# Guillaume-SOULIER/SOS-Radiative-Transfer

Measured on AMD Instinct MI355X. Metric: SOS columns/sec to 1e-4 convergence (Ntau=200, Nmu=128), higher is better.
Workload: dtype f64

## Files before the change

### __graft_entry__.py

```python
import os
import subprocess
import sys

ROOT = os.path.dirname(os.path.abspath(__file__))
PKG = os.path.join(ROOT, "sos-radiative-transfer_amd")
CSRC = os.path.join(PKG, "csrc")
LIB = os.path.join(PKG, "libsosrt.so")
SOURCES = ["api.hip", "kernels.hip", "jn_gemm.hip", "jn_gemm_f32.hip", "transport_fast.hip", "transport_ring.hip", "transport_scan.hip", "order_loop.hip", "epilogue.hip", "plan.cpp", "comm.cpp"]
HEADERS = ["kernels.hpp", "plan.hpp", "transport_util.hpp", "transport_scan_body.hpp", "jn_gemm_tile.hpp", "comm.hpp", os.path.join(ROOT, "include", "sosrt.h")]


OBJDIR = os.path.join(PKG, "build")
FLAGS = ["-O3", "--offload-arch=gfx950", "-std=c++17", "-fPIC", "-Wno-unused-value"]


def _deps():
    return [h if os.path.isabs(h) else os.path.join(CSRC, h) for h in HEADERS]


def _obj(src):
    return os.path.join(OBJDIR, src + ".o")


def _obj_stale(src):
    o = _obj(src)
    if not os.path.exists(o):
        return True
    t = os.path.getmtime(o)
    return any(os.path.getmtime(d) > t for d in [os.path.join(CSRC, src)] + _deps())


def _stale():
    if not os.path.exists(LIB):
        return True
    t = os.path.getmtime(LIB)
    deps = [os.path.join(CSRC, s) for s in SOURCES] + _deps()
    return any(os.path.getmtime(d) > t for d in deps)


def _hipcc():
    return os.environ.get("HIPCC") or ("/opt/rocm/bin/hipcc" if os.path.exists("/opt/rocm/bin/hipcc") else "hipcc")


def build(force: bool = False) -> None:
    if force or _stale():
        import fcntl
        with open(os.path.join(PKG, ".build.lock"), "w") as lock:
            fcntl.flock(lock, fcntl.LOCK_EX)
            if force or _stale():
                os.makedirs(OBJDIR, exist_ok=True)
                extra = os.environ.get("SOSRT_CXXFLAGS", "").split()
                todo = [s for s in SOURCES if force or extra or _obj_stale(s)]
                procs = []
                for src in todo:
                    cmd = [_hipcc()] + FLAGS + extra + ["-c", src, "-o", _obj(src)]
                    print("[build]", " ".join(cmd), file=sys.stderr, flush=True)
                    procs.append((src, subprocess.Popen(cmd, cwd=CSRC)))
                bad = [src for src, p in procs if p.wait() != 0]
                if bad:
                    raise RuntimeError("hipcc failed for: " + ", ".join(bad))
                tmp = LIB + ".tmp.%d" % os.getpid()
                cmd = [_hipcc(), "--offload-arch=gfx950", "-shared", "-fPIC", "-o", tmp] + [_obj(s) for s in SOURCES] + ["-ldl"]
                print("[build]", " ".join(cmd), file=sys.stderr, flush=True)
                subprocess.run(cmd, cwd=CSRC, check=True)
                os.replace(tmp, LIB)
    if PKG not in sys.path:
        sys.path.insert(0, PKG)
    import sosrt
    from sosrt import _lib
    _lib.lib()


def smoke() -> None:
    build()
    import numpy as np
    sys.path.insert(0, os.path.join(ROOT, "oracle"))
    import sos_oracle as O
    from sosrt.main import SOS_Aer
    p = dict(mu0=0.5, nb_layers=50, nb_angles=32, grd_alb=0.15, atm_phase_fun="iso", aer_phase_fun="iso")
    r = SOS_Aer(**p)
    mu = O.make_mu(32)
    P0, P = O.phase_isotropic(32, mu)
    c = O.make_column(0.5, 120, 25, 17, 50, 0.104, 0.120, 0.15, 1.0, 1.0, 32, P0, P, P0, P)
    ref = O.solve_column(c, literal=False)
    scale = np.max(np.abs(ref.I))
    sig = np.abs(ref.I) > 1e-9 * scale
    err = max(np.max(np.abs(r.I - ref.I)[sig] / np.abs(ref.I)[sig]), np.max(np.abs(r.I - ref.I)) / scale)
    print("[smoke] n=%d (oracle %d)  max rel err vs oracle %.3e  TOA-up max %.16g" % (r.n, ref.n, err, r.I[0, 32:].max()))
    assert r.n == ref.n and err < 1e-10, "HIP path disagrees with the oracle"


if __name__ == "__main__":
# ... 5 lines not shown
```

### include/sosrt.h

```cpp
#ifndef SOSRT_H
#define SOSRT_H

#ifdef __cplusplus
extern "C" {
#endif

typedef struct sosrt_handle sosrt_t;

#define SOSRT_OK              0
#define SOSRT_E_INVALID      -1
#define SOSRT_E_HIP          -2
#define SOSRT_E_STATE        -3
#define SOSRT_E_NOMEM        -4

#define SOSRT_COL_OK           0
#define SOSRT_COL_INDEXERROR   1
#define SOSRT_COL_MAXORDERS    2
#define SOSRT_COL_INTERNAL     3

#define SOSRT_GEOM_THREE_ZONE  0
#define SOSRT_GEOM_SINGLE_SLAB 1

#define SOSRT_SURFACE_NONE       0
#define SOSRT_SURFACE_SPECULAR   1
#define SOSRT_SURFACE_LAMBERTIAN 2
#define SOSRT_SURFACE_LAMBERTIAN_README 3

const char* sosrt_last_error(void);
#define SOSRT_VERSION 105
int sosrt_version(void);

int sosrt_create(int device, int L, int N, int max_batch, int max_orders, sosrt_t** out);
int sosrt_destroy(sosrt_t* h);
int sosrt_set_stream(sosrt_t* h, void* hip_stream);
int sosrt_use_own_stream(sosrt_t* h);
int sosrt_synchronize(sosrt_t* h);
int sosrt_set_saved_orders(sosrt_t* h, int slots);
int sosrt_set_order_budget(sosrt_t* h, int max_orders);

int sosrt_set_grid(sosrt_t* h, const double* mu);
int sosrt_set_phase(sosrt_t* h, const double* P_atm, const double* P_aer);

#define SOSRT_MAX_PHASE_SETS 64
int sosrt_set_phase_sets(sosrt_t* h, const double* P_atm, int S, const double* P_aer );
int sosrt_set_phase_sets_dev(sosrt_t* h, const double* P_atm , int S, const double* d_P_aer );
int sosrt_set_aerosol_sets(sosrt_t* h, int B, int nzmax, const int* zone_set );
int sosrt_phase_sets_info(sosrt_t* h, int* out );

int sosrt_set_atm_phase_sets(sosrt_t* h, int S_atm, const double* P_atm_sets );
int sosrt_set_atmosphere_sets(sosrt_t* h, int B, const int* col_set );
int sosrt_atm_sets_info(sosrt_t* h, int* out );

#define SOSRT_FIRST_ORDER_CODED 0
#define SOSRT_FIRST_ORDER_README 1
int sosrt_set_first_order(sosrt_t* h, int mode);

#define SOSRT_CONTRACT_F64 0
#define SOSRT_CONTRACT_F32 1
#define SOSRT_CONTRACT_F64_FULL 2
#define SOSRT_CONTRACT_F64_DENSE 3
#define SOSRT_SYMMETRY_TOL 1e-12
#define SOSRT_LOWRANK_TOL 1e-12
int sosrt_set_contraction(sosrt_t* h, int mode);

int sosrt_set_order_loop(sosrt_t* h, int mode);
int sosrt_order_loop_stats(sosrt_t* h, int* launches, int* refused, long long* column_orders );
int sosrt_phase_asymmetry(sosrt_t* h, double* asymmetry, int* uses_symmetry);
int sosrt_phase_rank(sosrt_t* h, int* rank, double* residual, int* uses);

int sosrt_set_columns(sosrt_t* h, int B, int geometry, int surface,
                      const int* idx_up, const int* idx_down,
                      const double* mu0, const double* grd_alb,
                      const double* alb_atm, const double* alb_aer,
                      const double* dtau_atm, const double* dtau_aer,
                      const double* tauStar_tot);

#define SOSRT_MAX_ZONES 8
int sosrt_set_columns_zones(sosrt_t* h, int B, int surface, int nzmax, const int* nz, const int* zone_r0, const int* zone_mix,
                            const double* mu0, const double* grd_alb, const double* alb_atm, const double* dtau_atm,
                            const double* zone_alb_aer, const double* zone_dtau_aer, const double* tauStar_tot);

int sosrt_first_order(sosrt_t* h, int B, const double* tau, const double* P0_atm, const double* P0_aer,
                      double* I1_out);
int sosrt_source(sosrt_t* h, int B, const double* In_1, double* Jn_out);
int sosrt_transport(sosrt_t* h, int B, const double* tau, const double* Jn, double* In_out, int* status_out);

int sosrt_solve(sosrt_t* h, int B, const double* tau, const double* P0_atm, const double* P0_aer,
                double tol, const double* I1_in,
                double* I_out, double* I_saved_out, int* n_orders_out, int* status_out);
int sosrt_solve_dev(sosrt_t* h, int B, const double* d_tau, const double* d_P0_atm, const double* d_P0_aer,
                    double tol, const double* d_I1_in,
                    double* d_I_out, double* d_I_saved_out, int* d_n_orders_out, int* d_status_out);
int sosrt_last_solve_stats(sosrt_t* h, int* max_orders_run, long long* sum_orders);

int sosrt_fluxes(sosrt_t* h, int B, const double* tau, const double* I, int beam_norm,
                 double* flux_down, double* flux_up);

int sosrt_epilogue_dev(sosrt_t* h, int B, const double* d_tau, const double* d_I, int beam_norm,
                       const double* d_z_profile, double* d_flux_down, double* d_flux_up, double* d_diffusivity,
                       double* d_heating_rate, double* d_net_toa);
int sosrt_epilogue(sosrt_t* h, int B, int beam_norm, const double* z_profile, double* flux_down, double* flux_up,
                   double* diffusivity, double* heating_rate, double* net_toa);

#define SOSRT_PHASE_ISO       0
#define SOSRT_PHASE_RAYLEIGH  1
#define SOSRT_PHASE_HG        2
#define SOSRT_PHASE_TABLE     3
int sosrt_phase_table(sosrt_t* h, const double* tab_mu, const double* tab_p, int ntab);
int sosrt_phase_table_dev(sosrt_t* h, const double* d_tab_mu, const double* d_tab_p, int ntab);

#define SOSRT_MIE_MAX_X 20000.0
#define SOSRT_MIE_MAX_MX 200000.0
#define SOSRT_MIE_MAX_WORKSPACE (2ull << 30)
int sosrt_mie_ensembles(sosrt_t* h, int S, const double* wl, const double* m_re, const double* m_im, const double* r_m,
                        const double* sig, int nb_radius, double r_min, double r_max, int ntab, double* p_out, double* bulk_out);
int sosrt_mie_ensembles_dev(sosrt_t* h, int S, const double* wl, const double* m_re, const double* m_im, const double* r_m,
                            const double* sig, int nb_radius, double r_min, double r_max, int ntab, double* d_p_out,
                            double* d_bulk_out);
int sosrt_mie_efficiencies(sosrt_t* h, int K, const double* m_re, const double* m_im, const double* x, double* out);
int sosrt_mie_timing(sosrt_t* h, double* ms );

int sosrt_phase_p0_dev(sosrt_t* h, int B, int kind, double g, const double* d_mu0, double* d_P0_out);
int sosrt_phase_p0(sosrt_t* h, int B, int kind, double g, const double* mu0, double* P0_out);
int sosrt_phase_matrix(sosrt_t* h, int kind, double g, double* P_out);
int sosrt_phase_matrix_dev(sosrt_t* h, int kind, double g, double* d_P_out);

#define SOSRT_MAX_MODES 64
int sosrt_phase_modes(sosrt_t* h, int kind, double g, int m_first, int m_count, int nphi, double* P_out);
int sosrt_phase_modes_dev(sosrt_t* h, int kind, double g, int m_first, int m_count, int nphi, int sign_odd, double* d_P_out);
int sosrt_phase_p0_modes_dev(sosrt_t* h, int B, int kind, double g, int m_first, int m_count, int nphi, const double* d_mu0,
                             double* d_P0_out);
int sosrt_phase_p0_modes(sosrt_t* h, int B, int kind, double g, int m_first, int m_count, int nphi, const double* mu0,
                         double* P0_out);
int sosrt_set_order_targets(sosrt_t* h, const int* d_targets);
int sosrt_azimuth_accumulate_dev(sosrt_t* h, int B, int m, const double* d_Im, int nlev, const int* d_levels, int nphi_out,
                                 const double* d_phi, double* d_out);
int sosrt_azimuth_synthesize_dev(sosrt_t* h, int B, int M, const double* d_I0, const double* d_Im, int nlev, const int* d_levels,
                                 int nphi_out, const double* d_phi, double* d_out);

int sosrt_comm_unique_id(void* id_out);
int sosrt_comm_init(sosrt_t* h, int rank, int world, const void* unique_id);
int sosrt_gather(sosrt_t* h, int root, const long long* counts, const double* d_send, double* d_recv);
int sosrt_comm_destroy(sosrt_t* h);

int sosrt_limit_mu_down(sosrt_t* h, int R, int idx, const double* rows, double* out);
int sosrt_asymptotic_down(sosrt_t* h, int R, int stride, const int* len, const double* J, const double* tau,
                          const double* tau_t, const double* mu, double* out);

int sosrt_plan_weights(sosrt_t* h, double* w_out );
// ... 33 lines not shown
```

### sos-radiative-transfer_amd/csrc/api.hip

```cpp
#include <hip/hip_runtime.h>

#include <algorithm>
#include <cmath>
#include <cstdarg>
#include <cstdio>
#include <cstdlib>
#include <chrono>
#include <cstring>
#include <mutex>
#include <new>
#include <string>
#include <vector>

#include "../../include/sosrt.h"
#include "comm.hpp"
#include "kernels.hpp"
#include "plan.hpp"

using namespace sosrt;

namespace {
thread_local std::string g_err;

int fail(int code, const char* fmt, ...) {
// ... 64 lines not shown
    char* h_mie = nullptr;
    size_t mie_cap = 0, mie_hcap = 0;
    hipEvent_t mie_ev = nullptr, mie_t[4] = {nullptr, nullptr, nullptr, nullptr};
    bool mie_timed = false;
    bool resident = false;
    int resident_B = 0;
    FixTab* d_fix = nullptr;
    int* d_small = nullptr;
    int *d_idx_up = nullptr, *d_idx_down = nullptr;
    int *d_nz = nullptr, *d_zr0 = nullptr, *d_zmix = nullptr;
    double *d_zwr = nullptr, *d_zdtr = nullptr;
    int max_nz = 1;
    bool simple_zones = true;
    double* d_scal = nullptr;
    ColDesc* d_desc = nullptr;
    double *d_rca = nullptr, *d_rcr = nullptr;
    int* d_slabrows = nullptr;
    int* d_mainrows = nullptr;
    int nslab = 0, nmain = 0;
    int max_main = 0, max_slab = 0;
    static constexpr int kMaxMixGroups = 32;
    static constexpr int kMaxMixGroupsSets = 128;
    static constexpr size_t kMixCacheBytes = 256ull << 20;
    int mix_groups_max = 1 << 30;
    bool wr_on_device = false;
    int nsets = 1;
    std::vector<std::vector<double>> Wrx_h;
    double* d_Wrsets = nullptr;
    size_t wrsets_capacity = 0;
    double* d_Wrsets_s = nullptr;
    size_t wrsets_s_capacity = 0;
    int* d_mixset = nullptr;
    int max_set_used = 0;
    int natm = 1;
    int max_atm_used = 0;
    std::vector<int> c_atmset;
    double* d_Wasets = nullptr;
    double *d_lrUsets = nullptr, *d_lrVsets = nullptr;
    int* d_lrranks = nullptr;
    int atm_capacity = 0;
    int* d_colatm = nullptr;
    int* d_mixatm = nullptr;
    int p0_zones = 0;
    double* d_P0rz = nullptr;
    size_t p0rz_capacity = 0;
    std::vector<int> c_nz, c_zr0, c_zmix, c_zset;
    std::vector<double> c_zwr, c_zdtr, c_alb_atm, c_dtau_atm;
    int mix_groups = 0;
    bool mix_dirty = true;
    double *d_Wmix = nullptr, *d_mixca = nullptr, *d_mixcr = nullptr;
    int* d_mixgroup = nullptr;
    int* d_slabtilegroup = nullptr;
    int contraction = SOSRT_CONTRACT_F64;
    double asymmetry = 0;
    bool sym_ok = false;
    bool sym_dirty = true, symmix_dirty = true, symsets_dirty = true;
    double *d_Wa_s = nullptr, *d_Wr_s = nullptr, *d_Wmix_s = nullptr;
    int lr_rank = -1;
    double lr_residual = 0;
    double *d_lrU = nullptr, *d_lrV = nullptr;
    size_t mixs_capacity = 0;
    float *d_Wa32 = nullptr, *d_Wmix32 = nullptr;
    size_t mix32_capacity = 0;
    bool w32_dirty = true;
    int* d_livelist = nullptr;
    size_t mix_capacity = 0;
    double *d_tau = nullptr, *d_P0a = nullptr, *d_P0r = nullptr;
    double *d_Jn = nullptr, *d_InA = nullptr, *d_InB = nullptr, *d_I = nullptr, *d_E = nullptr;
    int use_etab = 1;
    int *d_active = nullptr, *d_norders = nullptr, *d_status = nullptr, *d_redo = nullptr, *d_erep = nullptr;
    int *d_nactive_sets = nullptr, *d_nactive = nullptr;
    int nactive_set = 0;
    unsigned long long* d_tauhash = nullptr;
    int transport_mode = 3;
    int scan_cols = 200;
    bool ring_ok = false, scan_ok = false, scan_split_ok = false;
    int scan_split = 1;
    int cu_count = 0;
    double* d_scan_scratch = nullptr;
    int* d_scan_sync = nullptr;
    int gemm_tail_cols = 1 << 30;
    double gemm_tail_frac = 0.6;
    int gemm_small_cols = 200;
    int dense_live_list = 1;
    int gemm_regs_cols = -1;
    bool fast_ok = false;
    double* d_ratio = nullptr;
    int* h_pub = nullptr;
    bool need_small = true;
    int pub_seq = 0;
    int last_max_orders = 0;
    long long last_sum_orders = 0;
    Prof prof[kMaxGroups];
    int order_loop = 0;
    double ol_frac = 0.5;
    int* d_olsync = nullptr;
    int* h_oldone = nullptr;
    unsigned long long* d_ollog = nullptr;
    int ol_launches = 0, ol_refused = 0;
    bool ol_group_used[kMaxGroups] = {false, false};
    Rccl::comm_t comm = nullptr;
    int comm_rank = -1, comm_world = 0;
};

namespace {

size_t field_elems(const sosrt_handle* h) { return (size_t)h->max_batch * h->L * h->D; }

template <class T>
int dalloc(T** p, size_t n) {
    hipError_t e = hipMalloc((void**)p, n * sizeof(T));
    if (e != hipSuccess) return fail(SOSRT_E_NOMEM, "hipMalloc of %zu bytes failed: %s", n * sizeof(T), hipGetErrorString(e));
    return 0;
}

void mie_linspace(double a, double b, int n, double* out) {
    if (n == 1) { out[0] = a; return; }
    const double step = (b - a) / (n - 1);
    for (int i = 0; i < n; ++i) {
        volatile double t = i * step;
        out[i] = t + a;
    }
    out[n - 1] = b;
}

bool prof_room(Prof& p) {
    if (p.used + 2 > p.ev.size()) {
        const size_t n0 = p.ev.size();
        p.ev.resize(n0 + 4096);
        for (size_t i = n0; i < p.ev.size(); ++i)
            if (hipEventCreateWithFlags(&p.ev[i], hipEventDisableSystemFence) != hipSuccess) { p.ev.resize(i); break; }
        if (p.used + 2 > p.ev.size()) return false;
    }
    if (p.nint >= p.kind.size()) {
        const size_t n = p.kind.size() + 4096;
        p.kind.resize(n, -1); p.first.resize(n, 0); p.last.resize(n, 0);
    }
    return true;
}
hipStream_t group_stream(sosrt_handle* h, int grp) { return grp == 0 ? h->stream : h->stream2; }
void prof_begin(sosrt_handle* h, int kind, int grp = 0) {
    Prof& p = h->prof[grp];
    p.open = -1;
    if (!p.on || !prof_room(p)) return;
    if (p.adjacent >= 0) {
        p.open = p.adjacent;
    } else {
        p.open = (int)p.used++;
        hipEventRecord(p.ev[p.open], group_stream(h, grp));
    }
}
void prof_end(sosrt_handle* h, int kind, int grp = 0) {
    Prof& p = h->prof[grp];
    if (!p.on || p.open < 0) return;
    const int e = (int)p.used++;
    hipEventRecord(p.ev[e], group_stream(h, grp));
    p.kind[p.nint] = kind; p.first[p.nint] = p.open; p.last[p.nint] = e;
    ++p.nint;
    p.adjacent = e;
    p.open = -1;
}
void prof_break(sosrt_handle* h) { for (auto& p : h->prof) p.adjacent = -1; }

int need_gpu(sosrt_handle* h) {
    if (!h) return fail(SOSRT_E_INVALID, "null handle");
    if (!h->gpu) return fail(SOSRT_E_STATE, "handle was created host-only (device < 0)");
// ... 95 lines not shown
    if (!std::isfinite(wmax)) return -1;
    int rank = -1;
    for (int r = 0; r <= kLowRankMax; ++r) {
        size_t at = 0;
        const double amax = absmax(R, &at);
        *residual = wmax > 0 ? amax / wmax : amax;
        if (std::isnan(amax)) return -1;
        if (amax <= SOSRT_LOWRANK_TOL * wmax) { rank = r; break; }
        if (r == kLowRankMax) return -1;
        const int i = (int)(at / D), j = (int)(at % D);
        const long double piv = R[at];
        for (int k = 0; k < D; ++k) Ut[(size_t)r * D + k] = (double)(R[(size_t)k * D + j] / piv);
        for (int m = 0; m < D; ++m) V[(size_t)r * D + m] = R[(size_t)i * D + m];
        for (int k = 0; k < D; ++k) {
            const long double u = Ut[(size_t)r * D + k];
            double* row = &R[(size_t)k * D];
            const double* v = &V[(size_t)r * D];
            for (int m = 0; m < D; ++m) row[m] = (double)(row[m] - u * v[m]);
        }
    }
    double res = 0;
    for (int k = 0; k < D; ++k)
        for (int m = 0; m < D; ++m) {
            long double uv = 0;
            for (int q = 0; q < rank; ++q) uv += (long double)Ut[(size_t)q * D + k] * V[(size_t)q * D + m];
            const double d = std::fabs((double)(W[(size_t)k * D + m] - uv));
            if (!(d <= res)) res = d;
        }
    *residual = wmax > 0 ? res / wmax : res;
    return (res <= SOSRT_LOWRANK_TOL * wmax) ? rank : -1;
}

int ensure_matrices(sosrt_handle* h, hipStream_t s) {
    const Grid& g = h->g;
    const size_t per = (size_t)g.Dp * g.Wld;
    const bool mixed = h->mix_groups > 0 && h->mix_dirty;
    if (mixed) {
        prof_break(h);
        const bool sets = h->max_set_used > 0, atm = h->max_atm_used > 0;
        launch_wmix(s, per, h->mix_groups, atm ? h->d_Wasets : h->d_Wa, sets ? h->d_Wrsets : h->d_Wr, h->d_mixca, h->d_mixcr,
                    h->d_Wmix, sets ? h->d_mixset : nullptr, atm ? h->d_mixatm : nullptr);
        h->mix_dirty = false;
        h->symmix_dirty = true;
    }
    if (!use_sym(h)) return 0;
    if (h->sym_dirty) {
        prof_break(h);
        if (!h->d_Wa_s) { if (int e = dalloc(&h->d_Wa_s, per)) return e; }
        if (!h->d_Wr_s) { if (int e = dalloc(&h->d_Wr_s, per)) return e; }
        launch_symfold(s, 1, g.N, g.D, g.Dp, g.Wld, h->d_Wa, h->d_Wa_s);
        launch_symfold(s, 1, g.N, g.D, g.Dp, g.Wld, h->d_Wr, h->d_Wr_s);
        h->sym_dirty = false;
        h->symsets_dirty = true;
    }
    if (h->symsets_dirty && h->nsets > 1 && h->mix_groups == 0 && h->max_set_used > 0) {
        prof_break(h);
        {
            if (per * h->nsets > h->wrsets_s_capacity) {
                if (h->d_Wrsets_s) hipFree(h->d_Wrsets_s);
                h->d_Wrsets_s = nullptr; h->wrsets_s_capacity = 0;
                if (int e = dalloc(&h->d_Wrsets_s, per * h->nsets)) return e;
                h->wrsets_s_capacity = per * h->nsets;
            }
            launch_symfold(s, h->nsets, g.N, g.D, g.Dp, g.Wld, h->d_Wrsets, h->d_Wrsets_s);
        }
        h->symsets_dirty = false;
    }
    if (h->mix_groups > 0 && h->symmix_dirty) {
        prof_break(h);
        const size_t need = per * h->mix_groups;
        if (need > h->mixs_capacity) {
            if (h->d_Wmix_s) hipFree(h->d_Wmix_s);
            h->d_Wmix_s = nullptr; h->mixs_capacity = 0;
            if (int e = dalloc(&h->d_Wmix_s, need)) return e;
            h->mixs_capacity = need;
        }
        launch_symfold(s, h->mix_groups, g.N, g.D, g.Dp, g.Wld, h->d_Wmix, h->d_Wmix_s);
        h->symmix_dirty = false;
    }
    return 0;
}

void run_source(sosrt_handle* h, const double* In_1, double* Jn, const int* active, int tail_cols = 0, int pub_tag = 0,
                int grp = -1, bool all_live = false, bool regs_tile = false, int dense_live_cap = 0) {
    const int g0 = grp < 0 ? 0 : grp, g1 = grp < 0 ? h->ngroups : grp + 1;
    const int pg = grp < 0 ? 0 : grp;
    hipStream_t s = group_stream(h, pg);
    GemmArgs ga;
    ga.A = In_1; ga.Wa = h->d_Wa; ga.Wr = h->d_Wr; ga.ca = h->d_rca; ga.cr = h->d_rcr;
    if (h->nslab > 0) {
        ga.rows_main = h->d_mainrows + h->main_off[g0];
        ga.n_main = h->main_off[g1] - h->main_off[g0];
    } else {
        ga.rows_main = nullptr;
        ga.n_main = (h->gb[g1] - h->gb[g0]) * h->L;
        ga.A = In_1 + (size_t)h->gb[g0] * h->L * h->D;
        Jn += (size_t)h->gb[g0] * h->L * h->D;
        ga.ca = h->d_rca + (size_t)h->gb[g0] * h->L;
        ga.cr = h->d_rcr + (size_t)h->gb[g0] * h->L;
        if (active) active += h->gb[g0];
    }
    ga.rows_slab = h->d_slabrows + h->slab_off[g0]; ga.n_slab = h->slab_off[g1] - h->slab_off[g0];
    ga.D = h->g.D; ga.Dp = h->g.Dp; ga.Wld = h->g.Wld; ga.L = h->L; ga.C = Jn; ga.active = active;
    if (grp >= 0 && h->ngroups > 1) ga.pad_lds = h->coresident_pad;
    if (pub_tag) {
        ga.nactive = h->d_nactive + pg; ga.need_small = h->d_nactive + sosrt_handle::kMaxGroups;
        ga.host_pub = h->h_pub + 8 * pg; ga.tag = pub_tag;
    }
    ga.check_tiles = all_live ? 0 : 1;
    if (ensure_matrices(h, s)) return;
    if (h->mix_groups > 0) {
        ga.Wmix = h->d_Wmix; ga.mix_group = h->d_mixgroup; ga.slab_tile_group = h->d_slabtilegroup + h->slab_off[g0] / 32;
    }
    const bool two_pass_sets = h->mix_groups == 0 && h->max_set_used > 0 && h->nslab > 0;
    if (two_pass_sets) {
        ga.Wr = h->d_Wrsets; ga.mix_group = h->d_mixgroup; ga.slab_tile_group = h->d_slabtilegroup + h->slab_off[g0] / 32;
    }
    if (use_lowrank(h)) { ga.lr_rank = h->lr_rank; ga.lrU = h->d_lrU; ga.lrV = h->d_lrV; }
    AtmSets at;
    const AtmSets* atp = nullptr;
    if (h->max_atm_used > 0) {
        at.col_atm = h->d_colatm + (h->nslab > 0 ? 0 : h->gb[g0]);
        at.lr_ranks = h->d_lrranks;
        ga.lrU = h->d_lrUsets; ga.lrV = h->d_lrVsets;
        atp = &at;
    }
    if (use_sym(h)) {
        ga.sym = 1; ga.Ks = (h->g.N + GEMM_KC - 1) / GEMM_KC * GEMM_KC;
#ifdef SOSRT_DIAG
        if (h->diag_ks_mult > 1 && ga.Ks * h->diag_ks_mult <= h->g.Dp) ga.Ks *= h->diag_ks_mult;
#endif
        ga.Wa = h->d_Wa_s; ga.Wr = two_pass_sets ? h->d_Wrsets_s : h->d_Wr_s;
        if (ga.Wmix) ga.Wmix = h->d_Wmix_s;
    }
    if (h->contraction == SOSRT_CONTRACT_F32) {
        if (h->w32_dirty) {
            prof_break(h);
            const size_t per = (size_t)h->g.Dp * h->g.Wld;
            launch_to_float(s, per, h->d_Wa, h->d_Wa32);
            if (h->mix_groups > 0) launch_to_float(s, per * h->mix_groups, h->d_Wmix, h->d_Wmix32);
            h->w32_dirty = false;
        }
        prof_begin(h, SOSRT_K_GEMM, pg);
        launch_gemm_f32(s, ga, h->d_Wa32, h->d_Wmix32);
        prof_end(h, SOSRT_K_GEMM, pg);
        return;
    }
    prof_begin(h, SOSRT_K_GEMM, pg);
    if (tail_cols > 0 && active && h->nslab >= 0) {
        ga.col0 = h->nslab > 0 ? h->gb[g0] : 0; ga.B = h->gb[g1] - h->gb[g0];
        ga.max_main = h->max_main; ga.max_slab = h->max_slab;
        ga.idx_up = h->nslab > 0 ? h->d_idx_up : nullptr; ga.idx_down = h->nslab > 0 ? h->d_idx_down : nullptr;
        ga.live_list = h->d_livelist + h->gb[g0]; ga.live_cap = tail_cols;
        launch_gemm_tail(s, ga, tail_cols, tail_cols <= h->gemm_small_cols, regs_tile, atp);
    } else {
        if (dense_live_cap > 0 && active && h->nslab >= 0) {
            ga.col0 = h->nslab > 0 ? h->gb[g0] : 0; ga.B = h->gb[g1] - h->gb[g0];
            ga.live_list = h->d_livelist + h->gb[g0]; ga.live_cap = dense_live_cap;
        }
        launch_gemm(s, ga, atp);
    }
    prof_end(h, SOSRT_K_GEMM, pg);
}

struct SolveShape {
    bool ring_like = false;
    bool fast = false;
    int nzcap = kRingZones;
    int ring_mode = 1;
};
SolveShape solve_shape(const sosrt_handle* h, int max_nz) {
    SolveShape sh;
    sh.ring_like = h->transport_mode >= 2 && h->ring_ok && (max_nz <= kRingZones || transport_ring_fits(h->g, max_nz));
    sh.fast = h->transport_mode >= 1 && h->fast_ok && (max_nz <= kRingZones || sh.ring_like);
    sh.nzcap = max_nz > kRingZones ? max_nz : kRingZones;
    sh.ring_mode = (h->transport_mode >= 2 && h->ring_ok) ? 3 : 1;
    return sh;
}
struct OrderInputs {
    int nb = 0;
    int known = 0;
    int surface = SOSRT_SURFACE_NONE;
    bool simple_zones = true;
    bool slabs_mixed = true;
    bool need_small = false;
    bool saving = false;
    int orders_left = 1 << 30;
    int cu_share = 0;
};
struct LaunchPlan {
    int tail_cols = 0;
    int live_cap = 0;
    int gemm = SOSRT_PLAN_GEMM_DENSE;
    int transport = SOSRT_PLAN_TRANSPORT_GENERAL;
    int parts = 1;
    int repair = 0;
    int order_loop = 0;
    int ol_parts = 0;
    int ol_grid = 0;
};
LaunchPlan plan_order(const sosrt_handle* h, const SolveShape& sh, const OrderInputs& in) {
    LaunchPlan pl;
    const Grid& g = h->g;
    const bool live_tiling = h->contraction != SOSRT_CONTRACT_F32 && in.simple_zones && in.known <= h->gemm_tail_cols &&
                             (in.known <= h->gemm_tail_frac * in.nb || in.nb <= h->gemm_small_cols) &&
                             (in.known < in.nb || in.nb <= h->gemm_small_cols);
    pl.tail_cols = live_tiling ? in.known : 0;
    pl.gemm = !live_tiling ? SOSRT_PLAN_GEMM_DENSE
                           : (pl.tail_cols <= h->gemm_small_cols ? ((use_sym(h) && pl.tail_cols <= 32) ? SOSRT_PLAN_GEMM_LIVE32_DEEP : SOSRT_PLAN_GEMM_LIVE32)
                                                                 : SOSRT_PLAN_GEMM_LIVE64);
    {
        const int nct = (g.D + GEMM_BN - 1) / GEMM_BN;
        const int auto_cap = (3 * h->cu_count / 2) / (((g.L + 15) / 16 + 1) * nct);
        const int cap = h->gemm_regs_cols >= 0 ? h->gemm_regs_cols : auto_cap;
        if (live_tiling && use_sym(h) && pl.tail_cols <= cap && 16 * (g.D + 2) * 8 <= 150 * 1024 &&
            ((g.N + GEMM_KC - 1) / GEMM_KC * GEMM_KC) % 64 == 0) pl.gemm = SOSRT_PLAN_GEMM_LIVE16_REGS;
    }
    pl.live_cap = live_tiling ? pl.tail_cols : ((h->contraction != SOSRT_CONTRACT_F32 && h->dense_live_list && in.known < in.nb) ? in.known : 0);
    {
        const int cols_now = pl.live_cap > 0 ? pl.live_cap : in.nb;
        const int split_cap = sh.ring_mode == 3 ? h->cu_count : 4 * h->cu_count;
        const bool can_split = h->scan_split && h->scan_split_ok && transport_scan_parts(g) * cols_now <= split_cap &&
                               (in.surface == SOSRT_SURFACE_SPECULAR || in.surface == SOSRT_SURFACE_NONE);
        const bool want_scan = h->transport_mode == 4 || (h->transport_mode == 3 && cols_now <= h->scan_cols);
        const bool split = can_split && transport_scan_fits(g, sh.nzcap, true) && (sh.fast || (h->use_etab && h->transport_mode >= 3));
        const bool scan = want_scan && ((sh.fast && sh.ring_mode == 3 && h->scan_ok && transport_scan_fits(g, sh.nzcap, false)) || split);
        pl.transport = scan ? SOSRT_PLAN_TRANSPORT_SCAN
                            : (!sh.fast ? SOSRT_PLAN_TRANSPORT_GENERAL : (sh.ring_mode == 3 ? SOSRT_PLAN_TRANSPORT_RING : SOSRT_PLAN_TRANSPORT_FAST));
        if (scan && split) pl.parts = transport_scan_parts(g);
        pl.repair = (h->N - 3 > 61 && pl.transport == SOSRT_PLAN_TRANSPORT_FAST) ? 1 : 0;
    }
    if (h->order_loop && in.cu_share > 0 && h->transport_mode == 3 && sh.fast && sh.ring_mode == 3 && sh.nzcap <= kRingZones &&
        use_sym(h) && in.simple_zones && in.slabs_mixed && !in.saving && !in.need_small && in.orders_left >= 1 &&
        in.known <= kOrderLoopMaxCols) {
        Grid gt = g;
        gt.nsmall = 0;
        const bool split_ok = h->scan_split && (in.surface == SOSRT_SURFACE_SPECULAR || in.surface == SOSRT_SURFACE_NONE) && order_loop_ok(gt, true);
        const int sp = order_loop_parts(gt, true);
        if (split_ok && sp * in.known <= h->ol_frac * in.cu_share) {
            pl.order_loop = 1; pl.ol_parts = sp;
        } else if (order_loop_ok(gt, false) && in.known <= h->ol_frac * in.cu_share) {
            pl.order_loop = 1; pl.ol_parts = 1;
        }
        if (pl.order_loop) pl.ol_grid = in.cu_share;
    }
    return pl;
}

std::mutex g_ol_mutex;
int g_ol_held[64];
int ol_acquire(int device, int total, int want, int least) {
    if (device < 0 || device >= 64) return 0;
    std::lock_guard<std::mutex> lk(g_ol_mutex);
    int got = total - g_ol_held[device];
    if (got > want) got = want;
    if (got < least || got <= 0) return 0;
    g_ol_held[device] += got;
    return got;
}
void ol_release(int device, int n) {
    if (device < 0 || device >= 64 || n <= 0) return;
    std::lock_guard<std::mutex> lk(g_ol_mutex);
    g_ol_held[device] -= n;
}

}

extern "C" {

const char* sosrt_last_error(void) { return g_err.c_str(); }
int sosrt_version(void) { return SOSRT_VERSION; }

int sosrt_plan_fix_count(double tau_ref, int N) { return fix_count(tau_ref, N); }

int sosrt_create(int device, int L, int N, int max_batch, int max_orders, sosrt_t** out) {
    if (!out) return fail(SOSRT_E_INVALID, "out is null");
    *out = nullptr;
    if (L < 2) return fail(SOSRT_E_INVALID, "nb_layers must be >= 2 (got %d)", L);
    if (N < 4) return fail(SOSRT_E_INVALID, "nb_angles must be >= 4 (got %d)", N);
    if (N > 1024) return fail(SOSRT_E_INVALID, "nb_angles must be <= 1024 (got %d)", N);
    if (max_batch < 1 || max_orders < 1) return fail(SOSRT_E_INVALID, "max_batch and max_orders must be >= 1");
    {
        const int nt = (N + 63) / 64 * 64;
        const size_t need = (size_t)(3 * (size_t)L + nt + nt / 64 + 4) * sizeof(double);
        if (need > 64 * 1024)
            return fail(SOSRT_E_INVALID, "nb_layers = %d does not fit: at most %d layers at nb_angles = %d", L,
                        (int)((64 * 1024 / sizeof(double) - nt - nt / 64 - 4) / 3), N);
    }
    sosrt_handle* h = new (std::nothrow) sosrt_handle();
    if (!h) return fail(SOSRT_E_NOMEM, "out of host memory");
    h->device = device; h->L = L; h->N = N; h->D = 2 * N; h->max_batch = max_batch; h->max_orders = max_orders;
    h->order_budget = max_orders;
    h->saved_slots = max_orders;
    h->gpu = device >= 0;
    h->cu_count = 256;
    if (const char* ev = getenv("SOSRT_ETAB")) h->use_etab = atoi(ev);
    if (const char* ev = getenv("SOSRT_CONTRACT"))
        if (strcmp(ev, "full") == 0) h->contraction = SOSRT_CONTRACT_F64_FULL;
    if (const char* ev = getenv("SOSRT_TRANSPORT"))
        h->transport_mode = strcmp(ev, "general") == 0 ? 0 : (strcmp(ev, "ring") == 0 ? 2 : (strcmp(ev, "scan") == 0 ? 4 : (strcmp(ev, "auto") == 0 ? 3 : 1)));
    if (const char* ev = getenv("SOSRT_SCAN_COLS")) h->scan_cols = atoi(ev);
    if (const char* ev = getenv("SOSRT_SCAN_SPLIT")) h->scan_split = atoi(ev);
    if (const char* ev = getenv("SOSRT_GEMM_TAIL")) h->gemm_tail_cols = atoi(ev);
    if (const char* ev = getenv("SOSRT_GEMM_TAIL_FRAC")) h->gemm_tail_frac = atof(ev);
    if (const char* ev = getenv("SOSRT_GEMM_SMALL")) h->gemm_small_cols = atoi(ev);
    if (const char* ev = getenv("SOSRT_DENSE_LIVE_LIST")) h->dense_live_list = atoi(ev) != 0;
    if (const char* ev = getenv("SOSRT_GEMM_REGS")) h->gemm_regs_cols = atoi(ev);
    if (const char* ev = getenv("SOSRT_GROUPS")) h->want_groups = atoi(ev) >= 2 ? 2 : (atoi(ev) == 1 ? 1 : 0);
    if (const char* ev = getenv("SOSRT_SPLIT_MIN")) h->split_min = atoi(ev);
    if (const char* ev = getenv("SOSRT_MIX_GROUPS")) h->mix_groups_max = atoi(ev);
#ifdef SOSRT_DIAG
    if (const char* ev = getenv("SOSRT_STAGGER")) h->stagger = atof(ev);
    if (const char* ev = getenv("SOSRT_GROUP_SPLIT")) h->split_at = atoi(ev);
    if (const char* ev = getenv("SOSRT_GROUP_PRIO")) h->prio2 = atoi(ev);
    if (const char* ev = getenv("SOSRT_GEMM_PAD_LDS")) h->coresident_pad = atoi(ev);
    if (const char* ev = getenv("SOSRT_GEMM_KS_MULT")) h->diag_ks_mult = atoi(ev);
#endif
    if (const char* ev = getenv("SOSRT_GROUP_RING_SLOTS")) h->coresident_slots = atoi(ev);
    if (const char* ev = getenv("SOSRT_ORDER_LOOP")) h->order_loop = atoi(ev) != 0;
    if (const char* ev = getenv("SOSRT_RING_SLOTS")) g_ring_slots = atoi(ev);
#ifdef SOSRT_RING_DEBUG
    if (const char* ev = getenv("SOSRT_RING_DEBUG")) g_ring_debug = atoi(ev);
#endif
    Grid& g = h->g;
    g.L = L; g.N = N; g.D = 2 * N;
    g.Dp = (g.D + GEMM_KC - 1) / GEMM_KC * GEMM_KC;
    g.Wld = (g.D + GEMM_BN - 1) / GEMM_BN * GEMM_BN;
    if (h->gpu) {
        int e = 0;
        auto body = [&]() -> int {
            HIPCHK(hipSetDevice(device));
            HIPCHK(hipStreamCreateWithFlags(&h->own_stream, hipStreamDefault));
            h->stream = h->own_stream;
            HIPCHK(hipEventCreateWithFlags(&h->ev_fork, hipEventDisableTiming));
            HIPCHK(hipEventCreateWithFlags(&h->ev_join, hipEventDisableTiming));
            const size_t mb = max_batch, fe = field_elems(h);
            if ((e = dalloc(&h->d_mu, g.D))) return e;
            if ((e = dalloc(&h->d_Wa, (size_t)g.Dp * g.Wld))) return e;
            if ((e = dalloc(&h->d_Wr, (size_t)g.Dp * g.Wld))) return e;
            if ((e = dalloc(&h->d_lrU, (size_t)kLowRankMax * g.D))) return e;
            if ((e = dalloc(&h->d_lrV, (size_t)kLowRankMax * g.D))) return e;
            if ((e = dalloc(&h->d_wfdn, N))) return e;
            if ((e = dalloc(&h->d_wfup, N))) return e;
            if ((e = dalloc(&h->d_w, g.D))) return e;
            if ((e = dalloc(&h->d_phi, 2 * kNPhi))) return e;
            if ((e = dalloc(&h->d_z, L))) return e;
            if ((e = dalloc(&h->d_fix, 4))) return e;
            if ((e = dalloc(&h->d_small, N))) return e;
            if ((e = dalloc(&h->d_idx_up, mb))) return e;
            if ((e = dalloc(&h->d_idx_down, mb))) return e;
            if ((e = dalloc(&h->d_nz, mb))) return e;
            if ((e = dalloc(&h->d_zr0, mb * kMaxZones))) return e;
            if ((e = dalloc(&h->d_zmix, mb * kMaxZones))) return e;
            if ((e = dalloc(&h->d_zwr, mb * kMaxZones))) return e;
            if ((e = dalloc(&h->d_zdtr, mb * kMaxZones))) return e;
            if ((e = dalloc(&h->d_scal, 7 * mb))) return e;
            if ((e = dalloc(&h->d_desc, mb))) return e;
            if ((e = dalloc(&h->d_rca, mb * L))) return e;
            if ((e = dalloc(&h->d_rcr, mb * L))) return e;
            if ((e = dalloc(&h->d_slabrows, mb * L + 64 * (size_t)sosrt_handle::kMaxMixGroupsSets * sosrt_handle::kMaxGroups))) return e;
            if ((e = dalloc(&h->d_slabtilegroup, mb * L / 32 + 2 * sosrt_handle::kMaxMixGroupsSets * sosrt_handle::kMaxGroups + 2))) return e;
            if ((e = dalloc(&h->d_mainrows, mb * L))) return e;
            if ((e = dalloc(&h->d_tau, mb * L))) return e;
            if ((e = dalloc(&h->d_P0a, mb * g.D))) return e;
            if ((e = dalloc(&h->d_P0r, mb * g.D))) return e;
            if ((e = dalloc(&h->d_Jn, fe))) return e;
            if ((e = dalloc(&h->d_InA, fe))) return e;
            if ((e = dalloc(&h->d_InB, fe))) return e;
            if ((e = dalloc(&h->d_I, fe))) return e;
            if ((e = dalloc(&h->d_E, fe))) return e;
            if ((e = dalloc(&h->d_active, mb))) return e;
            if ((e = dalloc(&h->d_norders, mb))) return e;
            if ((e = dalloc(&h->d_status, mb))) return e;
            if ((e = dalloc(&h->d_nactive_sets, 2 * (sosrt_handle::kMaxGroups + 1)))) return e;
            HIPCHK(hipMemset(h->d_nactive_sets, 0, 2 * (sosrt_handle::kMaxGroups + 1) * sizeof(int)));
            h->d_nactive = h->d_nactive_sets;
            if ((e = dalloc(&h->d_redo, mb))) return e;
            if ((e = dalloc(&h->d_erep, mb))) return e;
            if ((e = dalloc(&h->d_mixgroup, mb))) return e;
            if ((e = dalloc(&h->d_livelist, mb))) return e;
            if ((e = dalloc(&h->d_mixca, sosrt_handle::kMaxMixGroupsSets))) return e;
            if ((e = dalloc(&h->d_mixcr, sosrt_handle::kMaxMixGroupsSets))) return e;
            if ((e = dalloc(&h->d_mixset, sosrt_handle::kMaxMixGroupsSets))) return e;
            if ((e = dalloc(&h->d_mixatm, sosrt_handle::kMaxMixGroupsSets))) return e;
            if ((e = dalloc(&h->d_colatm, mb))) return e;
            if ((e = dalloc(&h->d_tauhash, mb))) return e;
            if ((e = dalloc(&h->d_ratio, mb))) return e;
            if ((e = dalloc(&h->d_scan_scratch, mb * transport_scan_scratch_doubles()))) return e;
            if ((e = dalloc(&h->d_scan_sync, 2 * mb))) return e;
            if ((e = dalloc(&h->d_olsync, sosrt_handle::kMaxGroups * order_loop_sync_ints(kOrderLoopMaxCols)))) return e;
            HIPCHK(hipHostMalloc((void**)&h->h_oldone, 2 * sosrt_handle::kMaxGroups * sizeof(int), hipHostMallocCoherent));
            memset(h->h_oldone, 0, 2 * sosrt_handle::kMaxGroups * sizeof(int));
            HIPCHK(hipMemset(h->d_scan_sync, 0, 2 * mb * sizeof(int)));
            HIPCHK(hipDeviceGetAttribute(&h->cu_count, hipDeviceAttributeMultiprocessorCount, device));
            HIPCHK(hipHostMalloc((void**)&h->h_pub, (8 * sosrt_handle::kMaxGroups + 2) * sizeof(int), hipHostMallocCoherent));
            memset(h->h_pub, 0, (8 * sosrt_handle::kMaxGroups + 2) * sizeof(int));

            HIPCHK(hipMemset(h->d_Wa, 0, (size_t)g.Dp * g.Wld * sizeof(double)));
            HIPCHK(hipMemset(h->d_Wr, 0, (size_t)g.Dp * g.Wld * sizeof(double)));
            HIPCHK(hipMemset(h->d_status, 0, mb * sizeof(int)));
            HIPCHK(hipMemset(h->d_redo, 0, mb * sizeof(int)));
            HIPCHK(hipMemset(h->d_tau, 0, mb * L * sizeof(double)));
            return 0;
        };
        if ((e = body())) { sosrt_destroy(h); return e; }
        g.mu = h->d_mu; g.Wa = h->d_Wa; g.Wr = h->d_Wr; g.fix = h->d_fix; g.small_lanes = h->d_small;
        g.wflux_dn = h->d_wfdn; g.wflux_up = h->d_wfup; g.nsmall = 0;
    }
    *out = h;
    return 0;
}

int sosrt_destroy(sosrt_t* h) {
    if (!h) return 0;
    if (h->gpu) {
        hipSetDevice(h->device);
        if (h->comm) { rccl().CommDestroy(h->comm); h->comm = nullptr; }
        if (h->own_stream) hipStreamSynchronize(h->own_stream);
        void* ptrs[] = {h->d_mu, h->d_Wa, h->d_Wr, h->d_wfdn, h->d_wfup, h->d_fix, h->d_small, h->d_idx_up,
                        h->d_idx_down, h->d_scal, h->d_desc, h->d_rca, h->d_rcr, h->d_slabrows, h->d_mainrows, h->d_tau, h->d_P0a,
                        h->d_P0r, h->d_Jn, h->d_InA, h->d_InB, h->d_I, h->d_E, h->d_active, h->d_norders, h->d_status,
                        h->d_nactive_sets, h->d_ratio, h->d_redo, h->d_erep, h->d_tauhash, h->d_Wmix, h->d_mixca, h->d_mixcr,
                        h->d_mixgroup, h->d_Wa_s, h->d_Wr_s, h->d_Wmix_s, h->d_scan_scratch, h->d_scan_sync, h->d_w, h->d_phi, h->d_z, h->d_tab, h->d_slabtilegroup, h->d_livelist, h->d_Wa32, h->d_Wmix32, h->d_nz, h->d_zr0, h->d_zmix, h->d_zwr, h->d_zdtr, h->d_olsync, h->d_ollog, h->d_modetab, h->d_lrU, h->d_lrV, h->d_Wrsets, h->d_Wrsets_s, h->d_mixset, h->d_P0rz,
                        h->d_Wasets, h->d_lrUsets, h->d_lrVsets, h->d_lrranks, h->d_colatm, h->d_mixatm};
        for (void* p : ptrs)
            if (p) hipFree(p);
        if (h->h_pub) hipHostFree(h->h_pub);
        if (h->h_oldone) hipHostFree(h->h_oldone);
        if (h->d_mie) hipFree(h->d_mie);
        if (h->h_mie) hipHostFree(h->h_mie);
        if (h->mie_ev) hipEventDestroy(h->mie_ev);
        for (auto& e : h->mie_t)
            if (e) hipEventDestroy(e);

        for (auto& p : h->prof)
            for (auto& e : p.ev) hipEventDestroy(e);
        if (h->stream2) { hipStreamSynchronize(h->stream2); hipStreamDestroy(h->stream2); }
        if (h->ev_fork) hipEventDestroy(h->ev_fork);
        if (h->ev_join) hipEventDestroy(h->ev_join);
        if (h->own_stream) hipStreamDestroy(h->own_stream);
    }
    delete h;
    return 0;
}

int sosrt_set_stream(sosrt_t* h, void* s) {
    if (int e = need_gpu(h)) return e;
    h->stream = (hipStream_t)s;
    return 0;
}

int sosrt_use_own_stream(sosrt_t* h) {
    if (int e = need_gpu(h)) return e;
    h->stream = h->own_stream;
    return 0;
}

int sosrt_set_saved_orders(sosrt_t* h, int slots) {
    if (!h) return fail(SOSRT_E_INVALID, "null handle");
    if (slots < 1 || slots > h->max_orders) return fail(SOSRT_E_INVALID, "slots must be in 1..max_orders=%d (got %d)", h->max_orders, slots);
    h->saved_slots = slots;
    return 0;
}

int sosrt_set_order_budget(sosrt_t* h, int max_orders) {
    if (!h) return fail(SOSRT_E_INVALID, "null handle");
    if (max_orders < 1 || max_orders > h->max_orders)
        return fail(SOSRT_E_INVALID, "the order budget must be in 1..max_orders=%d of sosrt_create (got %d)", h->max_orders, max_orders);
    h->order_budget = max_orders;
    return 0;
}

int sosrt_set_first_order(sosrt_t* h, int mode) {
    if (int e = need_gpu(h)) return e;
    if (mode != SOSRT_FIRST_ORDER_CODED && mode != SOSRT_FIRST_ORDER_README) return fail(SOSRT_E_INVALID, "unknown first-order mode %d", mode);
    if (mode == SOSRT_FIRST_ORDER_README && (h->nsets > 1 || h->p0_zones > 0))
        return fail(SOSRT_E_INVALID, "SOSRT_FIRST_ORDER_README reads one aerosol matrix: it cannot be combined with several phase sets");
    if (mode == SOSRT_FIRST_ORDER_README && (h->natm > 1 || h->max_atm_used > 0))
        return fail(SOSRT_E_INVALID, "SOSRT_FIRST_ORDER_README reads one atmosphere matrix: it cannot be combined with atmosphere phase sets");
    if (mode == SOSRT_FIRST_ORDER_README && h->geom != SOSRT_GEOM_THREE_ZONE)
        return fail(SOSRT_E_INVALID, "the README's Lambertian first order needs the three-zone geometry (it has a surface)");
    h->first_order_mode = mode;
    return 0;
}

int sosrt_set_contraction(sosrt_t* h, int mode) {
    if (int e = need_gpu(h)) return e;
    if (mode != SOSRT_CONTRACT_F64 && mode != SOSRT_CONTRACT_F32 && mode != SOSRT_CONTRACT_F64_FULL && mode != SOSRT_CONTRACT_F64_DENSE) return fail(SOSRT_E_INVALID, "unknown contraction mode %d", mode);
    if (mode != SOSRT_CONTRACT_F64 && (h->natm > 1 || h->max_atm_used > 0))
        return fail(SOSRT_E_INVALID, "atmosphere phase sets are in use: their plain rows exist in the low-rank form of SOSRT_CONTRACT_F64 only "
                                     "(the other contractions tile row lists that straddle columns)");
    if (mode == SOSRT_CONTRACT_F32) {
        HIPCHK(hipSetDevice(h->device));
        const size_t per = (size_t)h->g.Dp * h->g.Wld;
        if (!h->d_Wa32) { if (int e = dalloc(&h->d_Wa32, per)) return e; }
        h->w32_dirty = true;
    }
    h->contraction = mode;
    return 0;
}

int sosrt_set_order_loop(sosrt_t* h, int mode) {
    if (!h) return fail(SOSRT_E_INVALID, "null handle");
    if (mode < 0 || mode > 2) return fail(SOSRT_E_INVALID, "order-loop mode must be 0, 1 or 2 (got %d)", mode);
    h->order_loop = mode;
    return 0;
}

int sosrt_order_loop_stats(sosrt_t* h, int* launches, int* refused, long long* column_orders) {
    if (!h) return fail(SOSRT_E_INVALID, "null handle");
    if (launches) *launches = h->ol_launches;
    if (refused) *refused = h->ol_refused;
    if (column_orders) {
        *column_orders = 0;
        if (h->gpu && h->ol_launches > 0) {
            HIPCHK(hipSetDevice(h->device));
            HIPCHK(hipStreamSynchronize(h->stream));
            if (h->stream2) HIPCHK(hipStreamSynchronize(h->stream2));
            for (int k = 0; k < sosrt_handle::kMaxGroups; ++k) {
                if (!h->ol_group_used[k]) continue;
                int v = 0;
                HIPCHK(hipMemcpy(&v, h->d_olsync + (size_t)k * order_loop_sync_ints(kOrderLoopMaxCols) + kOlOrders, sizeof v, hipMemcpyDeviceToHost));
                *column_orders += v;
            }
        }
    }
    return 0;
}

int sosrt_plan_launch(sosrt_t* h, int batch, int live, int surface, int zones, int cus, int* out) {
    if (!h || !out) return fail(SOSRT_E_INVALID, "null argument");
    if (!h->have_grid) return fail(SOSRT_E_STATE, "sosrt_set_grid has not been called");
    if (batch < 1 || live < 0 || live > batch) return fail(SOSRT_E_INVALID, "need 0 <= live <= batch, batch >= 1");
    if (zones < 1 || zones > kMaxZones) return fail(SOSRT_E_INVALID, "zones must be in 1..%d", kMaxZones);
    int want = h->want_groups;
    if (want == 0) want = batch > h->split_min ? 2 : 1;
    const int ng = (want >= 2 && batch >= h->split_min && batch >= 2) ? 2 : 1;
    const int nb = ng == 2 ? batch / 2 : batch;
    const int saved_cus = h->cu_count;
    if (cus > 0) h->cu_count = cus;
    const SolveShape sh = solve_shape(h, zones);
    OrderInputs oi;
    oi.nb = nb; oi.known = live < nb ? live : nb; oi.surface = surface;
    oi.simple_zones = zones == 3 || zones == 1;
    oi.cu_share = h->cu_count / ng;
    const bool saved_sym = h->sym_ok;
    if (!h->have_phase) h->sym_ok = true;
    const LaunchPlan pl = plan_order(h, sh, oi);
    h->sym_ok = saved_sym;
    h->cu_count = saved_cus;
    out[0] = ng; out[1] = pl.gemm; out[2] = pl.tail_cols; out[3] = pl.transport; out[4] = pl.parts; out[5] = pl.repair;
    out[6] = pl.order_loop; out[7] = pl.ol_parts; out[8] = pl.ol_grid;
    return 0;
}

int sosrt_phase_asymmetry(sosrt_t* h, double* asymmetry, int* uses_symmetry) {
    if (!h) return fail(SOSRT_E_INVALID, "null handle");
    if (!h->have_phase) return fail(SOSRT_E_STATE, "sosrt_set_phase has not been called");
    if (asymmetry) *asymmetry = h->asymmetry;
    if (uses_symmetry) *uses_symmetry = use_sym(h) ? 1 : 0;
    return 0;
}

int sosrt_phase_rank(sosrt_t* h, int* rank, double* residual, int* uses) {
    if (!h) return fail(SOSRT_E_INVALID, "null handle");
    if (!h->have_phase) return fail(SOSRT_E_STATE, "sosrt_set_phase has not been called");
    if (rank) *rank = h->lr_rank;
    if (residual) *residual = h->lr_residual;
    if (uses) *uses = use_lowrank(h) ? 1 : 0;
    return 0;
}

int sosrt_synchronize(sosrt_t* h) {
    if (int e = need_gpu(h)) return e;
    HIPCHK(hipStreamSynchronize(h->stream));
    return 0;
}

int sosrt_set_grid(sosrt_t* h, const double* mu) {
    if (!h || !mu) return fail(SOSRT_E_INVALID, "null argument");
    for (int k = 0; k < h->D; ++k)
        if (!std::isfinite(mu[k])) return fail(SOSRT_E_INVALID, "mu[%d] is not finite", k);
    for (int k = 0; k < h->N; ++k) {
        if (!(mu[k] <= 0)) return fail(SOSRT_E_INVALID, "mu[%d]=%g: the first nb_angles directions must be <= 0", k, mu[k]);
        if (!(mu[h->N + k] >= 0)) return fail(SOSRT_E_INVALID, "mu[%d]=%g: the last nb_angles directions must be >= 0", h->N + k, mu[h->N + k]);
    }
    h->plan.set_grid(h->N, mu);
    for (int b = 0; b < 4; ++b)
        if (h->plan.fix[b].idx > kFixMaxIdx) return fail(SOSRT_E_INVALID, "nb_angles too large for the extrapolation tables");
    h->have_grid = true;
    h->have_phase = false;
    h->fast_ok = transport_fast_ok(h->plan);
    if (h->gpu) {
        HIPCHK(hipSetDevice(h->device));
        HIPCHK(hipMemcpy(h->d_mu, mu, h->D * sizeof(double), hipMemcpyHostToDevice));
        HIPCHK(hipMemcpy(h->d_wfdn, h->plan.wflux_dn.data(), h->N * sizeof(double), hipMemcpyHostToDevice));
        HIPCHK(hipMemcpy(h->d_wfup, h->plan.wflux_up.data(), h->N * sizeof(double), hipMemcpyHostToDevice));
        HIPCHK(hipMemcpy(h->d_w, h->plan.w.data(), h->D * sizeof(double), hipMemcpyHostToDevice));
        {
            double phi[kNPhi], tab[2 * kNPhi];
            const double step = 3.141592653589793 / (kNPhi - 1);
            for (int q = 0; q < kNPhi; ++q) phi[q] = q * step;
            phi[kNPhi - 1] = 3.141592653589793;
            for (int q = 0; q < kNPhi; ++q) {
                tab[q] = std::cos(0 - phi[q]);
                tab[kNPhi + q] = ((q > 0 ? phi[q] - phi[q - 1] : 0.0) + (q + 1 < kNPhi ? phi[q + 1] - phi[q] : 0.0)) / 2;
            }
            HIPCHK(hipMemcpy(h->d_phi, tab, sizeof tab, hipMemcpyHostToDevice));
        }
// ... 702 lines not shown
    const double* src = I1 + (size_t)b * n;
    for (size_t i = tid; i < n; i += blockDim.x) {
        const double v = src[i];
        In1[(size_t)b * n + i] = v;
        I[(size_t)b * n + i] = v;
        if (saved) saved[(size_t)b * saved_col_stride + i] = v;
    }
    if (tid == 0) {
        double a = 1.0 / src[g.N];
        for (int m = g.N + 1; m < g.D; ++m) { const double x = 1.0 / src[m]; if (x > a) a = x; }
        const double* last = src + (size_t)(g.L - 1) * g.D;
        double bb = 1.0 / last[0];
        for (int m = 1; m < g.N; ++m) { const double x = 1.0 / last[m]; if (x > bb) bb = x; }
        const double r = (bb > a) ? bb : a;
        cv.ratio[b] = r; cv.norders[b] = 1; cv.status[b] = SOSRT_COL_OK;
        const int go = conv_go(cv, b, 1, r) ? 1 : 0;
        cv.active[b] = go;
        if (go) atomicAdd(cv.nactive, 1);
    }
}

int sosrt_solve_dev(sosrt_t* h, int B, const double* d_tau, const double* d_P0_atm, const double* d_P0_aer, double tol,
                    const double* d_I1_in, double* d_I_out, double* d_I_saved_out, int* d_n_orders_out,
                    int* d_status_out) {
    if (int e = check_ready(h, B, true)) return e;
    if (!d_tau || !d_I_out) return fail(SOSRT_E_INVALID, "null argument");
    if (!d_I1_in && !d_P0_atm) return fail(SOSRT_E_INVALID, "P0_atm is required unless I1 is supplied");
    if (!d_I1_in && h->geom == SOSRT_GEOM_THREE_ZONE && !d_P0_aer) return fail(SOSRT_E_INVALID, "three-zone geometry needs P0_aer");
    if (h->max_orders >= 65536) return fail(SOSRT_E_INVALID, "max_orders must be < 65536");
    HIPCHK(hipSetDevice(h->device));
    if (int e = ensure_w32(h)) return e;
    hipStream_t s = h->stream;
    const Grid& g = h->g;
    const size_t LD = (size_t)h->L * h->D;
    const size_t saved_stride = (size_t)h->saved_slots * LD;
    const int NG = h->ngroups;

    prof_break(h);
    h->nactive_set ^= 1;
    h->d_nactive = h->d_nactive_sets + h->nactive_set * (sosrt_handle::kMaxGroups + 1);
    SolveSetup su;
    su.zero_next = h->d_nactive_sets + (h->nactive_set ^ 1) * (sosrt_handle::kMaxGroups + 1);
    su.n_zero = sosrt_handle::kMaxGroups + 1;
    su.redo = h->d_redo;
    su.hash = h->d_tauhash;
    su.scan_sync = h->d_scan_sync;
    launch_prepare(s, g, B, h->geom, h->surface, scalars_of(h), d_tau, h->d_desc, h->d_rca, h->d_rcr,
                   h->d_nactive + sosrt_handle::kMaxGroups, su);
    h->need_small = true;
    const int small_tag = ((++h->pub_seq) & 0x3fffffff) | 0x40000000;
    bool small_published = false;
    const SolveShape shape = solve_shape(h, h->max_nz);
    const bool fast = shape.fast;
    const int nzcap = shape.nzcap;
    if (h->use_etab || fast) {
        launch_tau_groups(s, g, B, d_tau, h->d_tauhash, h->d_erep, h->d_nactive + sosrt_handle::kMaxGroups,
                          h->h_pub + 8 * sosrt_handle::kMaxGroups, small_tag);
        launch_attenuation(s, g, B, d_tau, h->d_E, h->d_erep);
        small_published = true;
    }
    if (int e = ensure_matrices(h, s)) return e;
    bool forked = false;
    int ol_held[sosrt_handle::kMaxGroups] = {0, 0};
    auto bail = [&](int code) {
        if (forked && hipEventRecord(h->ev_join, h->stream2) == hipSuccess) (void)hipStreamWaitEvent(s, h->ev_join, 0);
        for (int k = 0; k < NG; ++k)
            if (ol_held[k]) {
                (void)hipStreamSynchronize(group_stream(h, k));
                ol_release(h->device, ol_held[k]);
                ol_held[k] = 0;
            }
        return code;
    };

    struct GroupState {
        int b0 = 0, nb = 0, n = 1, known = 0;
        bool done = false, started = false;
        bool ol_pending = false, ol_off = false;
        int ol_tag = 0;
        unsigned ol_polls = 0;
        double *In_1 = nullptr, *In = nullptr;
        Conv cv;
    } gs[sosrt_handle::kMaxGroups];
    h->ol_launches = 0; h->ol_refused = 0;
    for (bool& u : h->ol_group_used) u = false;
    bool used_order_loop = false;
    const int tagbase = ((++h->pub_seq) & 0x3fff) << 16;
    for (int k = 0; k < NG; ++k) {
        GroupState& q = gs[k];
        q.b0 = h->gb[k]; q.nb = h->gb[k + 1] - h->gb[k]; q.known = q.nb;
        q.In_1 = h->d_InA; q.In = h->d_InB;
        if (!d_I1_in && h->first_order_mode != SOSRT_FIRST_ORDER_README) q.In_1 = d_I_out;
        q.cv = make_conv(h, tol);
        q.cv.active += q.b0; q.cv.norders += q.b0; q.cv.status += q.b0; q.cv.ratio += q.b0; q.cv.redo += q.b0;
        q.cv.nactive = h->d_nactive + k;
        if (h->d_targets) q.cv.target = h->d_targets + q.b0;
    }
    auto start_group = [&](int k) {
        GroupState& q = gs[k];
        q.started = true;
        hipStream_t sg = group_stream(h, k);
        const size_t fo = (size_t)q.b0 * LD;
        prof_begin(h, SOSRT_K_FIRST, k);
        if (d_I1_in)
            hipLaunchKernelGGL(k_init_from_I1, dim3(q.nb), dim3(256), 0, sg, g, d_I1_in + fo, q.In_1 + fo, d_I_out + fo,
                               d_I_saved_out ? d_I_saved_out + (size_t)q.b0 * saved_stride : nullptr, saved_stride, q.cv);
        else if (h->first_order_mode == SOSRT_FIRST_ORDER_README)
            launch_first_order_readme(sg, g, h->d_w, q.nb, d_tau + (size_t)q.b0 * h->L, d_P0_atm + (size_t)q.b0 * g.D,
                                      d_P0_aer ? d_P0_aer + (size_t)q.b0 * g.D : nullptr, h->d_desc + q.b0, q.In_1 + fo,
                                      d_I_out + fo, d_I_saved_out ? d_I_saved_out + (size_t)q.b0 * saved_stride : nullptr,
                                      saved_stride, q.cv, 1);
        else
            launch_first_order(sg, g, q.nb, d_tau + (size_t)q.b0 * h->L, d_P0_atm + (size_t)q.b0 * g.D,
                               d_P0_aer ? d_P0_aer + (size_t)q.b0 * g.D * (h->p0_zones > 0 ? h->p0_zones : 1) : nullptr, h->d_desc + q.b0,
                               d_I_out + fo, nullptr, d_I_saved_out ? d_I_saved_out + (size_t)q.b0 * saved_stride : nullptr, saved_stride,
                               q.cv, 1, h->p0_zones);
        prof_end(h, SOSRT_K_FIRST, k);
    };
    start_group(0);
    if (NG > 1) {
        HIPCHK(hipEventRecord(h->ev_fork, s));
        HIPCHK(hipStreamWaitEvent(h->stream2, h->ev_fork, 0));
        forked = true;
    }
    if (small_published && g.nsmall > 0) {
        volatile int* slot = h->h_pub + 8 * sosrt_handle::kMaxGroups;
        const auto t0 = std::chrono::steady_clock::now();
        for (unsigned it = 1; __atomic_load_n(&slot[1], __ATOMIC_ACQUIRE) != small_tag; ++it) {
            if ((it & 0x3fff) == 0 && std::chrono::steady_clock::now() - t0 > std::chrono::seconds(120))
                return bail(fail(SOSRT_E_HIP, "order loop: no progress for 120 s"));
            __builtin_ia32_pause();
        }
        h->need_small = slot[0] != 0;
    }
    int live_groups = NG, n_max = 1;
    while (live_groups > 0) {
        bool progressed = false;
        for (int k = 0; k < NG; ++k) {
            GroupState& q = gs[k];
            if (q.done) continue;
            if (q.ol_pending) {
                volatile int* dw = h->h_oldone + 2 * k;
                if (__atomic_load_n(&dw[1], __ATOMIC_ACQUIRE) != q.ol_tag) {
                    if ((++q.ol_polls & 0x3fff) != 0) continue;
                    const hipError_t qe = hipStreamQuery(group_stream(h, k));
                    if (qe != hipSuccess && qe != hipErrorNotReady) return bail(fail(SOSRT_E_HIP, "order loop: %s", hipGetErrorString(qe)));
                    if (qe == hipSuccess && __atomic_load_n(&dw[1], __ATOMIC_ACQUIRE) != q.ol_tag)
                        return bail(fail(SOSRT_E_HIP, "order loop: the order-loop launch ended without reporting"));
                    continue;
                }
                const int state = dw[0];
                q.ol_pending = false;
                ol_release(h->device, ol_held[k]);
                ol_held[k] = 0;
                progressed = true;
#ifdef SOSRT_OL_STAMPS
                if (h->d_ollog && getenv("SOSRT_OL_LOG")) {
                    std::vector<unsigned long long> lg(65001);
                    (void)hipStreamSynchronize(group_stream(h, k));
                    (void)hipMemcpy(lg.data(), h->d_ollog, lg.size() * 8, hipMemcpyDeviceToHost);
                    if (FILE* f = fopen(getenv("SOSRT_OL_LOG"), "a")) {
                        fprintf(f, "# launch columns<=%d order0=%d events=%llu\n", q.known, q.n + 1, lg[0]);
                        for (unsigned long long i = 0; i < lg[0] && i < 65000; ++i)
                            fprintf(f, "%llu %llu %llu %llu\n", lg[1 + i] >> 48, (lg[1 + i] >> 40) & 0xff, (lg[1 + i] >> 32) & 0xff, lg[1 + i] & 0xffffffffull);
                        fclose(f);
                    }
                }
// ... 14 lines not shown
                                     w[kOlArrive], w[kOlLeft], q.n + 1, q.known, cols.c_str()));
                }
                q.ol_off = true;
                ++h->ol_refused;
            }
            if (!q.started) {
                const GroupState& p = gs[k - 1];
                if (!(p.done || (p.n >= 2 && p.known <= h->stagger * p.nb))) continue;
                start_group(k);
            }
            progressed = true;
            if (q.n >= h->order_budget) { q.done = true; --live_groups; continue; }
            if (q.n >= 2) {
                const int live = wait_published(h, k, tagbase + q.n - 1);
                if (live < 0) return bail(live);
                if (live == 0) { q.done = true; --live_groups; continue; }
                q.known = live;
            }
            hipStream_t sg = group_stream(h, k);
            const size_t fo = (size_t)q.b0 * LD;
            const double* tau_g = d_tau + (size_t)q.b0 * h->L;
            const int* erep_g = h->d_erep + q.b0;
            OrderInputs oi;
            oi.nb = q.nb; oi.known = q.known; oi.surface = h->surface;
            oi.simple_zones = h->simple_zones; oi.slabs_mixed = h->nslab == 0 || h->mix_groups > 0;
            oi.need_small = g.nsmall > 0 && h->need_small; oi.saving = d_I_saved_out != nullptr;
            oi.orders_left = h->order_budget - q.n;
            oi.cu_share = (q.ol_off || h->d_targets || h->max_atm_used > 0) ? 0 : h->cu_count / NG;
            LaunchPlan pl = plan_order(h, shape, oi);
            if (pl.order_loop) {
                const int got = ol_acquire(h->device, h->cu_count, pl.ol_grid, (int)(pl.ol_parts * q.known / h->ol_frac));
                if (got == 0) { oi.cu_share = 0; pl = plan_order(h, shape, oi); }
                else { pl.ol_grid = got; ol_held[k] = got; }
            }
            if (pl.order_loop && h->order_loop == 2) pl.ol_grid = 2 * h->cu_count;
            if (pl.order_loop) {
                OrderLoopArgs oa;
                Grid gt = g;
                gt.nsmall = 0;
                oa.t = TransportArgs{gt, tau_g, h->d_Jn + fo, nullptr, d_I_out + fo, nullptr, 0, h->d_desc + q.b0, q.cv, 0, 1, h->d_E, erep_g, nullptr};
                oa.t.nzcap = kRingZones;
                oa.t.scan_split = pl.ol_parts > 1 ? 1 : 0;
                oa.t.scan_scratch = h->d_scan_scratch + (size_t)q.b0 * transport_scan_scratch_doubles();
                oa.t.scan_sync = h->d_scan_sync + 2 * q.b0;
                GemmArgs& ga = oa.gm;
                ga.A = nullptr; ga.Wa = h->d_Wa_s; ga.Wr = h->d_Wr_s; ga.ca = h->d_rca; ga.cr = h->d_rcr;
                ga.D = g.D; ga.Dp = g.Dp; ga.Wld = g.Wld; ga.L = h->L; ga.C = h->d_Jn;
                ga.sym = 1; ga.Ks = (g.N + GEMM_KC - 1) / GEMM_KC * GEMM_KC;
                if (use_lowrank(h)) { ga.lr_rank = h->lr_rank; ga.lrU = h->d_lrU; ga.lrV = h->d_lrV; }
                ga.max_main = h->max_main; ga.max_slab = h->max_slab;
                ga.idx_up = h->nslab > 0 ? h->d_idx_up : nullptr; ga.idx_down = h->nslab > 0 ? h->d_idx_down : nullptr;
                if (h->mix_groups > 0) { ga.Wmix = h->d_Wmix_s; ga.mix_group = h->d_mixgroup; }
                oa.in0 = q.In_1;
                oa.gbufP = q.In;
                oa.gbufQ = (q.In_1 == d_I_out) ? h->d_InA : q.In_1;
                oa.bufP = oa.gbufP + fo; oa.bufQ = oa.gbufQ + fo;
                oa.order0 = q.n + 1; oa.kmax = h->order_budget - q.n;
                oa.B = q.nb; oa.col0 = q.b0;
                oa.fixcap = (int)(0.06 * g.N) + 1;
                oa.sync = h->d_olsync + (size_t)k * order_loop_sync_ints(kOrderLoopMaxCols);
                oa.host_done = h->h_oldone + 2 * k;
                oa.tag = q.ol_tag = ((++h->pub_seq) & 0x3fffffff) | 0x40000000;
#ifdef SOSRT_OL_STAMPS
                if (getenv("SOSRT_OL_LOG")) {
                    if (!h->d_ollog) { if (int e = dalloc(&h->d_ollog, 65001)) return bail(e); }
                    HIPCHK(hipMemsetAsync(h->d_ollog, 0, 8, sg));
                    oa.log = h->d_ollog;
                }
#endif
                prof_break(h);
                HIPCHK(hipMemsetAsync(oa.sync, 0, order_loop_sync_ints(q.known) * sizeof(int), sg));
                prof_begin(h, SOSRT_K_ORDER_LOOP, k);
                const hipError_t le = launch_order_loop(sg, pl.ol_grid, pl.ol_parts > 1, oa);
                prof_end(h, SOSRT_K_ORDER_LOOP, k);
                if (le != hipSuccess) return bail(fail(SOSRT_E_HIP, "order-loop launch failed: %s", hipGetErrorString(le)));
                q.ol_pending = true;
                used_order_loop = true;
                ++h->ol_launches;
                continue;
            }
            const int n = ++q.n;
            n_max = n > n_max ? n : n_max;
            const int tail_cols = pl.tail_cols;
            run_source(h, q.In_1, h->d_Jn, h->d_active, tail_cols, tagbase + n - 1, k, q.known == q.nb, pl.gemm == SOSRT_PLAN_GEMM_LIVE16_REGS,
                       tail_cols > 0 ? 0 : pl.live_cap);
            if (g.nsmall > 0 && h->need_small) {
                prof_begin(h, SOSRT_K_SMALLMU, k);
                launch_smallmu(sg, g, q.nb, tau_g, h->d_Jn + fo, q.In + fo, h->d_desc + q.b0, q.cv.active);
                prof_end(h, SOSRT_K_SMALLMU, k);
            }
            prof_begin(h, SOSRT_K_TRANSPORT, k);
            double* sv_n = (d_I_saved_out && n <= h->saved_slots) ? d_I_saved_out + (size_t)q.b0 * saved_stride + (size_t)(n - 1) * LD : nullptr;
            if (pl.transport != SOSRT_PLAN_TRANSPORT_GENERAL) {
                Grid gt = g;
                if (pl.transport >= SOSRT_PLAN_TRANSPORT_RING && !h->need_small) gt.nsmall = 0;
                launch_transport(sg, gt, q.nb, tau_g, h->d_Jn + fo, q.In + fo, d_I_out + fo, sv_n, saved_stride, h->d_desc + q.b0, q.cv, n, 1,
                                 h->d_E, pl.transport, erep_g, pl.live_cap, h->d_livelist + q.b0, NG > 1 ? h->coresident_slots : 0,
                                 pl.parts > 1 ? 1 : 0, h->d_scan_scratch + (size_t)q.b0 * transport_scan_scratch_doubles(),
                                 h->d_scan_sync + 2 * q.b0, nzcap);
                if (pl.repair)
                    launch_transport(sg, g, q.nb, tau_g, h->d_Jn + fo, q.In + fo, d_I_out + fo, sv_n, saved_stride, h->d_desc + q.b0, q.cv, n, 1,
                                     h->d_E, 2, erep_g);
            } else {
                launch_transport(sg, g, q.nb, tau_g, h->d_Jn + fo, q.In + fo, d_I_out + fo, sv_n, saved_stride, h->d_desc + q.b0, q.cv, n, 1,
                                 h->use_etab ? h->d_E : nullptr, 0, erep_g);
            }
            prof_end(h, SOSRT_K_TRANSPORT, k);
            if (q.In_1 == d_I_out) { q.In_1 = q.In; q.In = h->d_InA; }
            else { double* tmp = q.In_1; q.In_1 = q.In; q.In = tmp; }
        }
        if (!progressed) __builtin_ia32_pause();
    }
    if (NG > 1) {
        HIPCHK(hipEventRecord(h->ev_join, h->stream2));
        HIPCHK(hipStreamWaitEvent(s, h->ev_join, 0));
    }
    prof_break(h);
    launch_finalize(s, B, make_conv(h, tol), h->order_budget, d_n_orders_out, d_status_out);
    HIPCHK(hipGetLastError());
    h->last_max_orders = used_order_loop ? -1 : n_max;
    h->last_sum_orders = -1;
    return 0;
}

int sosrt_solve(sosrt_t* h, int B, const double* tau, const double* P0_atm, const double* P0_aer, double tol,
                const double* I1_in, double* I_out, double* I_saved_out, int* n_orders_out, int* status_out) {
    if (int e = check_ready(h, B, true)) return e;
    if (!tau) return fail(SOSRT_E_INVALID, "null argument");
    HIPCHK(hipSetDevice(h->device));
    hipStream_t s = h->stream;
    h->resident = false;
    const size_t LD = (size_t)h->L * h->D, n = (size_t)B * LD;
    HIPCHK(hipMemcpyAsync(h->d_tau, tau, (size_t)B * h->L * sizeof(double), hipMemcpyHostToDevice, s));
    if (P0_atm) HIPCHK(hipMemcpyAsync(h->d_P0a, P0_atm, (size_t)B * h->D * sizeof(double), hipMemcpyHostToDevice, s));
    const double* d_p0r = nullptr;
    if (int e = stage_p0_aer(h, B, P0_aer, s, &d_p0r)) return e;
    double* d_I1 = nullptr;
    double* d_saved = nullptr;
    int rc = 0;
    auto body = [&]() -> int {
        if (I1_in) {
            if (int e = dalloc(&d_I1, n)) return e;
            HIPCHK(hipMemcpyAsync(d_I1, I1_in, n * sizeof(double), hipMemcpyHostToDevice, s));
        }
        if (I_saved_out) {
            if (int e = dalloc(&d_saved, (size_t)B * h->saved_slots * LD)) return e;
            HIPCHK(hipMemsetAsync(d_saved, 0, (size_t)B * h->saved_slots * LD * sizeof(double), s));
        }
        if (int e = sosrt_solve_dev(h, B, h->d_tau, P0_atm ? h->d_P0a : nullptr, d_p0r, tol, d_I1,
                                    h->d_I, d_saved, nullptr, nullptr))
            return e;
        if (I_out) HIPCHK(hipMemcpyAsync(I_out, h->d_I, n * sizeof(double), hipMemcpyDeviceToHost, s));
        if (I_saved_out)
            HIPCHK(hipMemcpyAsync(I_saved_out, d_saved, (size_t)B * h->saved_slots * LD * sizeof(double), hipMemcpyDeviceToHost, s));
        std::vector<int> no(B);
        HIPCHK(hipMemcpyAsync(no.data(), h->d_norders, B * sizeof(int), hipMemcpyDeviceToHost, s));
        if (status_out) HIPCHK(hipMemcpyAsync(status_out, h->d_status, B * sizeof(int), hipMemcpyDeviceToHost, s));
        HIPCHK(hipStreamSynchronize(s));
        long long sum = 0;
        int mx = 1;
        for (int b = 0; b < B; ++b) { sum += no[b] - 1; mx = no[b] > mx ? no[b] : mx; if (n_orders_out) n_orders_out[b] = no[b]; }
        h->last_sum_orders = sum;
        if (h->last_max_orders < 0) h->last_max_orders = mx;
        h->resident = true; h->resident_B = B;
        return 0;
    };
    rc = body();
    if (d_I1) hipFree(d_I1);
    if (d_saved) hipFree(d_saved);
    return rc;
}

int sosrt_last_solve_stats(sosrt_t* h, int* max_orders_run, long long* sum_orders) {
    if (int e = need_gpu(h)) return e;
    if ((h->last_sum_orders < 0 || h->last_max_orders < 0) && h->B > 0) {
        std::vector<int> no(h->B);
        HIPCHK(hipMemcpyAsync(no.data(), h->d_norders, h->B * sizeof(int), hipMemcpyDeviceToHost, h->stream));
        HIPCHK(hipStreamSynchronize(h->stream));
        long long sum = 0;
        int mx = 1;
        for (int v : no) { sum += v - 1; mx = v > mx ? v : mx; }
        h->last_sum_orders = sum;
// ... 762 lines not shown
```

### sos-radiative-transfer_amd/csrc/jn_gemm_tile.hpp

```cpp
#pragma once
#include "kernels.hpp"
#include "transport_util.hpp"

namespace sosrt {

namespace {

typedef double f64x4 __attribute__((ext_vector_type(4)));

constexpr int A_LD = GEMM_KC + 2;
constexpr int B_LD = GEMM_BN + 16;

struct ListRows {
    const int* rows;
    int n;
    __device__ int operator()(int lr) const { return lr < n ? (rows ? rows[lr] : lr) : -1; }
};
struct ColumnRows {
    int base, iu, ns, n;
    bool slab;
    __device__ int operator()(int lr) const {
        if (lr >= n) return -1;
        return base + (slab ? iu + lr : (lr < iu ? lr : lr + ns));
    }
};

template <int RT, bool SLAB, bool DEEP = false, bool SYM = false, class RowOf = ListRows, bool COH = false, bool ASTAGE = false>
__device__ __forceinline__ void gemm_tile(const GemmArgs& g, double* sA, double* sB, int* s_any, int tile, int bn0,
                                          RowOf row_of, bool check_active, const double* __restrict__ wmix = nullptr,
                                          double* sRaw = nullptr) {
    static_assert(!ASTAGE || (COH && DEEP), "ASTAGE is a form of the order-loop launch's tile");
    constexpr int BM = 16 * RT;
    double* const sAv = sA + BM * A_LD;
    const int Nn = g.D >> 1, Nh = g.Wld >> 1;
    int tid_ = threadIdx.x;
    if (COH) asm volatile("" : "+v"(tid_));
    const int tid = tid_, lane = tid & 63;
    const int wave = __builtin_amdgcn_readfirstlane(tid) >> 6;
    const int D = g.D, Dp = g.Dp, Wld = g.Wld;
    constexpr bool slab = SLAB;
    const int bm0 = tile * BM;

    const int arow = tid >> 2, akq = (tid & 3) * (GEMM_KC / 4);
    int grow = -1;
    if (arow < BM) grow = row_of(bm0 + arow);
    if (check_active && g.active && g.check_tiles) {
        if (tid == 0) *s_any = 0;
        __syncthreads();
        if ((tid & 3) == 0 && grow >= 0 && g.active[grow / g.L]) *s_any = 1;
        __syncthreads();
        if (!*s_any) return;
    }
    __shared__ int s_rowid[16 * (GEMM_RT > 2 ? GEMM_RT : 2)];
    if ((tid & 3) == 0 && arow < BM) s_rowid[arow] = grow;
    const double coef_a = grow >= 0 ? (wmix ? 1.0 : g.ca[grow]) : 0.0;
    const double coef_r = (slab && grow >= 0) ? g.cr[grow] : 0.0;
    const double* __restrict__ Arow = g.A + (size_t)(grow >= 0 ? grow : 0) * D;
    int colrow0 = 0;
    if constexpr (COH) colrow0 = row_of.base;
    const int colbytes = COH ? g.L * D * 8 : 0;
    const __amdgpu_buffer_rsrc_t rA = make_rsrc(g.A + (size_t)colrow0 * D, colbytes);
    const __amdgpu_buffer_rsrc_t rC = make_rsrc(g.C + (size_t)colrow0 * D, colbytes);
    const int avo = ((grow >= 0 ? grow : colrow0) - colrow0) * D * 8;
    const int RS = D + 2;
    if constexpr (ASTAGE) {
        typedef __attribute__((address_space(3))) void* lds_ptr_t_;
        __syncthreads();
        const int rowbytes = D * 8, pieces = (rowbytes + 1023) / 1024;
        for (int r = wave; r < BM; r += 4) {
            const int gr_ = s_rowid[r];
            if (gr_ < 0) continue;
            const int ro = (gr_ - colrow0) * rowbytes;
            for (int pc = 0; pc < pieces; ++pc)
                if (pc * 1024 + lane * 16 < rowbytes)
                    __builtin_amdgcn_raw_ptr_buffer_load_lds(rA, (lds_ptr_t_)(sRaw + (size_t)r * RS + pc * 128), 16, lane * 16, ro + pc * 1024, 0, 16);
        }
        asm volatile("s_waitcnt vmcnt(0)" ::: "memory");
        __syncthreads();
    }
#define SOSRT_A2(off_) (ASTAGE ? *reinterpret_cast<const double2*>(sRaw + (size_t)arow * RS + (off_)) \
                               : (COH ? bload2_aux<16>(rA, avo + (off_) * 8, 0) : *reinterpret_cast<const double2*>(Arow + (off_))))

    f64x4 acc[RT][2];
#pragma unroll
// ... 200 lines not shown
    }
}
template <bool SLAB, bool PRELOADED>
__device__ __forceinline__ void gemm_tile_lone(const GemmArgs& g, double* sRaw, int tile, int bn0, ColumnRows row_of,
                                               LoneFrag& f0, LoneFrag& f1, const double* __restrict__ wmix = nullptr) {
    static_assert(!(SLAB && PRELOADED), "two passes start from the column's own coefficients");
    typedef __attribute__((address_space(3))) void* lds_ptr_t_;
    const int tid = threadIdx.x, lane = tid & 63;
    const int wave = __builtin_amdgcn_readfirstlane(tid) >> 6;
    const int D = g.D, Wld = g.Wld, Nn = D >> 1, Nh = Wld >> 1;
    const int RS = D + 2;
    const int fr = lane & 15, fk = lane >> 4;
    const int nkb = (g.Ks >> 2) / LONE_KB;
    const int nblk = (SLAB ? 2 : 1) * nkb;
    const int grow = row_of(tile * 16 + fr);
    const double cf_a = grow >= 0 ? (wmix ? 1.0 : g.ca[grow]) : 0.0;
    const double cf_r = (SLAB && grow >= 0) ? g.cr[grow] : 0.0;
    const __amdgpu_buffer_rsrc_t rA = make_rsrc(g.A + (size_t)row_of.base * D, g.L * D * 8);
    const int rowbytes = D * 8, pieces = (rowbytes + 1023) / 1024;
    for (int r = wave; r < 16; r += 4) {
        const int gr_ = row_of(tile * 16 + r);
        if (gr_ < 0) continue;
        const int ro = (gr_ - row_of.base) * rowbytes;
        for (int pc = 0; pc < pieces; ++pc)
            if (pc * 1024 + lane * 16 < rowbytes)
                __builtin_amdgcn_raw_ptr_buffer_load_lds(rA, (lds_ptr_t_)(sRaw + (size_t)r * RS + pc * 128), 16, lane * 16, ro + pc * 1024, 0, 0);
    }
    const int mcol = (bn0 >> 1) + wave * 16 + fr;
#define SOSRT_LONE_LOAD(F, blk_)                                                                                  \
    {                                                                                                             \
        const int b_ = (blk_);                                                                                    \
        if (b_ < nblk) {                                                                                          \
            const int pass_ = b_ >= nkb ? 1 : 0;                                                                  \
            lone_load(F, pass_ ? rW1 : rW0, b_ - pass_ * nkb, fk, Wld, Nh, mcol);                                 \
        }                                                                                                         \
    }
    const __amdgpu_buffer_rsrc_t rW0 = make_rsrc(wmix ? wmix : g.Wa, g.Dp * Wld * 8);
    const __amdgpu_buffer_rsrc_t rW1 = make_rsrc(SLAB ? g.Wr : g.Wa, g.Dp * Wld * 8);
    if (!PRELOADED) {
        SOSRT_LONE_LOAD(f0, 0);
        SOSRT_LONE_LOAD(f1, 1);
    }
    asm volatile("s_waitcnt vmcnt(0)" ::: "memory");
    __syncthreads();
    f64x4 accx = (f64x4){0, 0, 0, 0}, accy = (f64x4){0, 0, 0, 0};
    const double* __restrict__ arow = sRaw + (size_t)fr * RS;
#define SOSRT_LONE_COMPUTE(F, blk_)                                                                               \
    {                                                                                                             \
        const int b_ = (blk_);                                                                                    \
        const int pass_ = b_ >= nkb ? 1 : 0;                                                                      \
        const double cf_ = pass_ ? cf_r : cf_a;                                                                   \
        const int k0_ = 4 * (b_ - pass_ * nkb) * LONE_KB + fk;                                                    \
        _Pragma("unroll") for (int q = 0; q < LONE_KB; ++q) {                                                     \
            const int k_ = k0_ + 4 * q;                                                                           \
            const bool ok_ = grow >= 0 && k_ < Nn;                                                                \
            const double a_ = arow[k_], m_ = arow[D - 1 - k_];                  \
            const double u_ = ok_ ? cf_ * (a_ + m_) : 0.0, v_ = ok_ ? cf_ * (a_ - m_) : 0.0;                      \
            accx = __builtin_amdgcn_mfma_f64_16x16x4f64(u_, F.s[q], accx, 0, 0, 0);                               \
            accy = __builtin_amdgcn_mfma_f64_16x16x4f64(v_, F.a[q], accy, 0, 0, 0);                               \
        }                                                                                                         \
    }
    for (int blk = 0; blk < nblk; blk += 2) {
        SOSRT_LONE_COMPUTE(f0, blk);
        SOSRT_LONE_LOAD(f0, blk + 2);
        if (blk + 1 < nblk) {
            SOSRT_LONE_COMPUTE(f1, blk + 1);
            SOSRT_LONE_LOAD(f1, blk + 3);
        }
    }
#undef SOSRT_LONE_LOAD
#undef SOSRT_LONE_COMPUTE
#pragma unroll
    for (int r = 0; r < 4; ++r) {
        const int gr = row_of(tile * 16 + 4 * r + fk);
        if (gr >= 0 && mcol < Nn) {
            const double x = accx[r], y = accy[r];
            g.C[(size_t)gr * D + mcol] = x + y;
            g.C[(size_t)gr * D + D - 1 - mcol] = x - y;
        }
    }
}

constexpr int LR_ROWS = 4;
template <bool COH, bool ATM = false>
__device__ __forceinline__ void lowrank_rows(const GemmArgs& g, const int (&rows)[LR_ROWS], int lane, const AtmSets& at = AtmSets()) {
    const int D = g.D, R = g.lr_rank;
    __amdgpu_buffer_rsrc_t rA[LR_ROWS], rC[LR_ROWS];
    double cf[LR_ROWS];
    int Ri[LR_ROWS];
    const double* __restrict__ Ui[LR_ROWS];
    const double* __restrict__ Vi[LR_ROWS];
#pragma unroll
    for (int i = 0; i < LR_ROWS; ++i) {
        const int r = rows[i] >= 0 ? rows[i] : rows[0];
        const int bytes = rows[i] >= 0 ? D * 8 : 0;
        rA[i] = make_rsrc(g.A + (size_t)r * D, bytes);
        rC[i] = make_rsrc(g.C + (size_t)r * D, bytes);
        cf[i] = rows[i] >= 0 ? g.ca[rows[i]] : 0.0;
        if constexpr (ATM) {
            const int st = __builtin_amdgcn_readfirstlane(at.col_atm[r / g.L]);
            Ri[i] = __builtin_amdgcn_readfirstlane(at.lr_ranks[st]);
            Ui[i] = g.lrU + (size_t)st * kLowRankMax * D;
            Vi[i] = g.lrV + (size_t)st * kLowRankMax * D;
        }
    }
    const double* __restrict__ U = g.lrU;
    const double* __restrict__ V = g.lrV;
    double m[LR_ROWS][kLowRankMax];
#pragma unroll
    for (int i = 0; i < LR_ROWS; ++i)
#pragma unroll
        for (int q = 0; q < kLowRankMax; ++q) m[i][q] = 0.0;
#pragma unroll 2
    for (int k = 2 * lane; k < D; k += 128) {
        double2 x[LR_ROWS];
#pragma unroll
        for (int i = 0; i < LR_ROWS; ++i) x[i] = bload2_aux<COH ? 16 : 0>(rA[i], k * 8, 0);
#pragma unroll
        for (int q = 0; q < kLowRankMax; ++q) {
            if constexpr (ATM) {
#pragma unroll
                for (int i = 0; i < LR_ROWS; ++i)
                    if (q < Ri[i]) {
                        const double2 u = *reinterpret_cast<const double2*>(Ui[i] + (size_t)q * D + k);
                        m[i][q] = __builtin_fma(x[i].y, u.y, __builtin_fma(x[i].x, u.x, m[i][q]));
                    }
            } else if (q < R) {
                const double2 u = *reinterpret_cast<const double2*>(U + (size_t)q * D + k);
#pragma unroll
                for (int i = 0; i < LR_ROWS; ++i) m[i][q] = __builtin_fma(x[i].y, u.y, __builtin_fma(x[i].x, u.x, m[i][q]));
            }
        }
    }
#pragma unroll
    for (int s = 32; s >= 1; s >>= 1)
#pragma unroll
        for (int q = 0; q < kLowRankMax; ++q) {
            if constexpr (ATM) {
#pragma unroll
                for (int i = 0; i < LR_ROWS; ++i)
                    if (q < Ri[i]) m[i][q] += __shfl_xor(m[i][q], s);
            } else if (q < R) {
#pragma unroll
                for (int i = 0; i < LR_ROWS; ++i) m[i][q] += __shfl_xor(m[i][q], s);
            }
        }
#pragma unroll 2
    for (int k = 2 * lane; k < D; k += 128) {
        double2 o[LR_ROWS];
#pragma unroll
        for (int i = 0; i < LR_ROWS; ++i) o[i] = make_double2(0.0, 0.0);
#pragma unroll
        for (int q = 0; q < kLowRankMax; ++q) {
            if constexpr (ATM) {
#pragma unroll
                for (int i = 0; i < LR_ROWS; ++i)
                    if (q < Ri[i]) {
                        const double2 v = *reinterpret_cast<const double2*>(Vi[i] + (size_t)q * D + k);
                        o[i].x = __builtin_fma(m[i][q], v.x, o[i].x);
                        o[i].y = __builtin_fma(m[i][q], v.y, o[i].y);
                    }
            } else if (q < R) {
                const double2 v = *reinterpret_cast<const double2*>(V + (size_t)q * D + k);
#pragma unroll
                for (int i = 0; i < LR_ROWS; ++i) {
                    o[i].x = __builtin_fma(m[i][q], v.x, o[i].x);
                    o[i].y = __builtin_fma(m[i][q], v.y, o[i].y);
                }
            }
        }
#pragma unroll
        for (int i = 0; i < LR_ROWS; ++i) bstore2_aux<COH ? 17 : 0>(rC[i], k * 8, 0, make_double2(cf[i] * o[i].x, cf[i] * o[i].y));
    }
}
template <bool COH, class RowOf, bool ATM = false>
__device__ __forceinline__ void lowrank_tile(const GemmArgs& g, RowOf row_of, int tile, int BM, int bn0, bool check_active,
                                             const AtmSets& at = AtmSets()) {
    const int nct = (g.D + GEMM_BN - 1) / GEMM_BN, ct = bn0 / GEMM_BN;
    const int lane = threadIdx.x & 63, wave = __builtin_amdgcn_readfirstlane(threadIdx.x) >> 6;
    const int per = (BM - ct + nct - 1) / nct;
    const bool chk = check_active && g.active && g.check_tiles;
    for (int j = LR_ROWS * wave; j < per; j += 4 * LR_ROWS) {
        int rows[LR_ROWS];
        int n = 0;
#pragma unroll
        for (int i = 0; i < LR_ROWS; ++i) {
            int r = j + i < per ? __builtin_amdgcn_readfirstlane(row_of(tile * BM + ct + nct * (j + i))) : -1;
            if (chk && r >= 0 && !g.active[r / g.L]) r = -1;
            rows[i] = r;
            n += r >= 0 ? 1 : 0;
        }
        if (n == 0) continue;
        if (rows[0] < 0)
#pragma unroll
            for (int i = 1; i < LR_ROWS; ++i)
                if (rows[i] >= 0) { rows[0] = rows[i]; rows[i] = -1; break; }
        lowrank_rows<COH, ATM>(g, rows, lane, at);
    }
}

constexpr int TAIL_RT_SLAB = 1;
constexpr int TAIL_RT = 2;

}
}
```

### sos-radiative-transfer_amd/csrc/kernels.hip

```cpp
#include <cstdlib>

#include "kernels.hpp"

#include "../../include/sosrt.h"

namespace sosrt {


typedef double f64x4 __attribute__((ext_vector_type(4)));

#define SOSRT_PI 3.14159265358979323846

__device__ __forceinline__ double wave_fmax(double v) {
#pragma unroll
    for (int o = 32; o > 0; o >>= 1) v = fmax(v, __shfl_xor(v, o, 64));
    return v;
}
__device__ __forceinline__ double wave_sum(double v) {
#pragma unroll
    for (int o = 32; o > 0; o >>= 1) v += __shfl_xor(v, o, 64);
    return v;
}

__device__ double block_pymax(double x, bool valid, double* s_red, int first_tid = 0) {
// ... 927 lines not shown
        } else {
            const double dl = tau[min(t + 1, g.L - 1)] - tau[t];
            if (m > g.N) E = exp(-dl * (1.0 / mu));
        }
        E_all[(size_t)b * LD + i] = E;
    }
}

void launch_attenuation(hipStream_t s, const Grid& g, int B, const double* tau, double* Etab, const int* erep) {
    const int slices = erep ? 64 : 8;
    hipLaunchKernelGGL(k_attenuation, dim3(slices, B), dim3(256), 0, s, g, B, tau, Etab, erep);
}

__global__ void k_tau_rep(int L, const double* __restrict__ tau_all, const unsigned long long* __restrict__ hash,
                          int* __restrict__ erep, const int* __restrict__ need_small, int* __restrict__ host_flag, int tag) {
    const int b = blockIdx.x, lane = threadIdx.x;
    if (host_flag && b == 0 && lane == 0) {
        __hip_atomic_store(host_flag, need_small[0], __ATOMIC_RELAXED, __HIP_MEMORY_SCOPE_SYSTEM);
        __hip_atomic_store(host_flag + 1, tag, __ATOMIC_RELEASE, __HIP_MEMORY_SCOPE_SYSTEM);
    }
    const unsigned long long hb = hash[b];
    const double* tb = tau_all + (size_t)b * L;
    int rep = b;
    for (int c0 = 0; c0 < b && rep == b; c0 += 64) {
        const int c = c0 + lane;
        unsigned long long cand = __ballot(c < b && hash[c] == hb);
        while (cand && rep == b) {
            const int cc = c0 + __ffsll((long long)cand) - 1;
            cand &= cand - 1;
            const double* tc = tau_all + (size_t)cc * L;
            bool same = true;
            for (int i = lane; i < L; i += 64) same = same && (tb[i] == tc[i]);
            if (__ballot(!same) == 0) rep = cc;
        }
    }
    if (lane == 0) erep[b] = rep;
}
void launch_tau_groups(hipStream_t s, const Grid& g, int B, const double* tau, unsigned long long* hash, int* erep,
                       const int* need_small, int* host_flag, int tag) {
    hipLaunchKernelGGL(k_tau_rep, dim3(B), dim3(64), 0, s, g.L, tau, hash, erep, need_small, host_flag, tag);
}

template <int MAXT>
static void launch_transport_t(hipStream_t s, dim3 grid, dim3 block, size_t shm, const TransportArgs& a, int mode) {
    if (mode == 1) {
        launch_transport_fast(s, grid, block, a);
    } else if (mode == 3) {
        launch_transport_ring(s, grid, a, g_ring_slots);
    } else if (mode == 4) {
        launch_transport_scan(s, grid, a);
    } else if (mode == 2) {
        if (a.accumulate) {
            if (a.saved) hipLaunchKernelGGL((k_transport<MAXT, true, true, true, true>), grid, block, shm, s, a);
            else hipLaunchKernelGGL((k_transport<MAXT, true, false, true, true>), grid, block, shm, s, a);
        } else {
            hipLaunchKernelGGL((k_transport<MAXT, false, false, true, true>), grid, block, shm, s, a);
        }
    } else if (a.accumulate) {
        if (a.Etab) {
            if (a.saved) hipLaunchKernelGGL((k_transport<MAXT, true, true, true>), grid, block, shm, s, a);
            else hipLaunchKernelGGL((k_transport<MAXT, true, false, true>), grid, block, shm, s, a);
        } else {
            if (a.saved) hipLaunchKernelGGL((k_transport<MAXT, true, true, false>), grid, block, shm, s, a);
            else hipLaunchKernelGGL((k_transport<MAXT, true, false, false>), grid, block, shm, s, a);
        }
    } else {
        if (a.Etab) hipLaunchKernelGGL((k_transport<MAXT, false, false, true>), grid, block, shm, s, a);
        else hipLaunchKernelGGL((k_transport<MAXT, false, false, false>), grid, block, shm, s, a);
    }
}

unsigned long long* g_transport_stamps = nullptr;
int g_ring_slots = 3, g_ring_debug = 0;

bool transport_fast_ok(const Plan& plan) {
    for (int bkt = 0; bkt < 4; ++bkt)
        if (plan.fix[bkt].idx > 0 && (plan.fix[bkt].s0 >> 6) != ((plan.N - 1) >> 6)) return false;
    return true;
}

void launch_transport(hipStream_t s, const Grid& g, int B, const double* tau, const double* Jn, double* In, double* I,
                      double* saved, size_t saved_col_stride, const ColDesc* desc, Conv cv, int order,
                      int accumulate, const double* Etab, int mode, const int* erep, int live, const int* live_list,
                      int ring_slots, int scan_split, double* scan_scratch, int* scan_sync, int nzcap) {
    const int nt = round64(g.N);
    const size_t shm = (size_t)(g.L + 2 * TC * (nt + 2) + 2 * nt + nt / 64 + 2) * sizeof(double);
    TransportArgs a{g, tau, Jn, In, I, accumulate ? saved : nullptr, saved_col_stride, desc, cv, order, accumulate, Etab, Etab ? erep : nullptr, g_transport_stamps};
    a.slots = ring_slots;
    a.nzcap = nzcap > kRingZones ? nzcap : kRingZones;
    if (mode == 4 && scan_split && scan_scratch && scan_sync) { a.scan_split = 1; a.scan_scratch = scan_scratch; a.scan_sync = scan_sync; }
    if ((mode == 3 || mode == 4) && accumulate && live > 0 && live < B && live_list) {
        a.live = live;
        a.live_list = live_list;
        B = live;
    }
    if (nt <= 128) launch_transport_t<128>(s, dim3(B), dim3(nt), shm, a, mode);
    else if (nt <= 256) launch_transport_t<256>(s, dim3(B), dim3(nt), shm, a, mode);
    else if (nt <= 512) launch_transport_t<512>(s, dim3(B), dim3(nt), shm, a, mode);
    else launch_transport_t<1024>(s, dim3(B), dim3(nt), shm, a, mode);
}

__global__ void k_finalize(int B, Conv cv, int max_orders, int* __restrict__ n_out, int* __restrict__ status_out) {
    const int b = blockIdx.x * blockDim.x + threadIdx.x;
    if (b >= B) return;
    int st = cv.status[b];
    if (cv.active[b]) { st = SOSRT_COL_MAXORDERS; cv.status[b] = st; }
    if (n_out) n_out[b] = cv.norders[b];
    if (status_out) status_out[b] = st;
}
void launch_finalize(hipStream_t s, int B, Conv cv, int max_orders, int* n_out, int* status_out) {
    hipLaunchKernelGGL(k_finalize, dim3((B + 127) / 128), dim3(128), 0, s, B, cv, max_orders, n_out, status_out);
}

__global__ void k_fluxes(Grid g, int B, const double* __restrict__ tau_all, const double* __restrict__ I_all,
                         const ColDesc* __restrict__ desc, int beam_norm, double* __restrict__ fdn,
                         double* __restrict__ fup) {
    const int row = blockIdx.x * (blockDim.x >> 6) + (threadIdx.x >> 6);
    if (row >= B * g.L) return;
    const int lane = threadIdx.x & 63, b = row / g.L, t = row % g.L;
    const double* I = I_all + (size_t)row * g.D;
    double sd = 0, su = 0;
    for (int k = lane; k < g.N; k += 64) {
        sd += g.wflux_dn[k] * I[k];
        su += g.wflux_up[k] * I[g.N + k];
    }
    sd = wave_sum(sd);
    su = wave_sum(su);
    if (lane == 0) {
        const ColDesc& d = desc[b];
        const double* tau = tau_all + (size_t)b * g.L;
        const double F0 = SOSRT_PI / d.mu0;
        const double fb = beam_norm ? F0 : F0 / (4 * SOSRT_PI);
        fdn[row] = sd - fb * exp(-tau[t] / d.mu0);
        fup[row] = su + fb * d.rho * exp(-(2 * tau[g.L - 1] - tau[t]) / d.mu0);
    }
}
void launch_fluxes(hipStream_t s, const Grid& g, int B, const double* tau, const double* I, const ColDesc* desc,
                   int beam_norm, double* fdn, double* fup) {
    const int rows = B * g.L;
    hipLaunchKernelGGL(k_fluxes, dim3((rows + 3) / 4), dim3(256), 0, s, g, B, tau, I, desc, beam_norm, fdn, fup);
}

__global__ void k_limit_rows(Grid g, int R, int table, const double* __restrict__ rows, double* __restrict__ out) {
    const FixTab& ft = g.fix[table];
    const int e = blockIdx.x * blockDim.x + threadIdx.x;
    if (e >= R * ft.idx) return;
    const int r = e / ft.idx, i = e % ft.idx;
    double acc = 0;
    for (int q = 0; q < ft.ns; ++q) acc += ft.C[i * ft.ns + q] * rows[(size_t)r * g.N + ft.s0 + q];
    out[e] = acc;
}
void launch_limit_rows(hipStream_t s, const Grid& g, int R, int table, const double* rows, double* out) {
    const int n = R * kFixMaxIdx;
    hipLaunchKernelGGL(k_limit_rows, dim3((n + 127) / 128), dim3(128), 0, s, g, R, table, rows, out);
}

__global__ void k_asymptotic(int R, int stride, const int* __restrict__ len, const double* __restrict__ J,
                             const double* __restrict__ tau, const double* __restrict__ tau_t,
                             const double* __restrict__ mu, double* __restrict__ out) {
    const int r = blockIdx.x * blockDim.x + threadIdx.x;
    if (r >= R) return;
    const int n = len[r];
    if (n <= 0) { out[r] = 0.0; return; }
    const double* Jr = J + (size_t)r * stride;
    const double* tr = tau + (size_t)r * stride;
    const double m = mu[r], tt = tau_t[r];
    const double Jl = Jr[n - 1];
    if (fabs(m) < kMuVerySmall) {
        double slope = 0;
        if (n > 1) slope = (Jl - Jr[n - 2]) / (tr[n - 1] - tr[n - 2]);
        out[r] = -Jl + m * slope;
        return;
// ... 73 lines not shown
```

### sos-radiative-transfer_amd/csrc/kernels.hpp

```cpp
#pragma once
#include <hip/hip_runtime.h>

#include "plan.hpp"

namespace sosrt {

constexpr int kMaxZones = 8;
constexpr int kRingZones = 3;

struct alignas(16) ColDesc {
    int nz;
    int r0[kMaxZones];
    int r1[kMaxZones];
    int mix[kMaxZones];
    int nfix[kMaxZones];
    int fixtab[kMaxZones];
    int surface;
    int geom;
    double mu0, rho, T, tau_bottom;
    double wa;
    double wr[kMaxZones];
    double fa[kMaxZones];
    double fr[kMaxZones];
    double ca[kMaxZones];
// ... 5 lines not shown
    double C[kFixMaxIdx * kFixMaxSrc];
};

struct ColScalars {
    const int* nz;
    const int* zr0;
    const int* zmix;
    const double* zwr;
    const double* zdtr;
    const int* idx_up;
    const int* idx_down;
    const double* mu0;
    const double* rho;
    const double* alb_atm;
    const double* alb_aer;
    const double* dtau_atm;
    const double* dtau_aer;
    const double* T;
};

struct Grid {
    int L, N, D;
    int Dp;
    int Wld;
    const double* mu;
    const double* Wa;
    const double* Wr;
    const FixTab* fix;
    const int* small_lanes;
    int nsmall;
    const double* wflux_dn;
    const double* wflux_up;
};

struct Conv {
    int* active;
    int* norders;
    int* status;
    int* nactive;
    double* ratio;
    int* redo;
    const int* target;
    double tol;
};

__device__ __forceinline__ bool conv_go(const Conv& cv, int b, int order, double r) {
    return cv.target ? order < cv.target[b] : r >= cv.tol;
}

constexpr int GEMM_BM = 64, GEMM_BN = 128, GEMM_KC = 16;
#ifndef SOSRT_GEMM_RT
#define SOSRT_GEMM_RT 4
#endif
#ifndef SOSRT_GEMM_WPS
#define SOSRT_GEMM_WPS 3
#endif
constexpr int GEMM_RT = SOSRT_GEMM_RT;
constexpr int GEMM_WPS = SOSRT_GEMM_WPS;

constexpr int TC = 8;

struct TransportArgs {
    Grid g;
    const double* tau;
    const double* Jn;
    double* In;
    double* I;
    double* saved;
    size_t saved_col_stride;
    const ColDesc* desc;
    Conv cv;
    int order;
    int accumulate;
    const double* Etab;
    const int* erep;
    unsigned long long* stamps;
    int live = 0;
    const int* live_list = nullptr;
    int slots = 0;
    int nzcap = kRingZones;
    int scan_split = 0;
    double* scan_scratch = nullptr;
    int* scan_sync = nullptr;
};
void launch_transport_fast(hipStream_t s, dim3 grid, dim3 block, const TransportArgs& a);
bool transport_ring_ok(const Grid& g);
bool transport_ring_fits(const Grid& g, int nzcap);
void launch_transport_ring(hipStream_t s, dim3 grid, const TransportArgs& a, int slots);
bool transport_scan_ok(const Grid& g);
bool transport_scan_split_ok(const Grid& g);
bool transport_scan_fits(const Grid& g, int nzcap, bool split);
int transport_scan_parts(const Grid& g);
size_t transport_scan_scratch_doubles();
void launch_transport_scan(hipStream_t s, dim3 grid, const TransportArgs& a);
constexpr int kOrderLoopMaxCols = 256;
constexpr int kOlArrive = 0, kOlState = 32, kOlLeft = 64, kOlAbort = 96, kOlOrders = 100, kOlCols = 128;
constexpr int kOlColStride = 64, kOlOrdDone = 0, kOlColStop = 1, kOlJnDone = 32;
constexpr int kOlReady = 1, kOlNotResident = 2, kOlAborted = 3;
inline size_t order_loop_sync_ints(int cols) { return (size_t)kOlCols + (size_t)cols * kOlColStride; }
extern int g_ring_slots, g_ring_debug;
extern unsigned long long* g_transport_stamps;

struct SolveSetup {
    int* zero_next = nullptr;
    int n_zero = 0;
    int* redo = nullptr;
    unsigned long long* hash = nullptr;
    int* scan_sync = nullptr;
};
void launch_prepare(hipStream_t s, const Grid& g, int B, int geom, int surface, ColScalars sc, const double* tau,
                    ColDesc* desc, double* rowcoef_a, double* rowcoef_r, int* need_small = nullptr, SolveSetup su = SolveSetup());
void launch_first_order_readme(hipStream_t s, const Grid& g, const double* w, int B, const double* tau, const double* P0a,
                               const double* P0r, const ColDesc* desc, double* I1_out, double* I_out, double* saved,
                               size_t saved_col_stride, Conv cv, int do_conv);
void launch_first_order(hipStream_t s, const Grid& g, int B, const double* tau, const double* P0a, const double* P0r,
                        const ColDesc* desc, double* I1_out, double* I_out, double* saved, size_t saved_col_stride,
                        Conv cv, int do_conv, int p0r_zones = 0 );
struct GemmArgs {
    const double* A;
    const double* Wa;
    const double* Wr;
    const double* ca;
    const double* cr;
    const int* rows_main;
    int n_main;
    const int* rows_slab;
    int n_slab;
    int D, Dp, Wld, L;
    double* C;
    const int* active;
    int B = 0;
    int col0 = 0;
    const int* idx_up = nullptr;
    const int* idx_down = nullptr;
    int max_main = 0, max_slab = 0;
    const double* Wmix = nullptr;
    const int* mix_group = nullptr;
    int pad_lds = 0;
    int* live_list = nullptr;
    int live_cap = 0;
    const int* slab_tile_group = nullptr;
    const int* nactive = nullptr;
    const int* need_small = nullptr;
    int* host_pub = nullptr;
    int tag = 0;
    int sym = 0;
    int Ks = 0;
    int check_tiles = 1;
    int lr_rank = -1;
    const double* lrU = nullptr;
    const double* lrV = nullptr;
};
struct AtmSets {
    const int* col_atm = nullptr;
    const int* lr_ranks = nullptr;
};
constexpr int kLowRankMax = 4;

__device__ inline void publish_live_now(const GemmArgs& g) {
    const int live = __hip_atomic_load(g.nactive, __ATOMIC_RELAXED, __HIP_MEMORY_SCOPE_AGENT);
    int* slot = g.host_pub + 4 * (g.tag & 1);
    __hip_atomic_store(slot, live, __ATOMIC_RELAXED, __HIP_MEMORY_SCOPE_SYSTEM);
    __hip_atomic_store(slot + 2, g.need_small ? g.need_small[0] : 1, __ATOMIC_RELAXED, __HIP_MEMORY_SCOPE_SYSTEM);
    __hip_atomic_store(slot + 1, g.tag, __ATOMIC_RELEASE, __HIP_MEMORY_SCOPE_SYSTEM);
}
__device__ inline void publish_live(const GemmArgs& g) {
    if (g.host_pub && blockIdx.x == 0 && blockIdx.y == 0 && threadIdx.x == 0) publish_live_now(g);
}
struct PerDeviceOnce {
    bool seen[64] = {};
    bool first() {
        int d = 0;
        if (hipGetDevice(&d) != hipSuccess || d < 0 || d >= 64) return true;
        if (seen[d]) return false;
        seen[d] = true;
        return true;
    }
};
void launch_gemm(hipStream_t s, const GemmArgs& a, const AtmSets* at = nullptr);
struct OrderLoopArgs {
    TransportArgs t;
    GemmArgs gm;
    const double* in0;
    double* gbufP;
    double* gbufQ;
    double* bufP;
    double* bufQ;
    int order0;
    int kmax;
    int B, col0;
    int fixcap;
    int* sync;
    int* host_done;
    int tag;
    unsigned long long* log = nullptr;
    int astage = 0;
};
bool order_loop_ok(const Grid& g, bool split);
int order_loop_parts(const Grid& g, bool split);
hipError_t launch_order_loop(hipStream_t s, int grid, bool split, const OrderLoopArgs& p);
void launch_gemm_f32(hipStream_t s, const GemmArgs& a, const float* Wa32, const float* Wmix32);
void launch_to_float(hipStream_t s, size_t n, const double* src, float* dst);
void launch_wmix(hipStream_t s, size_t n, int ngroups, const double* Wa, const double* Wr, const double* ca, const double* cr,
                 double* Wmix, const int* gset = nullptr ,
                 const int* gatm = nullptr );
void launch_fold_sets(hipStream_t s, int S, int D, int Wld, size_t per, const double* w, const double* P, double* W);
void launch_fold_asymmetry(hipStream_t s, int S, int nblk, int D, int Wld, size_t per, const double* W, double* out);
void launch_symfold(hipStream_t s, int nmat, int N, int D, int Dp, int Wld, const double* W, double* SA);
void launch_gemm_tail(hipStream_t s, const GemmArgs& a, int cols, bool small_tiles, bool regs = false, const AtmSets* at = nullptr);
void launch_smallmu(hipStream_t s, const Grid& g, int B, const double* tau, const double* Jn, double* In,
                    const ColDesc* desc, const int* active);
void launch_transport(hipStream_t s, const Grid& g, int B, const double* tau, const double* Jn, double* In, double* I,
                      double* saved, size_t saved_col_stride, const ColDesc* desc, Conv cv, int order, int accumulate,
                      const double* Etab, int mode, const int* erep = nullptr, int live = 0, const int* live_list = nullptr,
                      int ring_slots = 0, int scan_split = 0, double* scan_scratch = nullptr, int* scan_sync = nullptr,
                      int nzcap = kRingZones);
bool transport_fast_ok(const Plan& plan);
void launch_attenuation(hipStream_t s, const Grid& g, int B, const double* tau, double* Etab, const int* erep);
void launch_tau_groups(hipStream_t s, const Grid& g, int B, const double* tau, unsigned long long* hash, int* erep,
                       const int* need_small = nullptr, int* host_flag = nullptr, int tag = 0);
void launch_fluxes(hipStream_t s, const Grid& g, int B, const double* tau, const double* I, const ColDesc* desc,
                   int beam_norm, double* fdn, double* fup);
struct EpilogueOut {
    double* flux_down;
    double* flux_up;
    double* diffusivity;
    double* heating_rate;
    double* net_toa;
};
void launch_epilogue(hipStream_t s, const Grid& g, const double* w, int B, const double* tau, const double* I,
                     const ColDesc* desc, int beam_norm, const double* z_profile, const EpilogueOut& out);
void launch_phase_p0(hipStream_t s, const Grid& g, const double* w, int B, int kind, double gpar, const double* tab_mu,
                     const double* tab_p, int ntab, const double* cosphi, const double* wphi, int nphi,
                     const double* mu0, double* P0);
void launch_phase_matrix(hipStream_t s, const Grid& g, const double* w, int kind, double gpar, const double* tab_mu,
                         const double* tab_p, int ntab, const double* cosphi, const double* wphi, int nphi, double* P);
constexpr int kMaxModes = 64;
void launch_phase_modes(hipStream_t s, const Grid& g, const double* w, int kind, double gpar, const double* tab_mu,
                        const double* tab_p, int ntab, const double* cosphi, const double* tab, int nphi, int m_first,
                        int m_count, double* P_out);
void launch_phase_p0_modes(hipStream_t s, const Grid& g, const double* w, int B, int kind, double gpar, const double* tab_mu,
                           const double* tab_p, int ntab, const double* cosphi, const double* tab, int nphi, int m_first,
                           int m_count, const double* mu0, double* P0_out);
void launch_azimuth_accumulate(hipStream_t s, const Grid& g, int B, int m, const double* Im, int nlev, const int* levels,
                               int nphi_out, const double* phi, double* out);
void launch_azimuth_synthesize(hipStream_t s, const Grid& g, int B, int M, const double* I0, const double* Im, int nlev,
                               const int* levels, int nphi_out, const double* phi, double* out);
void launch_negate_odd_modes(hipStream_t s, size_t n, int m_first, int m_count, double* P);
constexpr int kMieQ = 6;
constexpr int kMieChunk = 4;
inline int mie_chunks(int R) { return (R + kMieChunk - 1) / kMieChunk; }
void launch_mie_coefficients(hipStream_t s, int nlanes, int R, int n_cap, const double* x, const int* nmax, const int* nstart,
                             const double* m_re, const double* m_im, const double* radii, const double* r_m, const double* sig,
                             double* ab, double* qw);
void launch_mie_angles(hipStream_t s, int S, int R, int ntab, int n_cap, const double* mu, const double* ab, const int* nmax,
                       const double* tn, const double* qw, double* part);
void launch_mie_integrate(hipStream_t s, int S, int R, int ntab, const double* part, const double* radii, const double* qw,
                          double* p, double* bulk);
void launch_limit_rows(hipStream_t s, const Grid& g, int R, int table, const double* rows, double* out);
void launch_asymptotic(hipStream_t s, int R, int stride, const int* len, const double* J, const double* tau,
                       const double* tau_t, const double* mu, double* out);
void launch_finalize(hipStream_t s, int B, Conv cv, int max_orders, int* n_out = nullptr, int* status_out = nullptr);
void launch_bench(hipStream_t s, int which, double* a, double* b, size_t n, int iters);

}
```

### sos-radiative-transfer_amd/csrc/transport_ring.hip

```cpp
#include <type_traits>

#include "../../include/sosrt.h"
#include "kernels.hpp"
#include "transport_util.hpp"

namespace sosrt {

namespace {

#ifndef SOSRT_RING_STORE_AUX
#define SOSRT_RING_STORE_AUX 0
#endif
__device__ __forceinline__ void rstore(__amdgpu_buffer_rsrc_t r, int voff, int soff, double x) { bstore_aux<SOSRT_RING_STORE_AUX>(r, voff, soff, x); }

typedef __attribute__((address_space(3))) void* lds_ptr_t;

constexpr size_t kRingLdsBytes = 152 * 1024;

template <int CNT>
__device__ __forceinline__ void wait_vm() {
    asm volatile("s_waitcnt vmcnt(%0)" ::"n"(CNT) : "memory");
}
__device__ __forceinline__ void wg_barrier() {
    asm volatile("s_waitcnt lgkmcnt(0)\n\ts_barrier" ::: "memory");
}

template <bool ACC, bool SAVED, int PIECES, bool MZ>
__global__ __launch_bounds__(512) void k_transport_ring(TransportArgs a, int NS, int dbg_arg, int fixcap) {
    constexpr int NWL = 2;
#ifdef SOSRT_RING_DEBUG
    const int dbg = dbg_arg;
#else
    constexpr int dbg = 0;
    (void)dbg_arg;
#endif
    int b = blockIdx.x;
    if (ACC && a.live > 0) {
        b = a.live_list[blockIdx.x];
        if (b < 0) return;
    } else if (ACC && !a.cv.active[b]) {
        return;
    }
    const Grid& g = a.g;
    const int tid = threadIdx.x, lane = tid & 63;
    const int wid = __builtin_amdgcn_readfirstlane(tid) >> 6;
    const int L = g.L, N = g.N, D = g.D;
    const int nwc = (N + 63) >> 6;
    const bool loader = wid >= nwc;
    const int lid = wid - nwc;
    const bool w0 = wid == 0 && !(dbg & 8);
    const bool wl = wid == ((N - 1) >> 6) && !(dbg & 4);
    auto stamp = [&](int i) {
        if (a.stamps && (tid == 0 || tid == 64)) a.stamps[((size_t)b * 2 + (tid >> 6)) * 8 + i] = clock64();
    };
    stamp(0);
    constexpr int NARR = ACC ? 3 : 2;
    constexpr int RS = 128 * PIECES;
    constexpr int SLOT = NARR * TC * RS;
    constexpr int IPC = NARR * TC * PIECES;
    extern __shared__ double sm[];
    double* ring = sm;
    double* s_sfc = ring + (size_t)NS * SLOT;
    double* s_fixc = s_sfc;
    double* s_red = s_sfc + max(RS, (MZ ? a.nzcap : kRingZones) * fixcap * kFixMaxSrc);
    double* s_hd = s_red + (blockDim.x >> 6) + 2;
    double* s_S = s_hd + L + 1;
    double* s_x = s_S + (size_t)g.nsmall * L;
    double* s_prmu = s_x + TC * 16;
    int* s_nf = reinterpret_cast<int*>(s_prmu + 16);
    const int xb_dn = max(((N - 1) & 63) - 15, 0);
    __shared__ int s_flag[3];
    const ColDesc* __restrict__ dg = a.desc + b;
    const int nz = dg->nz;
    const ZoneRows<MZ> zr(dg);
    const int nfix0 = dg->nfix[0], nfix1 = dg->nfix[1], nfix2 = dg->nfix[2];
    const int surface = dg->surface;
    const double rho = dg->rho;
    const int fbytes = L * D * 8, RB = D * 8;
    const int lbytes = (dbg & 1) ? 0 : fbytes, sbytes = (dbg & 2) ? 0 : fbytes;
    const __amdgpu_buffer_rsrc_t rJ = make_rsrc(a.Jn + (size_t)b * L * D, lbytes);
    const __amdgpu_buffer_rsrc_t rE = make_rsrc(a.Etab + (size_t)(a.erep ? a.erep[b] : b) * L * D, lbytes);
    const __amdgpu_buffer_rsrc_t rIn = make_rsrc(a.In + (size_t)b * L * D, sbytes);
    const __amdgpu_buffer_rsrc_t rIl = make_rsrc(ACC ? a.I + (size_t)b * L * D : a.In, ACC ? lbytes : 0);
    const __amdgpu_buffer_rsrc_t rI = make_rsrc(ACC ? a.I + (size_t)b * L * D : a.In, ACC ? sbytes : 0);
    const __amdgpu_buffer_rsrc_t rS = make_rsrc(SAVED ? a.saved + (size_t)b * a.saved_col_stride : a.In, SAVED ? sbytes : 0);
    const int NCH = (L + TC - 1) / TC, NQ = 2 * NCH, R = NS - 1;
    const bool valid = tid < N;
    const int tidc = valid ? tid : N - 1;
    unsigned long long sp_dn = NCH > 64 ? ~0ull : 1ull << (NCH - 1), sp_up = sp_dn;
    if (NCH <= 64) {
        sp_dn |= zr.boundary_chunks(L, TC, false);
        sp_up |= zr.boundary_chunks(L, TC, true);
    }
    auto plain_run = [&](unsigned long long mask, int j) {
        const unsigned long long rest = NCH > 64 ? 1ull : mask >> j;
        return rest ? __builtin_ctzll(rest) : 0;
    };
    double rdn_v = 0, rdn_i = 1, rup_v = 0, rup_i = 1;
    double sfc_own = 0;
    int slot_rd = 0;

    int slot_ld = 0;
    auto issue = [&](int q) {
        const bool up = q >= NCH;
        const int j = up ? q - NCH : q;
        double* dst = ring + (size_t)slot_ld * SLOT;
        slot_ld = slot_ld + 1 == NS ? 0 : slot_ld + 1;
        const int half = up ? N * 8 : 0;
        const int vo = lane * 16;
#pragma unroll
        for (int i = 0; i < TC / NWL; ++i) {
            const int u = i * NWL + lid;
            const int row = up ? max(L - 1 - j * TC - u, 0) : min(j * TC + u, L - 1);
#pragma unroll
            for (int p = 0; p < PIECES; ++p) {
                const int so = row * RB + half + p * 1024;
                __builtin_amdgcn_raw_ptr_buffer_load_lds(rJ, (lds_ptr_t)(dst + (0 * TC + u) * RS + p * 128), 16, vo, so, 0, 0);
                __builtin_amdgcn_raw_ptr_buffer_load_lds(rE, (lds_ptr_t)(dst + (1 * TC + u) * RS + p * 128), 16, vo, so, 0, 0);
                if (ACC) __builtin_amdgcn_raw_ptr_buffer_load_lds(rIl, (lds_ptr_t)(dst + (2 * TC + u) * RS + p * 128), 16, vo, so, 0, 0);
            }
        }
    };
    auto loader_phase = [&](auto keep_t, int qa, int qb) {
        constexpr int KEEP = decltype(keep_t)::value;
        for (int q = qa; q < qb; ++q) {
            if (q + R < NQ) {
                issue(q + R);
                wait_vm<KEEP>();
            } else {
                wait_vm<0>();
            }
            wg_barrier();
        }
    };
    const int ncomp = nwc * 64;
    if (loader) {
        for (int q = 0; q < min(R, NQ); ++q) issue(q);
    } else {
        for (int zz = 0; zz < (MZ ? nz : kRingZones); ++zz) {
            const FixTab& src = g.fix[dg->fixtab[zz]];
            for (int i = tid; i < fixcap * kFixMaxSrc; i += ncomp) s_fixc[zz * fixcap * kFixMaxSrc + i] = src.C[i];
        }
        if (tid < 3) s_flag[tid] = 0;
        for (int i = tid; i < (L + 31) / 32; i += ncomp) s_nf[i] = 0;
        const double* __restrict__ tau = a.tau + (size_t)b * L;
        for (int t = tid; t <= L; t += ncomp) s_hd[t] = (t == 0 || t == L) ? 0.0 : (tau[t] - tau[t - 1]) * 0.5;
        if (tid < 16) s_prmu[tid] = (tid > 0 && tid < N) ? 1.0 / g.mu[N + tid] : 0.0;
        const double* __restrict__ In0 = a.In + (size_t)b * L * D;
        for (int i = tid; i < g.nsmall * L; i += ncomp) {
            const int k = i / L, t = i - k * L;
            s_S[i] = In0[(size_t)t * D + g.small_lanes[k]];
        }
    }
    __syncthreads();

    const int seam_barriers = surface == SOSRT_SURFACE_NONE ? 0 : (surface == SOSRT_SURFACE_SPECULAR ? 1 : 3);
    double Bv = 0;
    if (loader) {
        constexpr int PER = IPC / NWL;
        auto run = [&](auto keep_t) {
            loader_phase(keep_t, 0, NCH);
            for (int i = 0; i < seam_barriers; ++i) wg_barrier();
            loader_phase(keep_t, NCH, NQ);
            wait_vm<0>();
        };
        if (R <= 1) run(std::integral_constant<int, 0>{});
        else if (R == 2) run(std::integral_constant<int, (PER < 60 ? PER : 60)>{});
        else if (R == 3) run(std::integral_constant<int, (2 * PER < 60 ? 2 * PER : 60)>{});
        else run(std::integral_constant<int, (3 * PER < 60 ? 3 * PER : 60)>{});
    } else {
    stamp(1);
    const double mu_up = (valid && tid > 0) ? g.mu[N + tidc] : 1.0;
    const int uT = lane >> 3, pT = lane & 7;
    const double muT = (pT + 1 < N) ? g.mu[N + pT + 1] : 1.0;
    const double* xrow = s_x + uT * 16;
    {
        const int m = tidc;
        const int vo = m * 8;
        const double mu = g.mu[m];
        const bool tr = valid && m <= N - 2;
        const bool small = tr && fabs(mu) < kMuThreshold;
        const bool stdl = tr && !small;
        const double nrmu = stdl ? -1.0 / mu : 0.0;
        const bool has_small = wl && g.nsmall > 0;
        double Dv = 0, Jprev = 0;
        double c[kFixMaxSrc] = {0, 0, 0, 0, 0};
        double cT[kFixMaxSrc] = {0, 0, 0, 0, 0};
        int sl[kFixMaxSrc] = {0, 0, 0, 0, 0};
        int nfx = 0;
        bool fixlane = false;
        auto load_fix = [&](int zz) {
            const double* ftC = s_fixc + zz * fixcap * kFixMaxSrc;
            nfx = zz == 0 ? nfix0 : (zz == 1 ? nfix1 : ((!MZ || zz == 2) ? nfix2 : zr.nfix(zz)));
            const int ns = nfx < 2 ? 2 : (nfx < kFixMaxSrc ? nfx : kFixMaxSrc);
            fixlane = valid && nfx > 0 && m >= N - nfx;
            const int i = fixlane ? N - 1 - m : 0;
            const int s0 = nfx < 2 ? N - nfx - 2 : N - nfx - ns;
#pragma unroll
            for (int q = 0; q < kFixMaxSrc; ++q) {
                c[q] = (fixlane && q < ns) ? ftC[i * ns + min(q, ns - 1)] : 0.0;
                cT[q] = (pT < nfx && q < ns) ? ftC[pT * ns + min(q, ns - 1)] : 0.0;
                sl[q] = (s0 + min(q, ns - 1)) & 63;
            }
        };
        if (wl) load_fix(0);
        const int sbase = small ? (m - g.small_lanes[0]) * L : 0;
        int t0 = 0, q = 0;
        auto process = [&](auto special_t, auto mode_t, const double* slot, double (&Jc)[TC], double (&Ic)[TC], double (&Ec)[TC]) __attribute__((always_inline)) {
            constexpr bool SP = decltype(special_t)::value;
            constexpr int MODE = decltype(mode_t)::value;
            double cc[TC], v[TC], Sc[TC];
#pragma unroll
            for (int u = 0; u < TC; ++u) Sc[u] = 0;
            if ((SP || MODE == 2) && has_small) {
#pragma unroll
                for (int u = 0; u < TC; ++u) {
                    const double sv = s_S[sbase + min(t0 + u, L - 1)];
                    Sc[u] = small ? sv : 0.0;
                }
            }
#pragma unroll
            for (int u = 0; u < TC; ++u) {
                const int t = SP ? min(t0 + u, L - 1) : t0 + u;
                const double hk = s_hd[t];
                const double Jp = u == 0 ? Jprev : Jc[u - 1];
                cc[u] = rec_src(rec_hr(hk, nrmu), Jp, Ec[u], Jc[u]);
            }
            if (!SP) {
                {
                    double d = 0, p = 1, dl[TC], pl[TC];
#pragma unroll
                    for (int u = 0; u < TC; ++u) {
                        d = rec_step(d, Ec[u], cc[u]);
                        p = u == 0 ? Ec[0] : rec_hr(p, Ec[u]);
                        dl[u] = d; pl[u] = p;
                    }
#pragma unroll
                    for (int u = 0; u < TC; ++u) v[u] = rec_step(Dv, pl[u], dl[u]);
                    Dv = v[TC - 1];
                }
                if (MODE == 2 && has_small) {
#pragma unroll
                    for (int u = 0; u < TC; ++u) v[u] = rec_add(v[u], Sc[u]);
                }
                const bool tfix = MODE == 1 || (MODE == 2 && wl && nfx > 0 && nfx <= 8 && sl[0] >= xb_dn);
                if (tfix) {
#pragma unroll
                    for (int u = 0; u < TC; ++u)
                        if (lane >= xb_dn && lane < xb_dn + 16) s_x[u * 16 + lane - xb_dn] = v[u];
                    double acc = 0;
#pragma unroll
                    for (int k = 0; k < kFixMaxSrc; ++k) acc = fix_acc(cT[k], xrow[max(sl[k] - xb_dn, 0)], acc);
                    const int mT = N - 1 - pT;
                    const double IcT = ACC ? slot[(2 * TC + uT) * RS + max(mT, 0)] : 0.0;
                    if (pT < nfx) {
                        const int voT = (t0 + uT) * RB + mT * 8;
                        rstore(rIn, voT, 0, acc);
                        if (ACC) rstore(rI, voT, 0, IcT + acc);
                        if (SAVED) rstore(rS, voT, 0, acc);
                    }
                } else if (MODE == 2 && wl && nfx > 0) {
#pragma unroll
                    for (int u = 0; u < TC; ++u) {
                        double acc = 0;
#pragma unroll
                        for (int k = 0; k < kFixMaxSrc; ++k) acc = fix_acc(c[k], readlane_f64(v[u], sl[k]), acc);
                        v[u] = fixlane ? acc : v[u];
                    }
                }
                if (valid && !(tfix && fixlane)) {
#pragma unroll
                    for (int u = 0; u < TC; ++u) {
                        const int so = (t0 + u) * RB;
                        rstore(rIn, vo, so, v[u]);
                        if (ACC) rstore(rI, vo, so, Ic[u] + v[u]);
                        if (SAVED) rstore(rS, vo, so, v[u]);
                    }
                }
            } else {
#pragma unroll
                for (int u = 0; u < TC; ++u) {
                    const int t = t0 + u;
                    if (wl) { const int zs = zr.starts(t); if (zs) load_fix(zs); }
                    const double Dn = rec_step(Dv, Ec[u], cc[u]);
                    double x = has_small ? rec_add(Dn, Sc[u]) : Dn;
                    if (wl && nfx > 0) {
                        double acc = 0;
#pragma unroll
                        for (int k = 0; k < kFixMaxSrc; ++k) acc = fix_acc(c[k], readlane_f64(x, sl[k]), acc);
                        x = fixlane ? acc : x;
                    }
                    v[u] = x;
                    const bool zone_end = zr.ends(t);
                    Dv = t < L ? (zone_end ? (stdl ? x : 0.0) : Dn) : Dv;
                    if (valid && t < L) {
                        const int so = t * RB;
                        rstore(rIn, vo, so, x);
                        if (ACC) rstore(rI, vo, so, Ic[u] + x);
                        if (SAVED) rstore(rS, vo, so, x);
                    }
                }
            }
            if (SP && t0 + TC >= L) {
#pragma unroll
                for (int u = 0; u < TC; ++u)
                    if (t0 + u == L - 1) { sfc_own = v[u]; rdn_v = v[u]; rdn_i = Ic[u] + v[u]; }
            }
            Jprev = Jc[TC - 1];
            t0 += TC;
        };
        auto chunk = [&](auto special_t, auto mode_t) __attribute__((always_inline)) {
            const double* sp = ring + (size_t)slot_rd * SLOT + tid;
            slot_rd = slot_rd + 1 == NS ? 0 : slot_rd + 1;
            double Jc[TC], Ic[TC], Ec[TC];
#pragma unroll
            for (int u = 0; u < TC; ++u) {
                Jc[u] = sp[(0 * TC + u) * RS];
                Ec[u] = sp[(1 * TC + u) * RS];
                Ic[u] = ACC ? sp[(2 * TC + u) * RS] : 0.0;
            }
            process(special_t, mode_t, sp - tid, Jc, Ic, Ec);
            wg_barrier();
        };
        using M0 = std::integral_constant<int, 0>;
        using M1 = std::integral_constant<int, 1>;
        using M2 = std::integral_constant<int, 2>;
        while (q < NCH) {
            const int qe = q + plain_run(sp_dn, q);
            const int mode = (!wl || (nfx == 0 && !has_small)) ? 0 : ((!has_small && nfx <= 8 && sl[0] >= xb_dn) ? 1 : 2);
            if (mode == 0) for (; q < qe; ++q) chunk(std::false_type{}, M0{});
            else if (mode == 1) for (; q < qe; ++q) chunk(std::false_type{}, M1{});
            else for (; q < qe; ++q) chunk(std::false_type{}, M2{});
            if (q < NCH) { chunk(std::true_type{}, M2{}); ++q; }
        }
    }

    stamp(2);
    if (surface != SOSRT_SURFACE_NONE) {
        if (valid) s_sfc[tid] = sfc_own;
        wg_barrier();
    }
    if (surface == SOSRT_SURFACE_SPECULAR) {
        Bv = valid ? rho * s_sfc[N - 1 - tid] : 0.0;
    } else if (surface == SOSRT_SURFACE_LAMBERTIAN || surface == SOSRT_SURFACE_LAMBERTIAN_README) {
        double term = 0;
        if (tid <= N - 3) {
            const int k0 = N - 2 - tid, k1 = k0 - 1;
            const double x0 = g.mu[k0], x1 = g.mu[k1];
            term = (x1 - x0) * (s_sfc[k1] * x1 + s_sfc[k0] * x0) / 2;
        }
        double ws = wave_sum_(term);
        wg_barrier();
        if (lane == 0) s_red[tid >> 6] = ws;
        wg_barrier();
        double S = 0;
        for (int i = 0; i < nwc; ++i) S += s_red[i];
        Bv = (surface == SOSRT_SURFACE_LAMBERTIAN_README ? 2 : -2) * rho * S;
    }

    stamp(3);
    {
        const int mj = N + tidc;
        const int vo = mj * 8;
        const bool tr = valid && tid > 0;
        const double mu = mu_up;
        const double prmu = tr ? 1.0 / mu : 0.0;
        const int last_cand = min(N - 3, 61);
        bool notfound = false;
        double U = Bv, Jnext = 0;
        auto blend = [&](double x, int t) {
            const double x1 = lane_up1(x), x2 = lane_up1(x1);
            const bool stop = lane >= 1 && lane <= last_cand && !(fabs((x - x1) - (x1 - x2)) > 0.0001);
            const unsigned long long mk = __ballot(stop);
            const int kf = mk ? __ffsll((long long)mk) : 1;
            if (mk == 0) {
                notfound = true;
                if (N - 3 > 61 && lane == 0) {
                    if (zr.starts(t)) s_flag[0] = 1;
                    else { flag_row(s_nf, t); s_flag[2] = 1; }
                }
            }
            const double r0 = readlane_f64(x, 0), rk = readlane_f64(x, kf);
            const double w = blend_weight(mu, readlane_f64(prmu, kf));
            const double bl = blend_val(w, r0, rk);
            return (tr && tid < kf) ? bl : x;
        };
        int t0 = L - 1, q = NCH;
        auto process = [&](auto special_t, auto mode_t, const double* slot, double (&Jc)[TC], double (&Ic)[TC], double (&Ec)[TC]) __attribute__((always_inline)) {
            constexpr bool SP = decltype(special_t)::value;
            constexpr int MODE = decltype(mode_t)::value;
            double cc[TC], v[TC];
#pragma unroll
            for (int u = 0; u < TC; ++u) {
                const int t = SP ? max(t0 - u, 0) : t0 - u;
                const double hk = s_hd[t + 1];
                const double Jx = u == 0 ? Jnext : Jc[u - 1];
                const double src = rec_src(rec_hr(hk, prmu), Jx, Ec[u], Jc[u]);
                cc[u] = (SP && zr.ends(t)) ? 0.0 : src;
            }
            if (!SP) {
                {
                    double d = 0, p = 1, dl[TC], pl[TC];
#pragma unroll
// ... 10 lines not shown
                if (MODE == 1) {
#pragma unroll
                    for (int u = 0; u < TC; ++u) {
                        v[u] = tid == 0 ? Jc[u] : v[u];
                        if (lane < 16) s_x[u * 16 + lane] = v[u];
                    }
                    const int k = pT + 1;
                    const double xa = xrow[k], xb = xrow[k + 1], xc = xrow[k + 2];
                    const bool stop = (k <= last_cand) & !(fabs((xa - xb) - (xb - xc)) > 0.0001);
                    const unsigned long long mk = __ballot(stop);
                    const unsigned bits = (unsigned)(mk >> (8 * uT)) & 0xffu;
                    tblend = __ballot(bits != 0) == ~0ull;
                    if (tblend) {
                        const int kf = __ffs((int)bits) + 1;
                        const double r0 = xrow[0], rk = xrow[kf];
                        const double w = blend_weight(muT, s_prmu[kf]);
                        const double bl = blend_val(w, r0, rk);
                        const double val = k < kf ? bl : xa;
                        const double IcT = ACC ? slot[(2 * TC + uT) * RS + k] : 0.0;
                        if (k < N) {
                            const int voT = (t0 - uT) * RB + (N + k) * 8;
                            rstore(rIn, voT, 0, val);
                            if (ACC) rstore(rI, voT, 0, IcT + val);
                            if (SAVED) rstore(rS, voT, 0, val);
                        }
                    } else {
#pragma unroll
                        for (int u = 0; u < TC; ++u) {
                            const double xb_ = blend(v[u], t0 - u);
                            if (valid) {
                                const int so = (t0 - u) * RB;
                                rstore(rIn, vo, so, xb_);
                                if (ACC) rstore(rI, vo, so, Ic[u] + xb_);
                                if (SAVED) rstore(rS, vo, so, xb_);
                            }
                        }
                    }
                }
                if (valid && (MODE == 0 || (tblend && !(tid >= 1 && tid <= 8)))) {
#pragma unroll
                    for (int u = 0; u < TC; ++u) {
                        const int so = (t0 - u) * RB;
                        rstore(rIn, vo, so, v[u]);
                        if (ACC) rstore(rI, vo, so, Ic[u] + v[u]);
                        if (SAVED) rstore(rS, vo, so, v[u]);
                    }
                }
            } else {
#pragma unroll
                for (int u = 0; u < TC; ++u) {
                    const int t = t0 - u;
                    const double Un = rec_step(U, Ec[u], cc[u]);
                    double x = Un;
                    if (w0 && t >= 0) x = blend(tid == 0 ? Jc[u] : Un, t);
                    v[u] = x;
                    const bool zone_start = zr.starts(t) != 0;
                    U = t >= 0 ? ((zone_start && tr) ? x : Un) : U;
                    if (valid && t >= 0) {
                        const int so = t * RB;
                        rstore(rIn, vo, so, x);
                        if (ACC) rstore(rI, vo, so, Ic[u] + x);
                        if (SAVED) rstore(rS, vo, so, x);
                    }
                }
            }
            if (SP && t0 - TC < 0) {
#pragma unroll
                for (int u = 0; u < TC; ++u)
                    if (t0 - u == 0) { rup_v = v[u]; rup_i = Ic[u] + v[u]; }
            }
            Jnext = Jc[TC - 1];
            t0 -= TC;
        };
        auto chunk = [&](auto special_t, auto mode_t) __attribute__((always_inline)) {
            const double* sp = ring + (size_t)slot_rd * SLOT + tid;
            slot_rd = slot_rd + 1 == NS ? 0 : slot_rd + 1;
            double Jc[TC], Ic[TC], Ec[TC];
#pragma unroll
            for (int u = 0; u < TC; ++u) {
                Jc[u] = sp[(0 * TC + u) * RS];
                Ec[u] = sp[(1 * TC + u) * RS];
                Ic[u] = ACC ? sp[(2 * TC + u) * RS] : 0.0;
            }
            process(special_t, mode_t, sp - tid, Jc, Ic, Ec);
            wg_barrier();
        };
        using M0 = std::integral_constant<int, 0>;
        using M1 = std::integral_constant<int, 1>;
        while (q < NQ) {
            const int qe = q + plain_run(sp_up, q - NCH);
            if (!w0) for (; q < qe; ++q) chunk(std::false_type{}, M0{});
            else for (; q < qe; ++q) chunk(std::false_type{}, M1{});
            if (q < NQ) { chunk(std::true_type{}, M1{}); ++q; }
        }
        if (w0 && notfound && lane == 0 && N - 3 <= 61) s_flag[1] = 1;
    }
    }
    stamp(4);
    __syncthreads();
    stamp(5);
    if (s_flag[1]) {
        if (tid == 0) {
            a.cv.status[b] = SOSRT_COL_INDEXERROR;
            if (ACC) { a.cv.active[b] = 0; a.cv.norders[b] = a.order; atomicSub(a.cv.nactive, 1); }
        }
        return;
    }
    if (!s_flag[0] && s_flag[2]) {
        if (finish_flagged_rows<ACC, SAVED>(s_nf, L, N, RB, g.mu, rIn, rI, rS, ring, rup_v, rup_i)) {
            if (tid == 0) {
                a.cv.status[b] = SOSRT_COL_INDEXERROR;
                if (ACC) { a.cv.active[b] = 0; a.cv.norders[b] = a.order; atomicSub(a.cv.nactive, 1); }
            }
            return;
        }
    }
    if (s_flag[0]) {
        const bool missing = redo_upward_sweep<ACC, SAVED, MZ>(L, N, RB, zr, s_hd, g.mu, rJ, rE, rIn, rI, rS, Bv, ring,
                                                            rup_v, rup_i);
        if (missing) {
            if (tid == 0) {
                a.cv.status[b] = SOSRT_COL_INDEXERROR;
                if (ACC) { a.cv.active[b] = 0; a.cv.norders[b] = a.order; atomicSub(a.cv.nactive, 1); }
            }
            return;
        }
    }
    if (ACC) {
        const double ra = block_pymax_(rup_v / rup_i, valid, s_red, 0);
        const double rb = block_pymax_(rdn_v / rdn_i, valid, s_red, 0);
        const double r = (rb > ra) ? rb : ra;
        if (tid == 0) {
            a.cv.ratio[b] = r;
            a.cv.norders[b] = a.order;
            if (!conv_go(a.cv, b, a.order, r)) {
                a.cv.active[b] = 0;
                atomicSub(a.cv.nactive, 1);
            }
        }
    } else if (tid == 0 && a.cv.status) {
        a.cv.status[b] = SOSRT_COL_OK;
    }
}

inline int ring_fixcap(const Grid& g) { return (int)(0.06 * g.N) + 1; }
inline size_t ring_extra_doubles(const Grid& g, int nt, int nzcap = kRingZones) {
    const int rs = g.N <= 128 ? 128 : 256, fc = nzcap * ring_fixcap(g) * kFixMaxSrc;
    return (size_t)(rs > fc ? rs : fc) + nt / 64 + 2 + g.L + 1 + (size_t)g.nsmall * g.L + TC * 16 + 16 + (g.L + 63) / 64;
}

template <int PIECES>
void launch_p(hipStream_t s, dim3 grid, dim3 block, const TransportArgs& a, int NS) {
    const int nt = (int)block.x;
    const int narr = a.accumulate ? 3 : 2;
    const size_t shm = ((size_t)NS * narr * TC * 128 * PIECES + ring_extra_doubles(a.g, nt, a.nzcap)) * sizeof(double);
#define SOSRT_RING_LAUNCH_Z(ACC_, SAVED_, MZ_)                                                                 \
    do {                                                                                                       \
        auto kern = k_transport_ring<ACC_, SAVED_, PIECES, MZ_>;                                               \
        static PerDeviceOnce big_lds;                                                                                 \
        if (big_lds.first()) {                                                                                        \
            hipFuncSetAttribute(reinterpret_cast<const void*>(kern), hipFuncAttributeMaxDynamicSharedMemorySize, \
                                (int)kRingLdsBytes);                                                                   \
        }                                                                                                      \
        hipLaunchKernelGGL(kern, grid, block, shm, s, a, NS, g_ring_debug, ring_fixcap(a.g));                           \
    } while (0)
#define SOSRT_RING_LAUNCH(ACC_, SAVED_)                                                                        \
    do {                                                                                                       \
        if (a.nzcap > kRingZones) SOSRT_RING_LAUNCH_Z(ACC_, SAVED_, true);                                     \
        else SOSRT_RING_LAUNCH_Z(ACC_, SAVED_, false);                                                         \
    } while (0)
    if (a.accumulate) {
        if (a.saved) SOSRT_RING_LAUNCH(true, true);
        else SOSRT_RING_LAUNCH(true, false);
    } else {
        SOSRT_RING_LAUNCH(false, false);
    }
#undef SOSRT_RING_LAUNCH
#undef SOSRT_RING_LAUNCH_Z
}

}

bool transport_ring_ok(const Grid& g) {
    if (g.N % 2 || g.N < 4 || g.N > 256) return false;
    const int nwc = (g.N + 63) / 64, pieces = g.N <= 128 ? 1 : 2;
    const size_t slot_bytes = (size_t)3 * TC * 128 * pieces * sizeof(double);
    if (flagged_rows_work_doubles(g.L, g.N) * sizeof(double) > 2 * slot_bytes * 2 / 3) return false;
    return 2 * slot_bytes + ring_extra_doubles(g, (nwc + 4) * 64) * sizeof(double) <= kRingLdsBytes;
}

bool transport_ring_fits(const Grid& g, int nzcap) {
    if (!transport_ring_ok(g)) return false;
    const int nwc = (g.N + 63) / 64, pieces = g.N <= 128 ? 1 : 2;
    const size_t slot_bytes = (size_t)3 * TC * 128 * pieces * sizeof(double);
    return 2 * slot_bytes + ring_extra_doubles(g, (nwc + 4) * 64, nzcap < kRingZones ? kRingZones : nzcap) * sizeof(double) <= kRingLdsBytes;
}

void launch_transport_ring(hipStream_t s, dim3 grid, const TransportArgs& a, int slots) {
    if (a.slots > 0) slots = a.slots;
    const int N = a.g.N;
    const int nwc = (N + 63) / 64;
    const int pieces = N <= 128 ? 1 : 2;
    const int narr = a.accumulate ? 3 : 2;
    const dim3 block((nwc + 2) * 64);
    const size_t slot_bytes = (size_t)narr * TC * 128 * pieces * sizeof(double);
    const size_t extra = ring_extra_doubles(a.g, (int)block.x, a.nzcap) * sizeof(double);
    int NS = slots < 2 ? 2 : slots;
    while (NS > 2 && NS * slot_bytes + extra > kRingLdsBytes) --NS;
    if (pieces == 1) launch_p<1>(s, grid, block, a, NS);
    else launch_p<2>(s, grid, block, a, NS);
}

}
```

### sos-radiative-transfer_amd/csrc/transport_util.hpp

```cpp
#pragma once
#include <hip/hip_runtime.h>

#include "kernels.hpp"

namespace sosrt {
namespace {

__device__ __forceinline__ double readlane_f64(double v, int srclane) {
    int lo = __double2loint(v), hi = __double2hiint(v);
    lo = __builtin_amdgcn_readlane(lo, srclane);
    hi = __builtin_amdgcn_readlane(hi, srclane);
    return __hiloint2double(hi, lo);
}

typedef unsigned int u32x2 __attribute__((ext_vector_type(2)));

__device__ __forceinline__ __amdgpu_buffer_rsrc_t make_rsrc(const void* p, int bytes) {
    return __builtin_amdgcn_make_buffer_rsrc(const_cast<void*>(p), 0, bytes, 0x00020000);
}
__device__ __forceinline__ double bload(__amdgpu_buffer_rsrc_t r, int voff, int soff) {
    const u32x2 v = __builtin_amdgcn_raw_buffer_load_b64(r, voff, soff, 0);
    return __hiloint2double((int)v.y, (int)v.x);
}
__device__ __forceinline__ double bload_glc(__amdgpu_buffer_rsrc_t r, int voff, int soff) {
    const u32x2 v = __builtin_amdgcn_raw_buffer_load_b64(r, voff, soff, 1);
    return __hiloint2double((int)v.y, (int)v.x);
}
template <int AUX>
__device__ __forceinline__ double bload_aux(__amdgpu_buffer_rsrc_t r, int voff, int soff) {
    const u32x2 v = __builtin_amdgcn_raw_buffer_load_b64(r, voff, soff, AUX);
    return __hiloint2double((int)v.y, (int)v.x);
}
__device__ __forceinline__ void bstore(__amdgpu_buffer_rsrc_t r, int voff, int soff, double x) {
    u32x2 v;
    v.x = (unsigned)__double2loint(x);
    v.y = (unsigned)__double2hiint(x);
    __builtin_amdgcn_raw_buffer_store_b64(v, r, voff, soff, 0);
}
template <int AUX>
__device__ __forceinline__ void bstore_aux(__amdgpu_buffer_rsrc_t r, int voff, int soff, double x) {
    u32x2 v;
    v.x = (unsigned)__double2loint(x);
    v.y = (unsigned)__double2hiint(x);
    __builtin_amdgcn_raw_buffer_store_b64(v, r, voff, soff, AUX);
}

typedef unsigned int u32x4 __attribute__((ext_vector_type(4)));
__device__ __forceinline__ double2 bload2(__amdgpu_buffer_rsrc_t r, int voff, int soff) {
    const u32x4 v = __builtin_amdgcn_raw_buffer_load_b128(r, voff, soff, 0);
    return make_double2(__hiloint2double((int)v.y, (int)v.x), __hiloint2double((int)v.w, (int)v.z));
}
template <int AUX>
__device__ __forceinline__ double2 bload2_aux(__amdgpu_buffer_rsrc_t r, int voff, int soff) {
    const u32x4 v = __builtin_amdgcn_raw_buffer_load_b128(r, voff, soff, AUX);
    return make_double2(__hiloint2double((int)v.y, (int)v.x), __hiloint2double((int)v.w, (int)v.z));
}
__device__ __forceinline__ void bstore2(__amdgpu_buffer_rsrc_t r, int voff, int soff, double2 x) {
    u32x4 v;
    v.x = (unsigned)__double2loint(x.x); v.y = (unsigned)__double2hiint(x.x);
    v.z = (unsigned)__double2loint(x.y); v.w = (unsigned)__double2hiint(x.y);
    __builtin_amdgcn_raw_buffer_store_b128(v, r, voff, soff, 0);
}
template <int AUX>
__device__ __forceinline__ void bstore2_aux(__amdgpu_buffer_rsrc_t r, int voff, int soff, double2 x) {
    u32x4 v;
    v.x = (unsigned)__double2loint(x.x); v.y = (unsigned)__double2hiint(x.x);
    v.z = (unsigned)__double2loint(x.y); v.w = (unsigned)__double2hiint(x.y);
    __builtin_amdgcn_raw_buffer_store_b128(v, r, voff, soff, AUX);
}

__device__ __forceinline__ double lane_up1(double v) {
    int lo = __double2loint(v), hi = __double2hiint(v);
    lo = __builtin_amdgcn_update_dpp(lo, lo, 0x130, 0xf, 0xf, false);
    hi = __builtin_amdgcn_update_dpp(hi, hi, 0x130, 0xf, 0xf, false);
    return __hiloint2double(hi, lo);
}

__device__ __forceinline__ double wave_fmax_(double v) {
#pragma unroll
    for (int o = 32; o > 0; o >>= 1) v = fmax(v, __shfl_xor(v, o, 64));
    return v;
}
__device__ __forceinline__ double wave_sum_(double v) {
#pragma unroll
    for (int o = 32; o > 0; o >>= 1) v += __shfl_xor(v, o, 64);
    return v;
// ... 97 lines not shown
        return m;
    }
};

constexpr int kNfBatch = 8;
__host__ __device__ inline size_t flagged_rows_work_doubles(int L, int N) { return (size_t)kNfBatch * (N + 2) + (L + kNfBatch + 2 + 1) / 2 + 1; }
__device__ __forceinline__ void flag_row(int* s_nf, int t) { atomicOr(&s_nf[t >> 5], 1 << (t & 31)); }
#ifdef SOSRT_HELPERS_AS_CALLS
#define SOSRT_HELPER_INLINE __attribute__((noinline))
#else
#define SOSRT_HELPER_INLINE __forceinline__
#endif
template <bool ACC, bool SAVED, int LDX = 0, int STX = 0>
__device__ SOSRT_HELPER_INLINE bool finish_flagged_rows(const int* s_nf, int L, int N, int RB, const double* __restrict__ gmu, __amdgpu_buffer_rsrc_t rIn,
                                    __amdgpu_buffer_rsrc_t rI, __amdgpu_buffer_rsrc_t rS, double* s_work, double& rup_v, double& rup_i) {
    const int tid = threadIdx.x, NP = N + 2;
    double* s_rows = s_work;
    int* s_list = reinterpret_cast<int*>(s_work + kNfBatch * NP);
    int* s_kf = s_list + L;
    int* s_cnt = s_kf + kNfBatch;
    if (tid == 0) {
        int c = 0;
        for (int t = L - 1; t >= 0; --t)
            if ((s_nf[t >> 5] >> (t & 31)) & 1) s_list[c++] = t;
        *s_cnt = c;
    }
    __syncthreads();
    const int cnt = *s_cnt;
    const bool act = tid < N, tr = act && tid > 0;
    const int j = act ? tid : 0;
    const double mu = tr ? gmu[N + j] : 1.0;
    const int vo = (N + j) * 8;
    bool missing = false;
    for (int c0 = 0; c0 < cnt; c0 += kNfBatch) {
        const int nb = min(kNfBatch, cnt - c0);
        double xo[kNfBatch], Io[kNfBatch];
#pragma unroll
        for (int i = 0; i < kNfBatch; ++i) {
            const int t = s_list[c0 + min(i, nb - 1)];
            xo[i] = bload_aux<LDX ? LDX : 1>(rIn, vo, t * RB);
            Io[i] = ACC ? bload_aux<LDX ? LDX : 1>(rI, vo, t * RB) : 0.0;
        }
#pragma unroll
        for (int i = 0; i < kNfBatch; ++i)
            if (act) s_rows[i * NP + j] = xo[i];
        if (tid < kNfBatch) s_kf[tid] = 1 << 30;
        __syncthreads();
#pragma unroll
        for (int i = 0; i < kNfBatch; ++i) {
            const double* r = s_rows + i * NP;
            if (i < nb && act && j >= 1 && j <= N - 3 && !(fabs((r[j] - r[j + 1]) - (r[j + 1] - r[j + 2])) > 0.0001)) atomicMin(&s_kf[i], j);
        }
        __syncthreads();
#pragma unroll
        for (int i = 0; i < kNfBatch; ++i) {
            if (i >= nb) continue;
            const double* r = s_rows + i * NP;
            const int ks = s_kf[i];
            missing |= ks == (1 << 30);
            const int kf = ks == (1 << 30) ? 1 : ks + 1;
            const int t = s_list[c0 + i];
            if (tr && tid < kf) {
                const double x = blend_val(blend_weight(mu, 1.0 / gmu[N + kf]), r[0], r[kf]);
                bstore_aux<STX>(rIn, vo, t * RB, x);
                double It = 0;
                if (ACC) {
                    It = Io[i] + (x - xo[i]);
                    bstore_aux<STX>(rI, vo, t * RB, It);
                }
                if (SAVED) bstore_aux<STX>(rS, vo, t * RB, x);
                if (t == 0) { rup_v = x; rup_i = It; }
            }
        }
        __syncthreads();
    }
    return missing;
}

constexpr int kRedoRows = 8;
template <bool ACC, bool SAVED, bool MZ, int LDX = 0, int STX = 0>
__device__ SOSRT_HELPER_INLINE bool redo_upward_sweep(int L, int N, int RB, const ZoneRows<MZ>& zr, const double* s_hd,
                                  const double* __restrict__ gmu, __amdgpu_buffer_rsrc_t rJ, __amdgpu_buffer_rsrc_t rE,
                                  __amdgpu_buffer_rsrc_t rIn, __amdgpu_buffer_rsrc_t rI, __amdgpu_buffer_rsrc_t rS, double U0,
                                  double* s_work, double& rup_v, double& rup_i) {
    const int tid = threadIdx.x;
    double* s_row = s_work;
    int* s_kf = reinterpret_cast<int*>(s_work + 2 * (N + 2));
    const bool act = tid < N, tr = act && tid > 0;
    const int j = act ? tid : 0;
    const double mu = tr ? gmu[N + j] : 1.0;
    const double prmu = tr ? 1.0 / mu : 0.0;
    const int vo = (N + j) * 8;
    double U = U0, Jnext = 0;
    bool missing = false;
    if (tid < 2) s_kf[tid] = 1 << 30;
    __syncthreads();
    int par = 0;
    for (int t0 = L - 1; t0 >= 0; t0 -= kRedoRows) {
        double Jc[kRedoRows], Ec[kRedoRows], xo[kRedoRows], Io[kRedoRows];
#pragma unroll
        for (int u = 0; u < kRedoRows; ++u) {
            const int t = max(t0 - u, 0);
            Jc[u] = bload_aux<LDX>(rJ, vo, t * RB);
            Ec[u] = bload(rE, vo, t * RB);
            xo[u] = bload_aux<LDX ? LDX : 1>(rIn, vo, t * RB);
            Io[u] = ACC ? bload_aux<LDX ? LDX : 1>(rI, vo, t * RB) : 0.0;
        }
#pragma unroll
        for (int u = 0; u < kRedoRows; ++u) {
            const int t = t0 - u;
            if (t < 0) break;
            double* row = s_row + par * (N + 2);
            const double src = rec_src(rec_hr(s_hd[t + 1], prmu), Jnext, Ec[u], Jc[u]);
            const double Un = rec_step(U, Ec[u], zr.ends(t) ? 0.0 : src);
            if (act) row[j] = tid == 0 ? Jc[u] : Un;
            __syncthreads();
            if (act && j >= 1 && j <= N - 3 && !(fabs((row[j] - row[j + 1]) - (row[j + 1] - row[j + 2])) > 0.0001)) atomicMin(&s_kf[par], j);
            if (tid == 0) s_kf[par ^ 1] = 1 << 30;
            __syncthreads();
            const int ks = s_kf[par];
            missing |= ks == (1 << 30);
            const int kf = ks == (1 << 30) ? 1 : ks + 1;
            double x = act ? row[j] : 0.0;
            if (tr && tid < kf) x = blend_val(blend_weight(mu, 1.0 / gmu[N + kf]), row[0], row[kf]);
            const bool zone_start = zr.starts(t) != 0;
            U = (zone_start && tr) ? x : Un;
            Jnext = Jc[u];
            if (act) {
                bstore_aux<STX>(rIn, vo, t * RB, x);
                double It = 0;
                if (ACC) {
                    It = Io[u] + (x - xo[u]);
                    bstore_aux<STX>(rI, vo, t * RB, It);
                }
                if (SAVED) bstore_aux<STX>(rS, vo, t * RB, x);
                if (t == 0) { rup_v = x; rup_i = It; }
            }
            par ^= 1;
        }
    }
    __syncthreads();
    return missing;
}

__device__ __forceinline__ double block_pymax_(double x, bool valid, double* s_red, int first_tid) {
    const int tid = threadIdx.x, nw = blockDim.x >> 6;
    double v = wave_fmax_(valid ? x : __builtin_nan(""));
    __syncthreads();
    if ((tid & 63) == 0) s_red[tid >> 6] = v;
    if (tid == first_tid) s_red[nw] = x;
    __syncthreads();
    double r = s_red[0];
    for (int i = 1; i < nw; ++i) r = fmax(r, s_red[i]);
    const double first = s_red[nw];
    return (first != first) ? first : r;
}

}
}
```

### sos-radiative-transfer_amd/sosrt/_lib.py

```python
import ctypes
import os
from ctypes import POINTER, c_char_p, c_double, c_int, c_longlong, c_void_p

_HERE = os.path.dirname(os.path.abspath(__file__))
LIB_PATH = os.environ.get("SOSRT_LIB") or os.path.join(os.path.dirname(_HERE), "libsosrt.so")

SOSRT_OK, E_INVALID, E_HIP, E_STATE, E_NOMEM = 0, -1, -2, -3, -4
COL_OK, COL_INDEXERROR, COL_MAXORDERS, COL_INTERNAL = 0, 1, 2, 3
GEOM_THREE_ZONE, GEOM_SINGLE_SLAB = 0, 1
SURFACE_NONE, SURFACE_SPECULAR, SURFACE_LAMBERTIAN, SURFACE_LAMBERTIAN_README = 0, 1, 2, 3
K_GEMM, K_TRANSPORT, K_FIRST, K_SMALLMU, K_ORDER_LOOP = 0, 1, 2, 3, 4
PLAN_GEMM_DENSE, PLAN_GEMM_LIVE64, PLAN_GEMM_LIVE32, PLAN_GEMM_LIVE32_DEEP, PLAN_GEMM_LIVE16_REGS = 0, 1, 2, 3, 4
PLAN_TRANSPORT_GENERAL, PLAN_TRANSPORT_FAST, PLAN_TRANSPORT_RING, PLAN_TRANSPORT_SCAN = 0, 1, 3, 4
CONTRACT_F64, CONTRACT_F32, CONTRACT_F64_FULL, CONTRACT_F64_DENSE = 0, 1, 2, 3
FIRST_ORDER_CODED, FIRST_ORDER_README = 0, 1
PHASE_ISO, PHASE_RAYLEIGH, PHASE_HG, PHASE_TABLE = 0, 1, 2, 3
MAX_MODES = 64
MAX_PHASE_SETS = 64

_dp = POINTER(c_double)
_ip = POINTER(c_int)

SIGNATURES = {
    "sosrt_last_error": (c_char_p, []),
    "sosrt_version": (c_int, []),
    "sosrt_create": (c_int, [c_int, c_int, c_int, c_int, c_int, POINTER(c_void_p)]),
    "sosrt_destroy": (c_int, [c_void_p]),
    "sosrt_set_stream": (c_int, [c_void_p, c_void_p]),
    "sosrt_use_own_stream": (c_int, [c_void_p]),
    "sosrt_synchronize": (c_int, [c_void_p]),
    "sosrt_set_saved_orders": (c_int, [c_void_p, c_int]),
    "sosrt_set_order_budget": (c_int, [c_void_p, c_int]),
    "sosrt_set_contraction": (c_int, [c_void_p, c_int]),
    "sosrt_phase_asymmetry": (c_int, [c_void_p, POINTER(c_double), _ip]),
    "sosrt_phase_rank": (c_int, [c_void_p, _ip, POINTER(c_double), _ip]),
    "sosrt_set_order_loop": (c_int, [c_void_p, c_int]),
    "sosrt_order_loop_stats": (c_int, [c_void_p, _ip, _ip, POINTER(c_longlong)]),
    "sosrt_plan_launch": (c_int, [c_void_p, c_int, c_int, c_int, c_int, c_int, _ip]),
    "sosrt_set_first_order": (c_int, [c_void_p, c_int]),
    "sosrt_set_grid": (c_int, [c_void_p, c_void_p]),
    "sosrt_set_phase": (c_int, [c_void_p, c_void_p, c_void_p]),
    "sosrt_set_phase_sets": (c_int, [c_void_p, c_void_p, c_int, c_void_p]),
    "sosrt_set_phase_sets_dev": (c_int, [c_void_p, c_void_p, c_int, c_void_p]),
    "sosrt_phase_matrix_dev": (c_int, [c_void_p, c_int, c_double, c_void_p]),
    "sosrt_set_aerosol_sets": (c_int, [c_void_p, c_int, c_int, c_void_p]),
    "sosrt_phase_sets_info": (c_int, [c_void_p, _ip]),
    "sosrt_set_atm_phase_sets": (c_int, [c_void_p, c_int, c_void_p]),
    "sosrt_set_atmosphere_sets": (c_int, [c_void_p, c_int, c_void_p]),
    "sosrt_atm_sets_info": (c_int, [c_void_p, _ip]),
    "sosrt_set_columns": (c_int, [c_void_p, c_int, c_int, c_int] + [c_void_p] * 9),
    "sosrt_set_columns_zones": (c_int, [c_void_p, c_int, c_int, c_int] + [c_void_p] * 10),
    "sosrt_first_order": (c_int, [c_void_p, c_int, c_void_p, c_void_p, c_void_p, c_void_p]),
    "sosrt_source": (c_int, [c_void_p, c_int, c_void_p, c_void_p]),
    "sosrt_transport": (c_int, [c_void_p, c_int, c_void_p, c_void_p, c_void_p, c_void_p]),
    "sosrt_solve": (c_int, [c_void_p, c_int, c_void_p, c_void_p, c_void_p, c_double, c_void_p, c_void_p, c_void_p, c_void_p, c_void_p]),
    "sosrt_solve_dev": (c_int, [c_void_p, c_int, c_void_p, c_void_p, c_void_p, c_double, c_void_p, c_void_p, c_void_p, c_void_p, c_void_p]),
    "sosrt_last_solve_stats": (c_int, [c_void_p, _ip, POINTER(c_longlong)]),
    "sosrt_fluxes": (c_int, [c_void_p, c_int, c_void_p, c_void_p, c_int, c_void_p, c_void_p]),
    "sosrt_epilogue_dev": (c_int, [c_void_p, c_int, c_void_p, c_void_p, c_int] + [c_void_p] * 6),
    "sosrt_epilogue": (c_int, [c_void_p, c_int, c_int] + [c_void_p] * 6),
    "sosrt_phase_table": (c_int, [c_void_p, c_void_p, c_void_p, c_int]),
    "sosrt_phase_table_dev": (c_int, [c_void_p, c_void_p, c_void_p, c_int]),
    "sosrt_mie_ensembles": (c_int, [c_void_p, c_int] + [c_void_p] * 5 + [c_int, c_double, c_double, c_int, c_void_p, c_void_p]),
    "sosrt_mie_ensembles_dev": (c_int, [c_void_p, c_int] + [c_void_p] * 5 + [c_int, c_double, c_double, c_int, c_void_p, c_void_p]),
    "sosrt_mie_efficiencies": (c_int, [c_void_p, c_int, c_void_p, c_void_p, c_void_p, c_void_p]),
    "sosrt_mie_timing": (c_int, [c_void_p, _dp]),
    "sosrt_phase_p0_dev": (c_int, [c_void_p, c_int, c_int, c_double, c_void_p, c_void_p]),
    "sosrt_phase_p0": (c_int, [c_void_p, c_int, c_int, c_double, c_void_p, c_void_p]),
    "sosrt_phase_matrix": (c_int, [c_void_p, c_int, c_double, c_void_p]),
    "sosrt_phase_modes": (c_int, [c_void_p, c_int, c_double, c_int, c_int, c_int, c_void_p]),
    "sosrt_phase_modes_dev": (c_int, [c_void_p, c_int, c_double, c_int, c_int, c_int, c_int, c_void_p]),
    "sosrt_phase_p0_modes_dev": (c_int, [c_void_p, c_int, c_int, c_double, c_int, c_int, c_int, c_void_p, c_void_p]),
    "sosrt_phase_p0_modes": (c_int, [c_void_p, c_int, c_int, c_double, c_int, c_int, c_int, c_void_p, c_void_p]),
    "sosrt_set_order_targets": (c_int, [c_void_p, c_void_p]),
    "sosrt_azimuth_accumulate_dev": (c_int, [c_void_p, c_int, c_int, c_void_p, c_int, c_void_p, c_int, c_void_p, c_void_p]),
    "sosrt_azimuth_synthesize_dev": (c_int, [c_void_p, c_int, c_int, c_void_p, c_void_p, c_int, c_void_p, c_int, c_void_p, c_void_p]),
    "sosrt_comm_unique_id": (c_int, [c_void_p]),
    "sosrt_comm_init": (c_int, [c_void_p, c_int, c_int, c_void_p]),
    "sosrt_gather": (c_int, [c_void_p, c_int, c_void_p, c_void_p, c_void_p]),
    "sosrt_comm_destroy": (c_int, [c_void_p]),
    "sosrt_limit_mu_down": (c_int, [c_void_p, c_int, c_int, c_void_p, c_void_p]),
    "sosrt_asymptotic_down": (c_int, [c_void_p, c_int, c_int, c_void_p, c_void_p, c_void_p, c_void_p, c_void_p, c_void_p]),
    "sosrt_plan_weights": (c_int, [c_void_p, c_void_p]),
    "sosrt_plan_fold": (c_int, [c_void_p, c_int, c_void_p]),
    "sosrt_plan_fix_table": (c_int, [c_void_p, c_int, _ip, _ip, c_void_p]),
    "sosrt_plan_fix_count": (c_int, [c_double, c_int]),
    "sosrt_debug_stamps": (c_int, [c_void_p, c_void_p]),
    "sosrt_microbench": (c_int, [c_void_p, c_int, _dp]),
    "sosrt_profile_enable": (c_int, [c_void_p, c_int]),
    "sosrt_profile_reset": (c_int, [c_void_p]),
    "sosrt_profile_get": (c_int, [c_void_p, c_int, _dp, POINTER(c_longlong), _dp]),
}

_lib = None


def _preload_hip_runtime():
    import importlib.util
    try:
        spec = importlib.util.find_spec("torch")
    except (ImportError, ValueError):
        spec = None
    if spec is None or not spec.submodule_search_locations:
        return
    p = os.path.join(list(spec.submodule_search_locations)[0], "lib", "libamdhip64.so")
    if os.path.exists(p):
        try:
            ctypes.CDLL(p, mode=ctypes.RTLD_GLOBAL)
        except OSError:
            pass


def lib():
    global _lib
    if _lib is None:
        if not os.path.exists(LIB_PATH):
            raise ImportError(
                "libsosrt.so not found at %s: build it with `python __graft_entry__.py build` "
                "(hipcc --offload-arch=gfx950); there is no CPU fallback" % LIB_PATH)
        _preload_hip_runtime()
# ... 23 lines not shown
```

### sos-radiative-transfer_amd/sosrt/solver.py

```python
from __future__ import annotations

import ctypes
from dataclasses import dataclass
from typing import Optional

import numpy as np

from . import _lib
from ._lib import check, lib


def _f64(a, shape=None, name="array"):
    a = np.ascontiguousarray(a, dtype=np.float64)
    if shape is not None and a.shape != tuple(shape):
        raise ValueError("%s has shape %s, expected %s" % (name, a.shape, tuple(shape)))
    return a


def _i32(a, n, name):
    a = np.ascontiguousarray(a, dtype=np.int32)
    if a.shape != (n,):
        raise ValueError("%s has shape %s, expected (%d,)" % (name, a.shape, n))
    return a


def _ptr(a):
    return None if a is None else a.ctypes.data_as(ctypes.c_void_p)


def _vec(x, B, name):
    a = np.ascontiguousarray(np.broadcast_to(np.asarray(x, dtype=np.float64), (B,)))
    return a


@dataclass
class DevicePhaseSets:
    address: int
    S: int
    keep: object = None


@dataclass
class SolveResult:
    I: np.ndarray
    n: np.ndarray
    status: np.ndarray
    I_saved: Optional[np.ndarray]


class Solver:

    def __init__(self, nb_layers: int, nb_angles: int, max_batch: int = 1, max_orders: int = 64, device: int = 0):
        self.L, self.N, self.D = int(nb_layers), int(nb_angles), 2 * int(nb_angles)
        self.max_batch, self.max_orders, self.device = int(max_batch), int(max_orders), int(device)
        self._h = ctypes.c_void_p()
        check(lib().sosrt_create(self.device, self.L, self.N, self.max_batch, self.max_orders, ctypes.byref(self._h)))
        self.B = 0
        self.order_budget = self.max_orders
        self.mu = None
        self._P = (None, None)
        self._p0_zones = 0

    def close(self):
        if getattr(self, "_h", None) is not None and self._h.value:
            lib().sosrt_destroy(self._h)
            self._h = ctypes.c_void_p()

    def __del__(self):
        try:
            self.close()
        except Exception:
            pass

    def set_stream(self, stream_handle: Optional[int]):
        if stream_handle is None:
            check(lib().sosrt_use_own_stream(self._h))
        else:
            check(lib().sosrt_set_stream(self._h, ctypes.c_void_p(stream_handle) if stream_handle else None))

    def synchronize(self):
        check(lib().sosrt_synchronize(self._h))

    def set_contraction(self, mode="f64"):
        m = {"f64": _lib.CONTRACT_F64, "f32": _lib.CONTRACT_F32, "f64_full": _lib.CONTRACT_F64_FULL,
             "f64_dense": _lib.CONTRACT_F64_DENSE}.get(mode)
        if m is None:
            raise ValueError("contraction must be 'f64', 'f64_dense', 'f64_full' or 'f32'")
        check(lib().sosrt_set_contraction(self._h, m))

    def set_order_budget(self, max_orders: int):
        check(lib().sosrt_set_order_budget(self._h, int(max_orders)))
        self.order_budget = int(max_orders)

    def set_order_loop(self, on=True):
        check(lib().sosrt_set_order_loop(self._h, int(on) if on in (0, 1, 2) else (1 if on else 0)))

    def order_loop_stats(self, column_orders=False):
        a, b, c = ctypes.c_int(), ctypes.c_int(), ctypes.c_longlong()
        check(lib().sosrt_order_loop_stats(self._h, ctypes.byref(a), ctypes.byref(b), ctypes.byref(c) if column_orders else None))
        return (a.value, b.value, c.value) if column_orders else (a.value, b.value)

    def phase_asymmetry(self):
        a, u = ctypes.c_double(), ctypes.c_int()
        check(lib().sosrt_phase_asymmetry(self._h, ctypes.byref(a), ctypes.byref(u)))
        return a.value, bool(u.value)

    def phase_rank(self):
        r, a, u = ctypes.c_int(), ctypes.c_double(), ctypes.c_int()
        check(lib().sosrt_phase_rank(self._h, ctypes.byref(r), ctypes.byref(a), ctypes.byref(u)))
        return r.value, a.value, bool(u.value)

    def set_first_order(self, mode="coded"):
        m = {"coded": _lib.FIRST_ORDER_CODED, "readme": _lib.FIRST_ORDER_README}.get(mode)
        if m is None:
            raise ValueError("first_order must be 'coded' or 'readme'")
        check(lib().sosrt_set_first_order(self._h, m))

    def set_grid(self, mu):
        mu = _f64(mu, (self.D,), "mu")
        check(lib().sosrt_set_grid(self._h, _ptr(mu)))
        self.mu = mu.copy()
        self._P = (None, None)

    def set_phase(self, P_atm, P_aer=None):
        Pa = _f64(P_atm, (self.D, self.D), "P_atm")
        Pr = None if P_aer is None else _f64(P_aer, (self.D, self.D), "P_aer")
        check(lib().sosrt_set_phase(self._h, _ptr(Pa), _ptr(Pr)))
        self._P = (Pa.copy(), None if Pr is None else Pr.copy())

    def set_phase_sets(self, P_atm, P_aer_sets):
        Pa = _f64(P_atm, (self.D, self.D), "P_atm")
        Pr = np.ascontiguousarray(P_aer_sets, dtype=np.float64)
        if Pr.ndim != 3 or Pr.shape[1:] != (self.D, self.D):
            raise ValueError("P_aer_sets has shape %s, expected (S, %d, %d)" % (Pr.shape, self.D, self.D))
        check(lib().sosrt_set_phase_sets(self._h, _ptr(Pa), int(Pr.shape[0]), _ptr(Pr)))
        self._P = (Pa.copy(), Pr.copy())

    def set_phase_sets_device(self, P_atm, d_P_aer: int, S: int):
        Pa = _f64(P_atm, (self.D, self.D), "P_atm")
        check(lib().sosrt_set_phase_sets_dev(self._h, _ptr(Pa), int(S), ctypes.c_void_p(d_P_aer) if d_P_aer else None))
        self._P = (None, None)

    def set_aerosol_sets(self, sets):
        z = np.ascontiguousarray(sets, dtype=np.int32)
        if z.ndim == 1:
            z = z.reshape(-1, 1)
        if z.ndim != 2 or z.shape[0] != self.B:
            raise ValueError("sets has shape %s, expected (%d,) or (%d, nzmax)" % (np.shape(sets), self.B, self.B))
        check(lib().sosrt_set_aerosol_sets(self._h, int(z.shape[0]), int(z.shape[1]), _ptr(z)))
        self._p0_zones = int(z.shape[1]) if z.shape[1] > 1 else 0

    def phase_sets_info(self):
        out = (ctypes.c_int * 4)()
        check(lib().sosrt_phase_sets_info(self._h, out))
        return {"sets": out[0], "groups": out[1], "single_pass": bool(out[2]), "group_cap": out[3]}

    def set_atm_phase_sets(self, P_atm_sets):
        Pa = np.ascontiguousarray(P_atm_sets, dtype=np.float64)
        if Pa.ndim != 3 or Pa.shape[1:] != (self.D, self.D):
            raise ValueError("P_atm_sets has shape %s, expected (S_atm, %d, %d)" % (Pa.shape, self.D, self.D))
        check(lib().sosrt_set_atm_phase_sets(self._h, int(Pa.shape[0]), _ptr(Pa)))
        self._P = (None, None)

    def set_atmosphere_sets(self, sets):
        z = np.ascontiguousarray(sets, dtype=np.int32)
        if z.shape != (self.B,):
            raise ValueError("sets has shape %s, expected (%d,)" % (np.shape(sets), self.B))
        check(lib().sosrt_set_atmosphere_sets(self._h, int(self.B), _ptr(z)))

    def atm_sets_info(self):
        out = (ctypes.c_int * 2)()
        check(lib().sosrt_atm_sets_info(self._h, out))
        return {"sets": out[0], "in_use": bool(out[1])}

    def same_grid(self, mu):
        return self.mu is not None and np.array_equal(self.mu, np.asarray(mu, dtype=np.float64))

    def same_phase(self, P_atm, P_aer=None):
        a, r = self._P
        if a is None or not np.array_equal(a, P_atm):
            return False
        if (r is None) != (P_aer is None):
            return False
# ... 323 lines not shown
```

Measured before the change: 124,500.

## Pass low-rank source moments to ring transport and expand Jn on the fly

```diff
diff --git a/__graft_entry__.py b/__graft_entry__.py
--- a/__graft_entry__.py
+++ b/__graft_entry__.py
@@ -7,7 +7,7 @@
 CSRC = os.path.join(PKG, "csrc")
 LIB = os.path.join(PKG, "libsosrt.so")
 SOURCES = ["api.hip", "kernels.hip", "jn_gemm.hip", "jn_gemm_f32.hip", "transport_fast.hip", "transport_ring.hip", "transport_scan.hip", "order_loop.hip", "epilogue.hip", "plan.cpp", "comm.cpp"]
-HEADERS = ["kernels.hpp", "plan.hpp", "transport_util.hpp", "transport_scan_body.hpp", "jn_gemm_tile.hpp", "comm.hpp", os.path.join(ROOT, "include", "sosrt.h")]
+HEADERS = ["kernels.hpp", "plan.hpp", "transport_util.hpp", "transport_scan_body.hpp", "jn_gemm_tile.hpp", "lowrank_expand.hpp", "comm.hpp", os.path.join(ROOT, "include", "sosrt.h")]
 
 
 OBJDIR = os.path.join(PKG, "build")
diff --git a/include/sosrt.h b/include/sosrt.h
--- a/include/sosrt.h
+++ b/include/sosrt.h
@@ -65,6 +65,7 @@
 
 int sosrt_set_order_loop(sosrt_t* h, int mode);
 int sosrt_order_loop_stats(sosrt_t* h, int* launches, int* refused, long long* column_orders );
+int sosrt_ring_moments_stats(sosrt_t* h, int* orders);
 int sosrt_phase_asymmetry(sosrt_t* h, double* asymmetry, int* uses_symmetry);
 int sosrt_phase_rank(sosrt_t* h, int* rank, double* residual, int* uses);
 
diff --git a/sos-radiative-transfer_amd/csrc/api.hip b/sos-radiative-transfer_amd/csrc/api.hip
--- a/sos-radiative-transfer_amd/csrc/api.hip
+++ b/sos-radiative-transfer_amd/csrc/api.hip
@@ -170,6 +170,9 @@
     int gemm_tail_cols = 1 << 30;
     double gemm_tail_frac = 0.6;
     int gemm_small_cols = 200;
+    double* d_mom = nullptr;
+    int ring_moments = 1;
+    int mom_orders = 0;
     int dense_live_list = 1;
     int gemm_regs_cols = -1;
     bool fast_ok = false;
@@ -431,7 +434,7 @@
 }
 
 void run_source(sosrt_handle* h, const double* In_1, double* Jn, const int* active, int tail_cols = 0, int pub_tag = 0,
-                int grp = -1, bool all_live = false, bool regs_tile = false, int dense_live_cap = 0) {
+                int grp = -1, bool all_live = false, bool regs_tile = false, int dense_live_cap = 0, double* mom = nullptr) {
     const int g0 = grp < 0 ? 0 : grp, g1 = grp < 0 ? h->ngroups : grp + 1;
     const int pg = grp < 0 ? 0 : grp;
     hipStream_t s = group_stream(h, pg);
@@ -447,6 +450,7 @@
         Jn += (size_t)h->gb[g0] * h->L * h->D;
         ga.ca = h->d_rca + (size_t)h->gb[g0] * h->L;
         ga.cr = h->d_rcr + (size_t)h->gb[g0] * h->L;
+        if (mom) mom += (size_t)h->gb[g0] * h->L * kLowRankMax;
         if (active) active += h->gb[g0];
     }
     ga.rows_slab = h->d_slabrows + h->slab_off[g0]; ga.n_slab = h->slab_off[g1] - h->slab_off[g0];
@@ -465,7 +469,7 @@
     if (two_pass_sets) {
         ga.Wr = h->d_Wrsets; ga.mix_group = h->d_mixgroup; ga.slab_tile_group = h->d_slabtilegroup + h->slab_off[g0] / 32;
     }
-    if (use_lowrank(h)) { ga.lr_rank = h->lr_rank; ga.lrU = h->d_lrU; ga.lrV = h->d_lrV; }
+    if (use_lowrank(h)) { ga.lr_rank = h->lr_rank; ga.lrU = h->d_lrU; ga.lrV = h->d_lrV; ga.mom = mom; }
     AtmSets at;
     const AtmSets* atp = nullptr;
     if (h->max_atm_used > 0) {
@@ -547,6 +551,7 @@
     int order_loop = 0;
     int ol_parts = 0;
     int ol_grid = 0;
+    int moments = 0;
 };
 LaunchPlan plan_order(const sosrt_handle* h, const SolveShape& sh, const OrderInputs& in) {
     LaunchPlan pl;
@@ -593,6 +598,8 @@
         }
         if (pl.order_loop) pl.ol_grid = in.cu_share;
     }
+    pl.moments = (h->ring_moments && pl.transport == SOSRT_PLAN_TRANSPORT_RING && use_lowrank(h) && use_sym(h) && h->max_atm_used == 0 &&
+                  !in.need_small && !pl.repair && !pl.order_loop) ? 1 : 0;
     return pl;
 }
 
@@ -654,6 +661,7 @@
     if (const char* ev = getenv("SOSRT_GEMM_TAIL_FRAC")) h->gemm_tail_frac = atof(ev);
     if (const char* ev = getenv("SOSRT_GEMM_SMALL")) h->gemm_small_cols = atoi(ev);
     if (const char* ev = getenv("SOSRT_DENSE_LIVE_LIST")) h->dense_live_list = atoi(ev) != 0;
+    if (const char* ev = getenv("SOSRT_RING_MOMENTS")) h->ring_moments = atoi(ev) != 0;
     if (const char* ev = getenv("SOSRT_GEMM_REGS")) h->gemm_regs_cols = atoi(ev);
     if (const char* ev = getenv("SOSRT_GROUPS")) h->want_groups = atoi(ev) >= 2 ? 2 : (atoi(ev) == 1 ? 1 : 0);
     if (const char* ev = getenv("SOSRT_SPLIT_MIN")) h->split_min = atoi(ev);
@@ -714,6 +722,8 @@
             if ((e = dalloc(&h->d_P0a, mb * g.D))) return e;
             if ((e = dalloc(&h->d_P0r, mb * g.D))) return e;
             if ((e = dalloc(&h->d_Jn, fe))) return e;
+            if ((e = dalloc(&h->d_mom, mb * L * kLowRankMax))) return e;
+            HIPCHK(hipMemset(h->d_mom, 0, mb * L * kLowRankMax * sizeof(double)));
             if ((e = dalloc(&h->d_InA, fe))) return e;
             if ((e = dalloc(&h->d_InB, fe))) return e;
             if ((e = dalloc(&h->d_I, fe))) return e;
@@ -771,7 +781,7 @@
                         h->d_P0r, h->d_Jn, h->d_InA, h->d_InB, h->d_I, h->d_E, h->d_active, h->d_norders, h->d_status,
                         h->d_nactive_sets, h->d_ratio, h->d_redo, h->d_erep, h->d_tauhash, h->d_Wmix, h->d_mixca, h->d_mixcr,
                         h->d_mixgroup, h->d_Wa_s, h->d_Wr_s, h->d_Wmix_s, h->d_scan_scratch, h->d_scan_sync, h->d_w, h->d_phi, h->d_z, h->d_tab, h->d_slabtilegroup, h->d_livelist, h->d_Wa32, h->d_Wmix32, h->d_nz, h->d_zr0, h->d_zmix, h->d_zwr, h->d_zdtr, h->d_olsync, h->d_ollog, h->d_modetab, h->d_lrU, h->d_lrV, h->d_Wrsets, h->d_Wrsets_s, h->d_mixset, h->d_P0rz,
-                        h->d_Wasets, h->d_lrUsets, h->d_lrVsets, h->d_lrranks, h->d_colatm, h->d_mixatm};
+                        h->d_Wasets, h->d_lrUsets, h->d_lrVsets, h->d_lrranks, h->d_colatm, h->d_mixatm, h->d_mom};
         for (void* p : ptrs)
             if (p) hipFree(p);
         if (h->h_pub) hipHostFree(h->h_pub);
@@ -874,6 +884,12 @@
             }
         }
     }
+    return 0;
+}
+
+int sosrt_ring_moments_stats(sosrt_t* h, int* orders) {
+    if (!h) return fail(SOSRT_E_INVALID, "null handle");
+    if (orders) *orders = h->mom_orders;
     return 0;
 }
 
@@ -1742,7 +1758,7 @@
         double *In_1 = nullptr, *In = nullptr;
         Conv cv;
     } gs[sosrt_handle::kMaxGroups];
-    h->ol_launches = 0; h->ol_refused = 0;
+    h->ol_launches = 0; h->ol_refused = 0; h->mom_orders = 0;
     for (bool& u : h->ol_group_used) u = false;
     bool used_order_loop = false;
     const int tagbase = ((++h->pub_seq) & 0x3fff) << 16;
@@ -1923,8 +1939,9 @@
             const int n = ++q.n;
             n_max = n > n_max ? n : n_max;
             const int tail_cols = pl.tail_cols;
+            if (pl.moments) ++h->mom_orders;
             run_source(h, q.In_1, h->d_Jn, h->d_active, tail_cols, tagbase + n - 1, k, q.known == q.nb, pl.gemm == SOSRT_PLAN_GEMM_LIVE16_REGS,
-                       tail_cols > 0 ? 0 : pl.live_cap);
+                       tail_cols > 0 ? 0 : pl.live_cap, pl.moments ? h->d_mom : nullptr);
             if (g.nsmall > 0 && h->need_small) {
                 prof_begin(h, SOSRT_K_SMALLMU, k);
                 launch_smallmu(sg, g, q.nb, tau_g, h->d_Jn + fo, q.In + fo, h->d_desc + q.b0, q.cv.active);
@@ -1935,10 +1952,11 @@
             if (pl.transport != SOSRT_PLAN_TRANSPORT_GENERAL) {
                 Grid gt = g;
                 if (pl.transport >= SOSRT_PLAN_TRANSPORT_RING && !h->need_small) gt.nsmall = 0;
+                const RingMoments rm{h->d_mom + (size_t)q.b0 * h->L * kLowRankMax, h->d_lrV, h->d_rca + (size_t)q.b0 * h->L, h->lr_rank};
                 launch_transport(sg, gt, q.nb, tau_g, h->d_Jn + fo, q.In + fo, d_I_out + fo, sv_n, saved_stride, h->d_desc + q.b0, q.cv, n, 1,
                                  h->d_E, pl.transport, erep_g, pl.live_cap, h->d_livelist + q.b0, NG > 1 ? h->coresident_slots : 0,
                                  pl.parts > 1 ? 1 : 0, h->d_scan_scratch + (size_t)q.b0 * transport_scan_scratch_doubles(),
-                                 h->d_scan_sync + 2 * q.b0, nzcap);
+                                 h->d_scan_sync + 2 * q.b0, nzcap, pl.moments ? &rm : nullptr);
                 if (pl.repair)
                     launch_transport(sg, g, q.nb, tau_g, h->d_Jn + fo, q.In + fo, d_I_out + fo, sv_n, saved_stride, h->d_desc + q.b0, q.cv, n, 1,
                                      h->d_E, 2, erep_g);
diff --git a/sos-radiative-transfer_amd/csrc/jn_gemm_tile.hpp b/sos-radiative-transfer_amd/csrc/jn_gemm_tile.hpp
--- a/sos-radiative-transfer_amd/csrc/jn_gemm_tile.hpp
+++ b/sos-radiative-transfer_amd/csrc/jn_gemm_tile.hpp
@@ -1,5 +1,6 @@
 #pragma once
 #include "kernels.hpp"
+#include "lowrank_expand.hpp"
 #include "transport_util.hpp"
 
 namespace sosrt {
@@ -366,6 +367,7 @@
 }
 
 constexpr int LR_ROWS = 4;
+static_assert(kLowRankMax == 4, "lowrank_rows stores a row's moments as two double2");
 template <bool COH, bool ATM = false>
 __device__ __forceinline__ void lowrank_rows(const GemmArgs& g, const int (&rows)[LR_ROWS], int lane, const AtmSets& at = AtmSets()) {
     const int D = g.D, R = g.lr_rank;
@@ -429,32 +431,49 @@
                 for (int i = 0; i < LR_ROWS; ++i) m[i][q] += __shfl_xor(m[i][q], s);
             }
         }
+    if (g.mom) {
+        if (lane == 0) {
+#pragma unroll
+            for (int i = 0; i < LR_ROWS; ++i)
+                if (rows[i] >= 0) {
+                    double2* mo = reinterpret_cast<double2*>(g.mom + (size_t)rows[i] * kLowRankMax);
+                    mo[0] = make_double2(m[i][0], m[i][1]);
+                    mo[1] = make_double2(m[i][2], m[i][3]);
+                }
+        }
+        return;
+    }
 #pragma unroll 2
     for (int k = 2 * lane; k < D; k += 128) {
         double2 o[LR_ROWS];
-#pragma unroll
-        for (int i = 0; i < LR_ROWS; ++i) o[i] = make_double2(0.0, 0.0);
-#pragma unroll
-        for (int q = 0; q < kLowRankMax; ++q) {
-            if constexpr (ATM) {
-#pragma unroll
-                for (int i = 0; i < LR_ROWS; ++i)
-                    if (q < Ri[i]) {
-                        const double2 v = *reinterpret_cast<const double2*>(Vi[i] + (size_t)q * D + k);
-                        o[i].x = __builtin_fma(m[i][q], v.x, o[i].x);
-                        o[i].y = __builtin_fma(m[i][q], v.y, o[i].y);
-                    }
-            } else if (q < R) {
-                const double2 v = *reinterpret_cast<const double2*>(V + (size_t)q * D + k);
-#pragma unroll
-                for (int i = 0; i < LR_ROWS; ++i) {
-                    o[i].x = __builtin_fma(m[i][q], v.x, o[i].x);
-                    o[i].y = __builtin_fma(m[i][q], v.y, o[i].y);
+        if constexpr (ATM) {
+#pragma unroll
+            for (int i = 0; i < LR_ROWS; ++i) {
+                double Mi[1][kLowRankMax], vx[kLowRankMax], vy[kLowRankMax], ox[1], oy[1];
+                const double ci[1] = {cf[i]};
+#pragma unroll
+                for (int q = 0; q < kLowRankMax; ++q) {
+                    const double2 v = q < Ri[i] ? *reinterpret_cast<const double2*>(Vi[i] + (size_t)q * D + k) : make_double2(0.0, 0.0);
+                    Mi[0][q] = m[i][q]; vx[q] = v.x; vy[q] = v.y;
                 }
-            }
-        }
-#pragma unroll
-        for (int i = 0; i < LR_ROWS; ++i) bstore2_aux<COH ? 17 : 0>(rC[i], k * 8, 0, make_double2(cf[i] * o[i].x, cf[i] * o[i].y));
+                lowrank_expand<1>(Mi, vx, Ri[i], ci, ox);
+                lowrank_expand<1>(Mi, vy, Ri[i], ci, oy);
+                o[i] = make_double2(ox[0], oy[0]);
+            }
+        } else {
+            double vx[kLowRankMax], vy[kLowRankMax], ox[LR_ROWS], oy[LR_ROWS];
+#pragma unroll
+            for (int q = 0; q < kLowRankMax; ++q) {
+                const double2 v = q < R ? *reinterpret_cast<const double2*>(V + (size_t)q * D + k) : make_double2(0.0, 0.0);
+                vx[q] = v.x; vy[q] = v.y;
+            }
+            lowrank_expand<LR_ROWS>(m, vx, R, cf, ox);
+            lowrank_expand<LR_ROWS>(m, vy, R, cf, oy);
+#pragma unroll
+            for (int i = 0; i < LR_ROWS; ++i) o[i] = make_double2(ox[i], oy[i]);
+        }
+#pragma unroll
+        for (int i = 0; i < LR_ROWS; ++i) bstore2_aux<COH ? 17 : 0>(rC[i], k * 8, 0, o[i]);
     }
 }
 template <bool COH, class RowOf, bool ATM = false>
diff --git a/sos-radiative-transfer_amd/csrc/kernels.hip b/sos-radiative-transfer_amd/csrc/kernels.hip
--- a/sos-radiative-transfer_amd/csrc/kernels.hip
+++ b/sos-radiative-transfer_amd/csrc/kernels.hip
@@ -1033,12 +1033,13 @@
 void launch_transport(hipStream_t s, const Grid& g, int B, const double* tau, const double* Jn, double* In, double* I,
                       double* saved, size_t saved_col_stride, const ColDesc* desc, Conv cv, int order,
                       int accumulate, const double* Etab, int mode, const int* erep, int live, const int* live_list,
-                      int ring_slots, int scan_split, double* scan_scratch, int* scan_sync, int nzcap) {
+                      int ring_slots, int scan_split, double* scan_scratch, int* scan_sync, int nzcap, const RingMoments* moments) {
     const int nt = round64(g.N);
     const size_t shm = (size_t)(g.L + 2 * TC * (nt + 2) + 2 * nt + nt / 64 + 2) * sizeof(double);
     TransportArgs a{g, tau, Jn, In, I, accumulate ? saved : nullptr, saved_col_stride, desc, cv, order, accumulate, Etab, Etab ? erep : nullptr, g_transport_stamps};
     a.slots = ring_slots;
     a.nzcap = nzcap > kRingZones ? nzcap : kRingZones;
+    if (mode == 3 && moments) { a.mom = moments->mom; a.lrV = moments->lrV; a.ca = moments->ca; a.lr_rank = moments->lr_rank; }
     if (mode == 4 && scan_split && scan_scratch && scan_sync) { a.scan_split = 1; a.scan_scratch = scan_scratch; a.scan_sync = scan_sync; }
     if ((mode == 3 || mode == 4) && accumulate && live > 0 && live < B && live_list) {
         a.live = live;
diff --git a/sos-radiative-transfer_amd/csrc/kernels.hpp b/sos-radiative-transfer_amd/csrc/kernels.hpp
--- a/sos-radiative-transfer_amd/csrc/kernels.hpp
+++ b/sos-radiative-transfer_amd/csrc/kernels.hpp
@@ -111,6 +111,16 @@
     int scan_split = 0;
     double* scan_scratch = nullptr;
     int* scan_sync = nullptr;
+    const double* mom = nullptr;
+    const double* lrV = nullptr;
+    const double* ca = nullptr;
+    int lr_rank = 0;
+};
+struct RingMoments {
+    const double* mom;
+    const double* lrV;
+    const double* ca;
+    int lr_rank;
 };
 void launch_transport_fast(hipStream_t s, dim3 grid, dim3 block, const TransportArgs& a);
 bool transport_ring_ok(const Grid& g);
@@ -179,6 +189,7 @@
     int lr_rank = -1;
     const double* lrU = nullptr;
     const double* lrV = nullptr;
+    double* mom = nullptr;
 };
 struct AtmSets {
     const int* col_atm = nullptr;
@@ -243,7 +254,7 @@
                       double* saved, size_t saved_col_stride, const ColDesc* desc, Conv cv, int order, int accumulate,
                       const double* Etab, int mode, const int* erep = nullptr, int live = 0, const int* live_list = nullptr,
                       int ring_slots = 0, int scan_split = 0, double* scan_scratch = nullptr, int* scan_sync = nullptr,
-                      int nzcap = kRingZones);
+                      int nzcap = kRingZones, const RingMoments* moments = nullptr );
 bool transport_fast_ok(const Plan& plan);
 void launch_attenuation(hipStream_t s, const Grid& g, int B, const double* tau, double* Etab, const int* erep);
 void launch_tau_groups(hipStream_t s, const Grid& g, int B, const double* tau, unsigned long long* hash, int* erep,
diff --git a/sos-radiative-transfer_amd/csrc/lowrank_expand.hpp b/sos-radiative-transfer_amd/csrc/lowrank_expand.hpp
--- /dev/null
+++ b/sos-radiative-transfer_amd/csrc/lowrank_expand.hpp
@@ -0,0 +1,32 @@
+#pragma once
+#include "kernels.hpp"
+
+namespace sosrt {
+namespace {
+
+template <int NR>
+__device__ __forceinline__ void lowrank_expand(const double (&M)[NR][kLowRankMax], const double (&V)[kLowRankMax], int R,
+                                               const double (&cf)[NR], double (&out)[NR]) {
+#pragma clang fp contract(off)
+#pragma unroll
+    for (int i = 0; i < NR; ++i) out[i] = 0.0;
+#pragma unroll
+    for (int q = 0; q < kLowRankMax; ++q)
+        if (q < R) {
+#pragma unroll
+            for (int i = 0; i < NR; ++i) out[i] = __builtin_fma(M[i][q], V[q], out[i]);
+        }
+#pragma unroll
+    for (int i = 0; i < NR; ++i) out[i] = cf[i] * out[i];
+}
+
+struct PlainRowSrc {
+    const double* mom = nullptr;
+    const double* ca = nullptr;
+    const double* V = nullptr;
+    int R = 0;
+    unsigned mixmask = 0;
+};
+
+}
+}
diff --git a/sos-radiative-transfer_amd/csrc/transport_ring.hip b/sos-radiative-transfer_amd/csrc/transport_ring.hip
--- a/sos-radiative-transfer_amd/csrc/transport_ring.hip
+++ b/sos-radiative-transfer_amd/csrc/transport_ring.hip
@@ -25,7 +25,10 @@
     asm volatile("s_waitcnt lgkmcnt(0)\n\ts_barrier" ::: "memory");
 }
 
-template <bool ACC, bool SAVED, int PIECES, bool MZ>
+typedef const __attribute__((address_space(4))) double* const_f64_t;
+__device__ __forceinline__ const_f64_t as_const(const double* p) { return reinterpret_cast<const_f64_t>(reinterpret_cast<uintptr_t>(p)); }
+
+template <bool ACC, bool SAVED, int PIECES, bool MZ, bool MOM>
 __global__ __launch_bounds__(512) void k_transport_ring(TransportArgs a, int NS, int dbg_arg, int fixcap) {
     constexpr int NWL = 2;
 #ifdef SOSRT_RING_DEBUG
@@ -74,6 +77,12 @@
     const int nz = dg->nz;
     const ZoneRows<MZ> zr(dg);
     const int nfix0 = dg->nfix[0], nfix1 = dg->nfix[1], nfix2 = dg->nfix[2];
+    unsigned mixmask = 0;
+    if constexpr (MOM) {
+#pragma unroll
+        for (int z = 0; z < (MZ ? kMaxZones : kRingZones); ++z) mixmask |= (z < nz && dg->mix[z]) ? 1u << z : 0u;
+    }
+    auto plain_row = [&](int t) { return MOM && !((mixmask >> zr.of(t)) & 1u); };
     const int surface = dg->surface;
     const double rho = dg->rho;
     const int fbytes = L * D * 8, RB = D * 8;
@@ -85,6 +94,9 @@
     const __amdgpu_buffer_rsrc_t rI = make_rsrc(ACC ? a.I + (size_t)b * L * D : a.In, ACC ? sbytes : 0);
     const __amdgpu_buffer_rsrc_t rS = make_rsrc(SAVED ? a.saved + (size_t)b * a.saved_col_stride : a.In, SAVED ? sbytes : 0);
     const int NCH = (L + TC - 1) / TC, NQ = 2 * NCH, R = NS - 1;
+    const const_f64_t momc = as_const(MOM ? a.mom + (size_t)b * L * kLowRankMax : nullptr);
+    const const_f64_t cac = as_const(MOM ? a.ca + (size_t)b * L : nullptr);
+    const int LR = MOM ? a.lr_rank : 0;
     const bool valid = tid < N;
     const int tidc = valid ? tid : N - 1;
     unsigned long long sp_dn = NCH > 64 ? ~0ull : 1ull << (NCH - 1), sp_up = sp_dn;
@@ -115,7 +127,8 @@
 #pragma unroll
             for (int p = 0; p < PIECES; ++p) {
                 const int so = row * RB + half + p * 1024;
-                __builtin_amdgcn_raw_ptr_buffer_load_lds(rJ, (lds_ptr_t)(dst + (0 * TC + u) * RS + p * 128), 16, vo, so, 0, 0);
+                const __amdgpu_buffer_rsrc_t rJu = MOM ? make_rsrc(a.Jn + (size_t)b * L * D, plain_row(row) ? 0 : lbytes) : rJ;
+                __builtin_amdgcn_raw_ptr_buffer_load_lds(rJu, (lds_ptr_t)(dst + (0 * TC + u) * RS + p * 128), 16, vo, so, 0, 0);
                 __builtin_amdgcn_raw_ptr_buffer_load_lds(rE, (lds_ptr_t)(dst + (1 * TC + u) * RS + p * 128), 16, vo, so, 0, 0);
                 if (ACC) __builtin_amdgcn_raw_ptr_buffer_load_lds(rIl, (lds_ptr_t)(dst + (2 * TC + u) * RS + p * 128), 16, vo, so, 0, 0);
             }
@@ -171,6 +184,27 @@
     } else {
     stamp(1);
     const double mu_up = (valid && tid > 0) ? g.mu[N + tidc] : 1.0;
+    double Vdn[kLowRankMax] = {0.0, 0.0, 0.0, 0.0}, Vup[kLowRankMax] = {0.0, 0.0, 0.0, 0.0};
+    if constexpr (MOM) {
+#pragma unroll
+        for (int q = 0; q < kLowRankMax; ++q) {
+            Vdn[q] = q < LR ? a.lrV[(size_t)q * D + tidc] : 0.0;
+            Vup[q] = q < LR ? a.lrV[(size_t)q * D + N + tidc] : 0.0;
+        }
+    }
+    auto expand_plain = [&](auto one_zone_t, const int (&r)[TC], const double (&V)[kLowRankMax], double (&Jc)[TC]) __attribute__((always_inline)) {
+        double M[TC][kLowRankMax], cf[TC], o[TC];
+#pragma unroll
+        for (int u = 0; u < TC; ++u) {
+#pragma unroll
+            for (int q = 0; q < kLowRankMax; ++q) M[u][q] = momc[r[u] * kLowRankMax + q];
+            cf[u] = cac[r[u]];
+        }
+        lowrank_expand<TC>(M, V, LR, cf, o);
+        const bool pl0 = plain_row(r[0]);
+#pragma unroll
+        for (int u = 0; u < TC; ++u) Jc[u] = (decltype(one_zone_t)::value ? pl0 : plain_row(r[u])) ? o[u] : Jc[u];
+    };
     const int uT = lane >> 3, pT = lane & 7;
     const double muT = (pT + 1 < N) ? g.mu[N + pT + 1] : 1.0;
     const double* xrow = s_x + uT * 16;
@@ -319,6 +353,12 @@
                 Ec[u] = sp[(1 * TC + u) * RS];
                 Ic[u] = ACC ? sp[(2 * TC + u) * RS] : 0.0;
             }
+            if constexpr (MOM) {
+                int r[TC];
+#pragma unroll
+                for (int u = 0; u < TC; ++u) r[u] = decltype(special_t)::value ? min(t0 + u, L - 1) : t0 + u;
+                expand_plain(std::integral_constant<bool, !decltype(special_t)::value>{}, r, Vdn, Jc);
+            }
             process(special_t, mode_t, sp - tid, Jc, Ic, Ec);
             wg_barrier();
         };
@@ -495,6 +535,12 @@
                 Ec[u] = sp[(1 * TC + u) * RS];
                 Ic[u] = ACC ? sp[(2 * TC + u) * RS] : 0.0;
             }
+            if constexpr (MOM) {
+                int r[TC];
+#pragma unroll
+                for (int u = 0; u < TC; ++u) r[u] = decltype(special_t)::value ? max(t0 - u, 0) : t0 - u;
+                expand_plain(std::integral_constant<bool, !decltype(special_t)::value>{}, r, Vup, Jc);
+            }
             process(special_t, mode_t, sp - tid, Jc, Ic, Ec);
             wg_barrier();
         };
@@ -529,8 +575,10 @@
         }
     }
     if (s_flag[0]) {
+        PlainRowSrc ps;
+        if constexpr (MOM) { ps.mom = a.mom + (size_t)b * L * kLowRankMax; ps.ca = a.ca + (size_t)b * L; ps.V = a.lrV; ps.R = LR; ps.mixmask = mixmask; }
         const bool missing = redo_upward_sweep<ACC, SAVED, MZ>(L, N, RB, zr, s_hd, g.mu, rJ, rE, rIn, rI, rS, Bv, ring,
-                                                            rup_v, rup_i);
+                                                            rup_v, rup_i, ps);
         if (missing) {
             if (tid == 0) {
                 a.cv.status[b] = SOSRT_COL_INDEXERROR;
@@ -567,15 +615,20 @@
     const int nt = (int)block.x;
     const int narr = a.accumulate ? 3 : 2;
     const size_t shm = ((size_t)NS * narr * TC * 128 * PIECES + ring_extra_doubles(a.g, nt, a.nzcap)) * sizeof(double);
-#define SOSRT_RING_LAUNCH_Z(ACC_, SAVED_, MZ_)                                                                 \
+#define SOSRT_RING_LAUNCH_M(ACC_, SAVED_, MZ_, MOM_)                                                           \
     do {                                                                                                       \
-        auto kern = k_transport_ring<ACC_, SAVED_, PIECES, MZ_>;                                               \
+        auto kern = k_transport_ring<ACC_, SAVED_, PIECES, MZ_, MOM_>;                                         \
         static PerDeviceOnce big_lds;                                                                                 \
         if (big_lds.first()) {                                                                                        \
             hipFuncSetAttribute(reinterpret_cast<const void*>(kern), hipFuncAttributeMaxDynamicSharedMemorySize, \
                                 (int)kRingLdsBytes);                                                                   \
         }                                                                                                      \
         hipLaunchKernelGGL(kern, grid, block, shm, s, a, NS, g_ring_debug, ring_fixcap(a.g));                           \
+    } while (0)
+#define SOSRT_RING_LAUNCH_Z(ACC_, SAVED_, MZ_)                                                                 \
+    do {                                                                                                       \
+        if (a.mom) SOSRT_RING_LAUNCH_M(ACC_, SAVED_, MZ_, true);                                               \
+        else SOSRT_RING_LAUNCH_M(ACC_, SAVED_, MZ_, false);                                                    \
     } while (0)
 #define SOSRT_RING_LAUNCH(ACC_, SAVED_)                                                                        \
     do {                                                                                                       \
@@ -590,6 +643,7 @@
     }
 #undef SOSRT_RING_LAUNCH
 #undef SOSRT_RING_LAUNCH_Z
+#undef SOSRT_RING_LAUNCH_M
 }
 
 }
diff --git a/sos-radiative-transfer_amd/csrc/transport_util.hpp b/sos-radiative-transfer_amd/csrc/transport_util.hpp
--- a/sos-radiative-transfer_amd/csrc/transport_util.hpp
+++ b/sos-radiative-transfer_amd/csrc/transport_util.hpp
@@ -2,6 +2,7 @@
 #include <hip/hip_runtime.h>
 
 #include "kernels.hpp"
+#include "lowrank_expand.hpp"
 
 namespace sosrt {
 namespace {
@@ -265,7 +266,7 @@
 __device__ SOSRT_HELPER_INLINE bool redo_upward_sweep(int L, int N, int RB, const ZoneRows<MZ>& zr, const double* s_hd,
                                   const double* __restrict__ gmu, __amdgpu_buffer_rsrc_t rJ, __amdgpu_buffer_rsrc_t rE,
                                   __amdgpu_buffer_rsrc_t rIn, __amdgpu_buffer_rsrc_t rI, __amdgpu_buffer_rsrc_t rS, double U0,
-                                  double* s_work, double& rup_v, double& rup_i) {
+                                  double* s_work, double& rup_v, double& rup_i, const PlainRowSrc& ps = PlainRowSrc()) {
     const int tid = threadIdx.x;
     double* s_row = s_work;
     int* s_kf = reinterpret_cast<int*>(s_work + 2 * (N + 2));
@@ -276,6 +277,11 @@
     const int vo = (N + j) * 8;
     double U = U0, Jnext = 0;
     bool missing = false;
+    double Vp[kLowRankMax] = {0.0, 0.0, 0.0, 0.0};
+    if (ps.mom) {
+#pragma unroll
+        for (int q = 0; q < kLowRankMax; ++q) Vp[q] = q < ps.R ? ps.V[(size_t)q * 2 * N + N + j] : 0.0;
+    }
     if (tid < 2) s_kf[tid] = 1 << 30;
     __syncthreads();
     int par = 0;
@@ -285,6 +291,14 @@
         for (int u = 0; u < kRedoRows; ++u) {
             const int t = max(t0 - u, 0);
             Jc[u] = bload_aux<LDX>(rJ, vo, t * RB);
+            if (ps.mom && !((ps.mixmask >> zr.of(t)) & 1)) {
+                double Mt[1][kLowRankMax], o[1];
+#pragma unroll
+                for (int q = 0; q < kLowRankMax; ++q) Mt[0][q] = ps.mom[(size_t)t * kLowRankMax + q];
+                const double cf[1] = {ps.ca[t]};
+                lowrank_expand<1>(Mt, Vp, ps.R, cf, o);
+                Jc[u] = o[0];
+            }
             Ec[u] = bload(rE, vo, t * RB);
             xo[u] = bload_aux<LDX ? LDX : 1>(rIn, vo, t * RB);
             Io[u] = ACC ? bload_aux<LDX ? LDX : 1>(rI, vo, t * RB) : 0.0;
diff --git a/sos-radiative-transfer_amd/sosrt/_lib.py b/sos-radiative-transfer_amd/sosrt/_lib.py
--- a/sos-radiative-transfer_amd/sosrt/_lib.py
+++ b/sos-radiative-transfer_amd/sosrt/_lib.py
@@ -36,6 +36,7 @@
     "sosrt_phase_rank": (c_int, [c_void_p, _ip, POINTER(c_double), _ip]),
     "sosrt_set_order_loop": (c_int, [c_void_p, c_int]),
     "sosrt_order_loop_stats": (c_int, [c_void_p, _ip, _ip, POINTER(c_longlong)]),
+    "sosrt_ring_moments_stats": (c_int, [c_void_p, _ip]),
     "sosrt_plan_launch": (c_int, [c_void_p, c_int, c_int, c_int, c_int, c_int, _ip]),
     "sosrt_set_first_order": (c_int, [c_void_p, c_int]),
     "sosrt_set_grid": (c_int, [c_void_p, c_void_p]),
diff --git a/sos-radiative-transfer_amd/sosrt/solver.py b/sos-radiative-transfer_amd/sosrt/solver.py
--- a/sos-radiative-transfer_amd/sosrt/solver.py
+++ b/sos-radiative-transfer_amd/sosrt/solver.py
@@ -99,6 +99,11 @@
         a, b, c = ctypes.c_int(), ctypes.c_int(), ctypes.c_longlong()
         check(lib().sosrt_order_loop_stats(self._h, ctypes.byref(a), ctypes.byref(b), ctypes.byref(c) if column_orders else None))
         return (a.value, b.value, c.value) if column_orders else (a.value, b.value)
+
+    def ring_moments_orders(self):
+        a = ctypes.c_int()
+        check(lib().sosrt_ring_moments_stats(self._h, ctypes.byref(a)))
+        return a.value
 
     def phase_asymmetry(self):
         a, u = ctypes.c_double(), ctypes.c_int()
```

Measured after the change: 130,800 (median of 5 runs). +5.1%, better.
